# bentherien/point-cloud-reid

Hardware: AMD Instinct MI355X
Metric: siamese pair-comparisons/sec @1024 pts (higher is better)
Workload: dtype bf16x3

## Files before the change

### include/pcr.h

```cpp
#ifndef PCR_H_
#define PCR_H_

#ifdef __cplusplus
extern "C" {
#endif

typedef void *pcr_stream_t;

enum pcr_status {
  PCR_OK = 0,
  PCR_ERR_INVALID = 1,
  PCR_ERR_LAUNCH = 2
};

int pcr_abi_version(void);
#define PCR_PREC_F32 0
#define PCR_PREC_BF16X3 1
#define PCR_PREC_BF16 2
const char *pcr_status_string(int status);


int pcr_fps_f32(const float *xyz, float *temp, int *idx, int B, int N, int M, pcr_stream_t stream);

int pcr_fps_dist_f32(const float *dist, float *temp, int *idx, int B, int N, int M,
                     pcr_stream_t stream);

int pcr_pairwise_sqdist_f32(const float *a, const float *b, float *out, int B, int N, int M, int C, int norm,
                            pcr_stream_t stream);

int pcr_ball_query_f32(const float *centres, const float *xyz, int *idx, int B, int N, int M,
                       float min_r, float max_r, int K, pcr_stream_t stream);

int pcr_ball_query_cnt_f32(const float *centres, const float *xyz, int *idx, int *cnt, int B, int N, int M,
                           float min_r, float max_r, int K, pcr_stream_t stream);

long pcr_ball_query_rows_floats(int B, int M, int K);
int pcr_ball_query_rows_ok(int N, int K, float min_r);
int pcr_ball_query_rows_f32(const float *centres, const float *xyz, int *idx, int *cnt, float *rows, int B, int N, int M,
                            float min_r, float max_r, int K, pcr_stream_t stream);

int pcr_fps_ball_query_rows_ok(int N, int M, int K);
int pcr_fps_ball_query_rows_f32(const float *xyz, float *temp, int *idx, float *new_xyz, int *cnt, float *rows, int B,
                                int N, int M, float max_r, int K, pcr_stream_t stream);

int pcr_fps_py_f32(const float *xyz, float *temp, const int *start, int *idx, int B, int N, int M,
                   pcr_stream_t stream);
int pcr_query_ball_point_f32(const float *centres, const float *xyz, int *idx, int B, int N, int M, float radius,
                             int K, pcr_stream_t stream);

int pcr_knn_f32(const float *xyz, const float *centres, int *idx, float *dist2, int B, int N, int M,
                int K, pcr_stream_t stream);

int pcr_gather_fwd_f32(const float *feat, const int *idx, float *out, int B, int C, int N, int M,
                       pcr_stream_t stream);
int pcr_gather_bwd_f32(const float *grad_out, const int *idx, float *grad_feat, int B, int C, int N,
                       int M, pcr_stream_t stream);

int pcr_group_fwd_f32(const float *feat, const int *idx, float *out, int B, int C, int N, int S,
                      int K, pcr_stream_t stream);
int pcr_group_bwd_f32(const float *grad_out, const int *idx, float *grad_feat, int B, int C, int N,
                      int S, int K, pcr_stream_t stream);

int pcr_three_nn_f32(const float *unknown, const float *known, float *dist2, int *idx, int B, int N,
                     int M, pcr_stream_t stream);

int pcr_three_interp_fwd_f32(const float *feat, const int *idx, const float *weight, float *out,
                             int B, int C, int M, int N, pcr_stream_t stream);
int pcr_three_interp_bwd_f32(const float *grad_out, const int *idx, const float *weight,
                             float *grad_feat, int B, int C, int N, int M, pcr_stream_t stream);


int pcr_box_frames_f32(const float *boxes, float *frames, int T, pcr_stream_t stream);

int pcr_points_in_boxes_batch_f32(const float *points, const float *boxes, int *out, int B, int P, int T,
                                  pcr_stream_t stream);

int pcr_points_in_boxes_f32(const float *points, const float *boxes, int *out, int B, int P, int T, pcr_stream_t stream);

#define PCR_CROP_FRAME_SENSOR 0
#define PCR_CROP_FRAME_CENTRED 1
#define PCR_CROP_FRAME_BOX 2
#define PCR_CROP_RULE_TRACKER 0
#define PCR_CROP_RULE_DATASET 1
#define PCR_CROP_MAX_POINTS 2617344
#define PCR_CROP_MAX_BOXES 65536
#define PCR_CROP_MAX_SAMPLES 65536
#define PCR_CROP_MAX_STRIDE 16
int pcr_crop_boxes_ok(int P, int M, int n, int stride);
int pcr_crop_boxes_f32(const float *points, int stride, const float *boxes, const int *rand, const long long *seed,
                       float *clouds, int *lengths, int P, int M, int n, int frame, int rule, int z_is_centre,
                       pcr_stream_t stream);


int pcr_knn_prefix_f32(const float *xyz, int *idx, int B, int N, int S, int K, pcr_stream_t stream);
int pcr_knn_prefix2_f32(const float *xyz, int *idx, int *idx2, int B, int N, int S, int K, int S2, int K2,
                        pcr_stream_t stream);

long pcr_packed_weight_floats(int cout, int cin);
int pcr_pack_weight_f32(const float *w, int cout, int cin, float *packed);
long pcr_packed_weight_bf16_floats(int cout, int cin);
int pcr_pack_weight_bf16x2_f32(const float *w, int cout, int cin, float *packed);

typedef struct pcr_sa_params {
  int mode, B, N, S, K, D;
  int c1, c2, c3;
  const float *xyz, *feat;
  const int *idx, *centre_idx;
  const float *wp[3], *scale[3], *shift[3];
  const float *wa, *wpq;
  const float *wps[2], *shift_pad[2];
  const int *cnt;
  int *tile_ws;
  float *pq_ws;
  int pq_ready;
  int feat_point_major, out_point_major;
  float *out;
  const float *wa_packed;
  int precision;
  const float *wps_bf[2];
  const float *wa_shift_packed;
  const float *row_tab;
  int *claim_ws;
  int pq_has_xyz;
} pcr_sa_params;
int pcr_sa_mlp_f32(const pcr_sa_params *p, pcr_stream_t stream);
long pcr_sa_claim_ws_ints(int c1, int c2, int c3, int K, int N, int precision);
long pcr_sa_tile_ws_ints(int B, int S, int K, int c2, int c3);
int pcr_sa_krow_uses_tiles(int c1, int c2, int c3, int K, int precision);
int pcr_sa_uses_row_table(int c1, int c2, int c3, int K, int precision);

int pcr_dense_pm_f32(const float *x, const float *wp, float *y, int B, int cin, int cout, int L,
                     int x_point_major, pcr_stream_t stream);
int pcr_dense_pm_prec_f32(const float *x, const float *wp_bf, float *y, int B, int cin, int cout, int L,
                          int x_point_major, int precision, pcr_stream_t stream);
int pcr_dense_pm_xyz_f32(const float *x, const float *wp_bf, const float *xyz, const float *wxyz, float *y, int B, int cin,
                         int cout, int L, int x_point_major, int precision, int q_rows, int q_off, pcr_stream_t stream);
int pcr_sa_tables_take_xyz(int mode, int D, int c1, int c2, int c3, int K, int precision);

typedef struct pcr_attn_params {
  int B, Lq, Sk;
  int c1, c2, d, cout;
  int nhead;
  int q_pos, residual;
  const float *feat_q, *xyz_q;
  const float *feat_k, *xyz_k;
  const int *kv_index;
  const int *q_index;
  const float *pos0_w, *pos0_b;
  const float *wq, *bq;
  const float *wkv, *bkv;
  const float *wmerge;
  const float *wmlp0, *wmlp2;
  const float *ln1_g, *ln1_b, *ln2_g, *ln2_b;
  const float *wfinal, *bfinal; int cfinal;
  const float *wkv_wide, *bkv_wide, *wmerge_packed;
  float *kv;
  float *out;
  int precision;
  const float *wq_bf, *wmlp0_bf, *wmlp2_bf, *wfinal_bf;
  int kv_splits;
  float *kv_part;
  const float *wkv_bf;
  const float *wmlp0_bf_xpad;
  float *pool_out;
} pcr_attn_params;
long pcr_attn_kv_floats(int d);
int pcr_attn_kv_splits(int B, int Sk, int d);
int pcr_attn_kv_f32(const pcr_attn_params *p, pcr_stream_t stream);
int pcr_attn_apply_f32(const pcr_attn_params *p, pcr_stream_t stream);
int pcr_attn_apply_pool_ok(const pcr_attn_params *p);

typedef struct pcr_head_params {
  int P, C, L, groups;
  const float *o;
  const float *w1, *w2;
  const float *gn1_g, *gn1_b, *gn2_g, *gn2_b;
  const float *w_out, *b_out;
  float *pooled, *logits;
  const float *w1t, *w2t;
} pcr_head_params;
int pcr_pool_head_f32(const pcr_head_params *p, pcr_stream_t stream);

int pcr_pool_both_f32(const float *x, float *out, int B, int C, int L, pcr_stream_t stream);

int pcr_channel_max_f32(const float *x, float *out, int B, int C, int L, int window, pcr_stream_t stream);

int pcr_dense_f32(const float *x, const float *wp, const float *scale, const float *shift, float *y,
                  int B, int cin, int cout, int L, int act, pcr_stream_t stream);
int pcr_dense_xpm_f32(const float *x, const float *wp, const float *scale, const float *shift, float *y,
                      int B, int cin, int cout, int L, int act, pcr_stream_t stream);

int pcr_dense_gn_f32(const float *x, const float *wp, const float *gamma, const float *beta, const float *res,
                     float *y, int B, int cin, int cout, int L, int groups, int relu, pcr_stream_t stream);
int pcr_dense_prec_ok(int cin, int cout, int L);
int pcr_dense_prec_f32(const float *x, const float *wp_bf, const float *scale, const float *shift, float *y, int B, int cin,
                       int cout, int L, int act, int precision, pcr_stream_t stream);
int pcr_dense_gn_prec_f32(const float *x, const float *wp_bf, const float *gamma, const float *beta, const float *res,
                          float *y, int B, int cin, int cout, int L, int groups, int relu, int precision,
                          pcr_stream_t stream);
int pcr_dense_xpm_prec_ok(int cin, int cout, int L);
int pcr_dense_xpm_prec_f32(const float *x, const float *wp_bf, const float *scale, const float *shift, float *y, int B,
                           int cin, int cout, int L, int act, int precision, pcr_stream_t stream);


int pcr_max_over_l_f32(const float *x, float *out, int B, int C, int L, pcr_stream_t stream);

int pcr_dense_max_ok(int cin, int cout, int L);
int pcr_dense_max_f32(const float *x, const float *wp, const float *scale, const float *shift, float *out, int B, int cin,
                      int cout, int L, int act, pcr_stream_t stream);

int pcr_pack_bmm_f32(const float *t, float *wp_per_cloud, int B, int k, pcr_stream_t stream);
int pcr_dense_bmm_f32(const float *x, const float *wp_per_cloud, float *y, int B, int cin, int cout, int L,
                      pcr_stream_t stream);

int pcr_groupnorm_f32(const float *x, const float *gamma, const float *beta, const float *res, float *y, int B,
                      int C, int L, int groups, int relu, pcr_stream_t stream);


int pcr_knn_feat_f32(const float *x, float *xx_ws, int *idx, int B, int C, int N, int K, long x_bstride,
                     pcr_stream_t stream);

int pcr_edge_max_f32(const float *ta, const float *tb, const int *idx, const float *shift, float slope, float *out,
                     long out_bstride, float *out2, long out2_bstride, int B, int N, int Co, int K,
                     pcr_stream_t stream);

int pcr_local_attn_f32(const float *qkv, const int *idx, float *msg, int B, int N, int C, int K, int nhead, float eps,
                       pcr_stream_t stream);


int pcr_pack_weight_dev_f32(const float *w, int rows, int cols, int ld, int transpose, float *packed, pcr_stream_t stream);

int pcr_train_groups(int B, int L);
int pcr_train_groups_bwd(int B, int L, int cout, int cin);
struct pcr_tdense_fwd;
struct pcr_tdense_bwd;
int pcr_tdense_fwd_groups(const struct pcr_tdense_fwd *p);
int pcr_tdense_bwd_groups(const struct pcr_tdense_bwd *p);
int pcr_set_stream_min_blocks(int n);

typedef struct pcr_tdense_fwd {
  int B, cin1, cin2, cout, L;
  const float *x, *x2;
  const float *isc, *ish;
  int in_relu;
  const float *wp, *bias;
  const float *res;
  int out_relu;
  float *y;
  float *stats;
  int pool_K;
  const float *pool_gamma;
  float *pool_ymax;
  int *pool_arg;
} pcr_tdense_fwd;
int pcr_tdense_fwd_f32(const pcr_tdense_fwd *p, pcr_stream_t stream);
int pcr_tdense_fwd_pooled(const pcr_tdense_fwd *p);

typedef struct pcr_tdense_bwd {
  int B, cin1, cin2, cout, L;
  const float *g, *y;
  int dy_mode;
  const float *ka, *kb, *kc;
  const int *argmax;
  const float *pooled;
  int K, S;
  const float *x, *x2;
  const float *isc, *ish, *iinv;
  int in_relu;
  const float *wpT;
  float *dx, *dx2, *dstats, *dwp, *dbp;
  long part_stride;
  int precision;
  const float *wpT_bf;
} pcr_tdense_bwd;
int pcr_tdense_bwd_f32(const pcr_tdense_bwd *p, pcr_stream_t stream);
int pcr_pack_weight_bf16_dev_f32(const float *w, int rows, int cols, int ld, int transpose, float *packed,
                                 pcr_stream_t stream);

int pcr_local_attn_train_fwd_f32(const float *qkv, const int *idx, float *msg, int B, int N, int C, int K, int nhead,
                                 float eps, pcr_stream_t stream);
int pcr_local_attn_train_bwd_f32(const float *qkv, const int *idx, const float *g, float *dq, long dq_bstride, float *edge,
                                 int B, int N, int C, int K, int nhead, float eps, pcr_stream_t stream);

int pcr_reduce_parts_f32(const float *part, int nparts, long stride, int rows, int cols, int ld, float *out,
                         pcr_stream_t stream);

typedef struct pcr_reduce_job {
  const float *part;
  float *out;
  long stride;
  int nparts, rows, cols, ld;
} pcr_reduce_job;
int pcr_reduce_multi_f32(const pcr_reduce_job *jobs, int n, pcr_stream_t stream);

typedef struct pcr_bn_fwd_fin {
  const float *part;
  int nparts, C;
  double R;
  const float *gamma, *beta;
  float eps, momentum;
  float *running_mean, *running_var;
  float *scale, *shift, *inv_scale, *mean, *invstd;
  const float *shift0;
  int shift0_stride;
} pcr_bn_fwd_fin;
int pcr_bn_fwd_finalize_f32(const pcr_bn_fwd_fin *p, pcr_stream_t stream);

typedef struct pcr_bn_bwd_fin {
  const float *part;
  int nparts, C;
  double R;
  const float *gamma, *mean, *invstd;
  float *ka, *kb, *kc, *dgamma, *dbeta;
  const float *centre;
} pcr_bn_bwd_fin;
int pcr_bn_bwd_finalize_f32(const pcr_bn_bwd_fin *p, pcr_stream_t stream);

int pcr_sa_l1_fwd_f32(const float *xyz, const int *idx, const float *tab, const float *wa, const float *bias,
                      float *y, float *stats, int B, int N, int S, int K, int c1, pcr_stream_t stream);
int pcr_sa_l1_bwd_f32(const float *xyz, const int *idx, const float *g, const float *y, const float *ka,
                      const float *kb, const float *kc, float *dtab, float *dwa, int B, int N, int S, int K, int c1,
                      pcr_stream_t stream);
int pcr_sa_pool_fwd_f32(const float *y, const float *scale, const float *shift, float *pooled, int *argmax, float *ymax,
                        int B, int C, int S, int K, pcr_stream_t stream);
int pcr_sa_pool_bwd_stats_f32(const float *gp, const float *pooled, const float *ymax, float *part, float *gz, int B, int C,
                              int S, pcr_stream_t stream);

int pcr_tnorm_fwd_f32(const float *x, const float *gamma, const float *beta, const float *res, float *y, float *mean,
                      float *rstd, int B, int C, int L, int G, float eps, int relu, pcr_stream_t stream);
int pcr_tnorm_bwd_f32(const float *g, const float *x, const float *gamma, const float *mean, const float *rstd,
                      const float *y_relu, float *dx, float *dres, float *part, int B, int C, int L, int G,
                      pcr_stream_t stream);

typedef struct pcr_linattn {
  int B, Lq, Sk, d, H;
  float eps;
  const float *q, *k, *v;
  long q_bs, k_bs, v_bs;
  float *out, *A, *ks;
  const float *dout;
  float *dq, *dk, *dv;
  long dq_bs, dk_bs, dv_bs;
  int kv_roll;
} pcr_linattn;
int pcr_linattn_fwd_f32(const pcr_linattn *p, pcr_stream_t stream);
int pcr_linattn_bwd_f32(const pcr_linattn *p, pcr_stream_t stream);

typedef struct pcr_attn_tail {
  int B, L, d, c1, hid, out, residual;
  float eps;
  const float *msg, *res;
  const float *wm, *w0, *w2, *wmT, *w0T, *w2T;
  const float *g1, *b1, *g2, *b2;
  float *outp;
  const float *dout;
  float *dmsg, *dres, *parts;
  long part_stride;
  int precision;
  int fwd_precision;
} pcr_attn_tail;
int pcr_attn_tail_ok(int d, int c1, int hid, int out, int residual);
int pcr_attn_tail_part_floats(int d, int c1, int hid, int out);
int pcr_attn_tail_groups(const pcr_attn_tail *p);
int pcr_attn_tail_fwd_f32(const pcr_attn_tail *p, pcr_stream_t stream);
int pcr_attn_tail_bwd_f32(const pcr_attn_tail *p, pcr_stream_t stream);

typedef struct pcr_attn_head {
  int B, L, c, hd, d, np, src;
  const float *x, *xyz;
  const float *p1, *p2, *c1, *c2, *p2T;
  const float *w[3], *wT[3];
  float *outp;
  const float *dout;
  float *dx, *parts;
  long part_stride;
  int precision;
  int fwd_precision;
} pcr_attn_head;
int pcr_attn_head_ok(int c, int hd, int d, int np, int src);
int pcr_attn_head_part_floats(int c, int hd, int d, int np, int src);
int pcr_attn_head_groups(const pcr_attn_head *p);
int pcr_attn_head_fwd_f32(const pcr_attn_head *p, pcr_stream_t stream);
int pcr_attn_head_bwd_f32(const pcr_attn_head *p, pcr_stream_t stream);

int pcr_pool_pair_fwd_f32(const float *o, float *pooled, int *arg, int P, int C, int L, pcr_stream_t stream);
int pcr_pool_pair_bwd_f32(const float *g, const int *arg, float *dout, int P, int C, int L, pcr_stream_t stream);
int pcr_pool_both_fwd_f32(const float *o, float *pooled, int *arg, int P, int C, int L, pcr_stream_t stream);
int pcr_pool_both_bwd_f32(const float *g, const int *arg, float *dout, int P, int C, int L, pcr_stream_t stream);
int pcr_channel_max_fwd_f32(const float *x, float *y, int *arg, int B, int C, int L, int W, pcr_stream_t stream);
int pcr_channel_max_bwd_f32(const float *g, const int *arg, float *dx, int B, int C, int L, int W, pcr_stream_t stream);

int pcr_bn_sums_f32(const float *y, const float *g, const float *scale, const float *shift, int relu, float slope,
                    const float *centre, int centre_first, float *part, int nparts, int B, int C, int L,
                    pcr_stream_t stream);
int pcr_bn_affine_f32(const float *y, const float *g, const float *a0, const float *a1, const float *a2,
                      const float *scale, const float *shift, const float *centre, int relu, float slope, float *out,
                      int B, int C, int L, pcr_stream_t stream);
int pcr_edge_pool_fwd_f32(const float *y, const float *scale, const float *shift, float slope, float *pooled, int *arg,
                          float *yraw, int B, int C, int N, int K, pcr_stream_t stream);
int pcr_edge_pool_route_f32(const float *gp, const float *pooled, const int *arg, float slope, float *g, int B, int C,
                            int N, int K, pcr_stream_t stream);
int pcr_bmm_apply_f32(const float *x, const float *T, float *y, int B, int k, int N, int transposed, pcr_stream_t stream);
int pcr_bmm_dt_f32(const float *x, const float *dy, float *dT, int B, int k, int N, pcr_stream_t stream);

typedef struct pcr_pack_desc {
  const float *w;
  float *out;
  int rows, cols;
  int kind;
  int reserved;
} pcr_pack_desc;
int pcr_pack_weights_multi_f32(const pcr_pack_desc *descs_dev, int n, pcr_stream_t stream);

typedef struct pcr_opt_tensor {
  float *p, *g, *m, *v;
  long n;
  float step_size, bc2_sqrt, decay, one_m_beta1, beta2, one_m_beta2, eps, pad_;
} pcr_opt_tensor;
int pcr_opt_chunk(void);
int pcr_grad_sumsq_f32(const pcr_opt_tensor *tab, const int *chunk_tensor, const int *chunk_first, int n_chunks,
                       double *part, pcr_stream_t stream);
int pcr_adamw_step_f32(const pcr_opt_tensor *tab, const int *chunk_tensor, const int *chunk_first, int n_chunks,
                       const double *part, float max_norm, float *grad_norm, pcr_stream_t stream);


int pcr_wall_clock_khz(void);
int pcr_last_launch_arith(void);
int pcr_clock_probe(unsigned long long *ticks, int n_wg, int iters, pcr_stream_t stream);

#ifdef __cplusplus
}
#endif
#endif
```

### point-cloud-reid_amd/csrc/attn_kernels_impl.h

```cpp
#pragma once
#ifndef PCR_ATTN_PREC
#define PCR_ATTN_PREC 0
#endif
#include "tile_dense.h"

#include <stdio.h>

#include <vector>

namespace {
constexpr int kAPrec = PCR_ATTN_PREC;
struct AttnArgs {
  pcr_attn_params p;
  int dbg;
  int wpc;
};

constexpr int kATraceWgs = 512, kATraceRecs = 24, kATraceMarks = 8;
__device__ unsigned long long g_attn_trace[2 * kATraceWgs * kATraceRecs * kATraceMarks];


__device__ __forceinline__ void pos_hidden(float *dst, int RP, const float *P, const float *w0,
                                           const float *b0, int d, int T) {
  for (int e = threadIdx.x; e < d * T; e += blockDim.x) {
    const int o = e / T, t = e - o * T;
    const float v = w0[o * 3] * P[t] + w0[o * 3 + 1] * P[RP + t] + w0[o * 3 + 2] * P[2 * RP + t] + b0[o];
    dst[o * RP + t] = fmaxf(v, 0.f);
  }
}

__device__ __forceinline__ void load_xyz3(float *P, int RP, const float *xyz, int L, int t0, int T) {
  for (int e = threadIdx.x; e < 3 * T; e += blockDim.x) {
    const int c = e / T, t = e - c * T;
    P[c * RP + t] = t0 + t < L ? xyz[(size_t)(t0 + t) * 3 + c] : 0.f;
  }
}

__device__ __forceinline__ void attn_kv_fold_write(const pcr_attn_params &p, const float *KVl, const float *s_kt, size_t b) {
  const int d = p.d, dh = d / p.nhead, ld = d + 1, tid = threadIdx.x;
  float *kv = p.kv + b * ((size_t)d * d + d);
  const int d_o = kThreads / d, d_dd = kThreads - d_o * d;
  int o = tid / d, dd = tid - o * d;
  int v0 = (dd / dh) * dh;
  for (int e = tid; e < d * d; e += kThreads, o += d_o, dd += d_dd) {
    if (dd >= d) {
      dd -= d;
      o++;
    }
    if (d_dd) v0 = (dd / dh) * dh;
    const float *wm = p.wmerge + (size_t)o * d + v0;
    const float *kr = KVl + dd * ld + v0;
    float m = 0.f;
#pragma unroll 8
    for (int v = 0; v < dh; v++) m += wm[v] * kr[v];
    if constexpr (kAPrec == 0) {
      const int kb = dd >> 3, rem = dd & 7;
      kv[(((size_t)kb * d + o) * 2 + (rem & 1)) * 4 + (rem >> 1)] = m;
    } else {
      const int s16 = dd >> 4, kk = dd & 15;
      const int hh = (kk >> 2) & 1, jj = (kk & 3) + ((kk >> 3) << 2);
      const size_t unit = (((size_t)s16 * (d >> 5) + (o >> 5)) * 2) * 64 + hh * 32 + (o & 31);
      const __bf16 hi = (__bf16)m;
      const __bf16 lo = (__bf16)(m - (float)hi);
      __bf16 *img = reinterpret_cast<__bf16 *>(kv);
      img[unit * 8 + jj] = hi;
      img[(unit + 64) * 8 + jj] = lo;
    }
  }
  __syncthreads();
  if (tid < d) kv[(size_t)d * d + tid] = s_kt[tid];
}

__device__ __forceinline__ void attn_kv_fold_mfma(const pcr_attn_params &p, const float *KVt, const float *s_kt, size_t b) {
  const int d = p.d, dh = d / p.nhead, ld = d + 1, tid = threadIdx.x;
  float *kv = p.kv + b * ((size_t)d * d + d);
  for (int hd = 0; hd < p.nhead; hd++) {
    const float *wm = p.wmerge_packed + (size_t)(hd * dh / 8) * d * 8;
    tile_dense(KVt + (size_t)(hd * dh) * ld + hd * dh, dh, ld, dh >> 5, wm, d, [&](float m, int o, int t) {
      const int dd = hd * dh + t;
      if constexpr (kAPrec == 0) {
        const int kb = dd >> 3, rem = dd & 7;
        kv[(((size_t)kb * d + o) * 2 + (rem & 1)) * 4 + (rem >> 1)] = m;
      } else {
        const int s16 = dd >> 4, kk = dd & 15;
        const int hh = (kk >> 2) & 1, jj = (kk & 3) + ((kk >> 3) << 2);
        const size_t unit = (((size_t)s16 * (d >> 5) + (o >> 5)) * 2) * 64 + hh * 32 + (o & 31);
        const __bf16 hi = (__bf16)m;
        const __bf16 lo = (__bf16)(m - (float)hi);
        __bf16 *img = reinterpret_cast<__bf16 *>(kv);
        img[unit * 8 + jj] = hi;
        img[(unit + 64) * 8 + jj] = lo;
      }
    });
  }
  __syncthreads();
  if (tid < d) kv[(size_t)d * d + tid] = s_kt[tid];
}

template <int TB, int NR, int WSEL, int NTW, bool BFP = false>
__device__ __forceinline__ void attn_kv_body(const AttnArgs &a) {
  constexpr int T = 32 * TB, RP = T + 1;
  constexpr int NPF = 4;
  extern __shared__ __attribute__((aligned(16))) float smem[];
  const pcr_attn_params &p = a.p;
  const int d = p.d, c2 = p.c2;
  float *XH = smem;
  float *KB = XH;
  float *VB = XH + d * RP;
  float *P = XH + (c2 + d) * RP;
  float *s_w0 = P + 3 * RP, *s_b0 = s_w0 + 3 * d;
  const int tail_a = (c2 + d + 3) * RP + 4 * d, tail_b = d * (d + 1) + d;
  float *s_ks = smem + (tail_a > tail_b ? tail_a : tail_b);
  const int tid = threadIdx.x, lane = tid & 63, wave = tid >> 6;
  const int l31 = lane & 31, h = lane >> 5;
  const size_t b = blockIdx.x;
  for (int e = tid; e < 3 * d; e += kThreads) s_w0[e] = p.pos0_w[e];
  for (int e = tid; e < d; e += kThreads) s_b0[e] = p.pos0_b[e];
  const float *feat = p.feat_k + b * c2 * p.Sk;
  const float *xyz = p.xyz_k + b * p.Sk * 3;
  const int nb = d >> 5, nT = nb * nb;
  const int dh = d / p.nhead;
  const float sk = (float)p.Sk;
  const float *bkv = p.bkv;

  f32x16 acc[NTW];
#pragma unroll
  for (int i = 0; i < NTW; i++)
#pragma unroll
    for (int r = 0; r < 16; r++) acc[i][r] = 0.f;
  int tile_ib[NTW];
#pragma unroll
  for (int it = 0; it < NTW; it++) tile_ib[it] = (wave + 4 * it) / nb;
  const int krow = tid % d, kpart = tid / d, kparts = kThreads / d;
  float ksum = 0.f;

  const int Q = T >> 2, npieces = c2 * Q;
#ifndef PCR_KV_PREFETCH
#define PCR_KV_PREFETCH 1
#endif
  const bool vec_ok = PCR_KV_PREFETCH && ((p.Sk & 3) == 0) && ((reinterpret_cast<size_t>(feat) & 15) == 0) && npieces <= NPF * kThreads;
  f32x4 pf[NPF];
  auto fetch = [&](int t0) {
#pragma unroll
    for (int u = 0; u < NPF; u++) {
      const int e = tid + u * kThreads;
      const int c = e / Q, q = e - c * Q;
      const bool ok = e < npieces;
      pf[u] = *reinterpret_cast<const f32x4 *>(feat + (size_t)(ok ? c : 0) * p.Sk + t0 + 4 * (ok ? q : 0));
    }
  };
  auto stash = [&]() {
#pragma unroll
    for (int u = 0; u < NPF; u++) {
      const int e = tid + u * kThreads;
      if (e < npieces) {
        const int c = e / Q, q = e - c * Q;
        float *dst = XH + c * RP + 4 * q;
        dst[0] = pf[u][0];
        dst[1] = pf[u][1];
        dst[2] = pf[u][2];
        dst[3] = pf[u][3];
      }
    }
  };
  const int nsplit = p.kv_splits > 1 ? p.kv_splits : 1;
  const int ntile = (p.Sk + T - 1) / T, tps = (ntile + nsplit - 1) / nsplit;
  const int t_lo = (int)blockIdx.y * tps * T;
  const int t_hi = (t_lo + tps * T) < p.Sk ? (t_lo + tps * T) : p.Sk;
  bool have = false;
  if (vec_ok && t_lo + T <= p.Sk && t_lo < t_hi) {
    fetch(t_lo);
    have = true;
  }
  for (int t0 = t_lo; t0 < t_hi; t0 += T) {
    const int valid = p.Sk - t0;
    if (have) stash();
    else load_tile(XH, RP, feat, c2, c2, p.Sk, t0, T);
    load_xyz3(P, RP, xyz, p.Sk, t0, T);
    __syncthreads();
    have = vec_ok && t0 + 2 * T <= p.Sk && t0 + T < t_hi;
    pos_hidden(XH + c2 * RP, RP, P, s_w0, s_b0, d, T);
    __syncthreads();
    auto kv_epi = [&](const f32x16 &acc, int cb, int tb, int l31, int h) {
      const int t = tb * 32 + l31;
      float *dst = XH + (cb * 32 + 4 * h) * RP + t;
      const bool live = t < valid;
      if (cb * 32 < d) {
#pragma unroll
        for (int r = 0; r < 16; r++) dst[((r & 3) + 8 * (r >> 2)) * RP] = live ? elu1(acc[r]) : 0.f;
      } else {
#pragma unroll
        for (int r = 0; r < 16; r++) dst[((r & 3) + 8 * (r >> 2)) * RP] = live ? acc[r] / sk : 0.f;
      }
    };
    auto kv_hook = [&]() { if (have) fetch(t0 + T); };
    if constexpr (BFP && kAPrec != 0 && WSEL != 0)
      tile_dense2p<kAPrec, TB, NR, WSEL, true>(XH, c2 + d, p.wkv_bf, 2 * d, true, kv_epi, bkv, nullptr, kv_hook);
    else
      tile_dense2<TB, NR, WSEL, true>(XH, c2 + d, p.wkv, 2 * d, true, kv_epi, bkv, nullptr, kv_hook);
    __syncthreads();
    {
      const float *row = KB + krow * RP;
      for (int t = kpart; t < T; t += kparts) ksum += row[t];
    }
#pragma unroll
    for (int it = 0; it < NTW; it++) {
      const int item = wave + 4 * it;
      if (item < nT) {
        const int ib = tile_ib[it], jb = item - ib * nb;
        const float *ap = KB + (ib * 32 + l31) * RP + h;
        const float *bp = VB + (jb * 32 + l31) * RP + h;
#pragma unroll 4
        for (int ks = 0; ks < T / 2; ks++)
          acc[it] = __builtin_amdgcn_mfma_f32_32x32x2f32(ap[2 * ks], bp[2 * ks], acc[it], 0, 0, 0);
      }
    }
    __syncthreads();
  }
  if (nsplit > 1) {
    float *part = p.kv_part + ((size_t)b * nsplit + blockIdx.y) * ((size_t)d * d + d);
    s_ks[tid] = ksum;
#pragma unroll
    for (int it = 0; it < NTW; it++) {
      const int item = wave + 4 * it;
      if (item < nT) {
        const int ib = tile_ib[it], jb = item - ib * nb;
#pragma unroll
        for (int r = 0; r < 16; r++)
          part[(size_t)(ib * 32 + (r & 3) + 8 * (r >> 2) + 4 * h) * d + jb * 32 + l31] = acc[it][r];
      }
    }
    __syncthreads();
    if (tid < d) {
      float s = 0.f;
      for (int pp = 0; pp < kparts; pp++) s += s_ks[pp * d + tid];
      part[(size_t)d * d + tid] = s;
    }
    return;
  }
  float *KVl = smem;
  const int ld = d + 1;
  const bool mfma_fold = p.wmerge_packed != nullptr && (dh & 31) == 0 && (d & 31) == 0;
  float *s_kt = smem + d * ld;
  s_ks[tid] = ksum;
#pragma unroll
  for (int it = 0; it < NTW; it++) {
    const int item = wave + 4 * it;
    if (item < nT) {
      const int ib = tile_ib[it], jb = item - ib * nb;
      const int v = jb * 32 + l31;
      const int hv = v / dh;
      const bool aligned = (dh & 31) == 0;
      const bool same_blk = (ib * 32) / dh == hv;
#pragma unroll
      for (int r = 0; r < 16; r++) {
        const int dd = ib * 32 + (r & 3) + 8 * (r >> 2) + 4 * h;
        const bool same = aligned ? same_blk : (dd / dh == hv);
        if (mfma_fold) KVl[v * ld + dd] = same ? acc[it][r] : 0.f;
        else KVl[dd * ld + v] = same ? acc[it][r] : 0.f;
      }
    }
  }
  __syncthreads();
  if (tid < d) {
    float s = 0.f;
    for (int pp = 0; pp < kparts; pp++) s += s_ks[pp * d + tid];
    s_kt[tid] = s;
  }
  if (mfma_fold) attn_kv_fold_mfma(p, KVl, s_kt, b);
  else attn_kv_fold_write(p, KVl, s_kt, b);
}

template <int TB, int NR, int WSEL, int NTW>
__global__ __launch_bounds__(kThreads) void attn_kv_kernel(AttnArgs a) {
  attn_kv_body<TB, NR, WSEL, NTW>(a);
}
template <int TB, int NR, int WSEL, int NTW>
__global__ __launch_bounds__(kThreads) __attribute__((amdgpu_waves_per_eu(3, 3))) void attn_kv_kernel_o3(AttnArgs a) {
  attn_kv_body<TB, NR, WSEL, NTW>(a);
}
template <int TB, int NR, int WSEL, int NTW, bool BFP = false>
__global__ __launch_bounds__(kThreads) __attribute__((amdgpu_waves_per_eu(2, 2))) void attn_kv_kernel_o2(AttnArgs a) {
  attn_kv_body<TB, NR, WSEL, NTW, BFP>(a);
}

constexpr int kKvsWaves = 8;
template <bool DIAG, bool BF, int XS = 4, bool ONEW = false>
__global__ __launch_bounds__(64 * kKvsWaves) __attribute__((amdgpu_waves_per_eu(2, 2)))
void attn_kv_stream64_kernel(AttnArgs a) {
  static_assert(BF || XS == 4, "the f32 form is c2 = 64 only");
  constexpr int D = 64, LD = D + 1, KVS = D * LD + D;
  constexpr int NKV = DIAG ? 2 : 4;
  constexpr int C2 = 16 * XS, WU = BF ? (XS + 4) * 512 : 4096, MINW = XS == 8 ? 4 : 2;
  extern __shared__ __attribute__((aligned(16))) float smem[];
  const pcr_attn_params &p = a.p;
  f32x4 *s_w = reinterpret_cast<f32x4 *>(smem);
  f32x4 *s_p0 = reinterpret_cast<f32x4 *>(smem + 4 * WU);
  float *s_bkv = smem + 4 * WU + 256;
  float *s_wm = s_bkv + 128;
  float *s_red = s_wm + D * LD;
  const int tid = threadIdx.x, lane = tid & 63, j = lane & 31, h = lane >> 5;
  const int wave = __builtin_amdgcn_readfirstlane(tid >> 6);
  {
    const f32x4 *src = reinterpret_cast<const f32x4 *>(BF ? p.wkv_bf : p.wkv);
    for (int e = tid; e < WU; e += 64 * kKvsWaves) s_w[e] = src[e];
    for (int e = tid; e < D * D; e += 64 * kKvsWaves) s_wm[(e >> 6) * LD + (e & 63)] = p.wmerge[e];
    if (tid < D) s_p0[tid] = f32x4{p.pos0_w[3 * tid], p.pos0_w[3 * tid + 1], p.pos0_w[3 * tid + 2], p.pos0_b[tid]};
    if (tid < 2 * D) s_bkv[tid] = p.bkv[tid];
  }
  __syncthreads();
  const int nblk = p.Sk >> 5;
  constexpr int kMaxWpc = 4;
  const int wpc = nblk < kMaxWpc ? nblk : kMaxWpc;
  int wpc2 = 1;
  while (wpc2 * 2 <= wpc) wpc2 *= 2;
  if (wpc2 < MINW) wpc2 = MINW;
  if constexpr (ONEW) wpc2 = 1;
  const int cpg = kKvsWaves / wpc2;
  const int cslot = wave / wpc2, wsub = wave - cslot * wpc2;
  const float inv_sk = 1.0f / (float)p.Sk;
  float bias[4];
#pragma unroll
  for (int cb = 0; cb < 4; cb++) bias[cb] = s_bkv[cb * 32 + j];
  const int dh = D / p.nhead;
#ifdef PCR_SA_TRACE_BUILD
  const bool tracing = (a.dbg & 256) && lane == 0 && (wave == 0 || wave == 5) && blockIdx.x < kATraceWgs;
  unsigned long long *trace = g_attn_trace + (size_t)(2 * blockIdx.x + (wave ? 1 : 0)) * (kATraceRecs * kATraceMarks);
  int trace_it = 0;
#define PCR_AMARK(m)                                                                                       \
  do {                                                                                                     \
    if (tracing && trace_it < kATraceRecs) trace[trace_it * kATraceMarks + (m)] = __builtin_readcyclecounter(); \
  } while (0)
#define PCR_ANEXT() trace_it++
#else
#define PCR_AMARK(m) do { } while (0)
#define PCR_ANEXT() do { } while (0)
#endif
  for (long c0 = (long)blockIdx.x * cpg; c0 < p.B; c0 += (long)gridDim.x * cpg) {
    const long b = c0 + cslot;
    const bool live = b < p.B;
    PCR_AMARK(4);
    f32x16 kv[NKV];
#pragma unroll
    for (int i = 0; i < NKV; i++)
#pragma unroll
      for (int r = 0; r < 16; r++) kv[i][r] = 0.f;
    float ks0 = 0.f, ks1 = 0.f;
    if (live) {
      const float *feat = p.feat_k + (size_t)b * C2 * p.Sk;
      const float *xyz = p.xyz_k + (size_t)b * p.Sk * 3;
      const __amdgpu_buffer_rsrc_t rfeat =
          __builtin_amdgcn_make_buffer_rsrc(const_cast<float *>(feat), 0, C2 * p.Sk * 4, 0x00020000);
      for (int blk = wsub; blk < nblk; blk += wpc2) {
        asm volatile("" ::: "memory");
        PCR_AMARK(0);
        const int t = blk * 32 + j;
        const float px = xyz[3 * t], py = xyz[3 * t + 1], pz = xyz[3 * t + 2];
        f32x16 acc[4];
        if constexpr (!BF) {
          float xr[64];
          {
            const int vo = (h * p.Sk + t) * 4;
#pragma unroll
            for (int s2 = 0; s2 < 32; s2++)
              xr[s2] = __builtin_bit_cast(float, __builtin_amdgcn_raw_buffer_load_b32(rfeat, vo, s2 * 2 * p.Sk * 4, 0));
          }
#pragma unroll
          for (int s2 = 0; s2 < 32; s2++) {
            const f32x4 w = s_p0[2 * s2 + h];
            const float v = w[0] * px + w[1] * py + w[2] * pz + w[3];
            xr[32 + s2] = fmaxf(v, 0.f);
          }
#pragma unroll
          for (int s2 = 0; s2 < 32; s2++) asm volatile("" : "+v"(xr[s2]));
#pragma unroll
          for (int cb = 0; cb < 4; cb++)
#pragma unroll
            for (int r = 0; r < 16; r++) acc[cb][r] = 0.f;
#pragma unroll
          for (int kb = 0; kb < 16; kb++) {
            f32x4 w[4];
#pragma unroll
            for (int cb = 0; cb < 4; cb++) w[cb] = s_w[((kb * 128 + cb * 32 + j) << 1) + h];
#pragma unroll
            for (int i = 0; i < 4; i++)
#pragma unroll
              for (int cb = 0; cb < 4; cb++)
                acc[cb] = __builtin_amdgcn_mfma_f32_32x32x2f32(xr[4 * kb + i], w[cb][i], acc[cb], 0, 0, 0);
          }
        } else {
          float xf[8 * XS];
          {
            const int vo = (4 * h * p.Sk + t) * 4;
#pragma unroll
            for (int e = 0; e < 8 * XS; e++) {
              const int ch = 16 * (e >> 3) + bf_kpos(0, e & 7);
              xf[e] = __builtin_bit_cast(float, __builtin_amdgcn_raw_buffer_load_b32(rfeat, vo, ch * p.Sk * 4, 0));
            }
          }
          bf16x8 ah[XS + 4], al[XS + 4];
#pragma unroll
          for (int s2 = 0; s2 < 4; s2++) {
            float hv[8];
#pragma unroll
            for (int e = 0; e < 8; e++) {
              const f32x4 w = s_p0[16 * s2 + bf_kpos(0, e) + 4 * h];
              const float v = w[0] * px + w[1] * py + w[2] * pz + w[3];
              hv[e] = relu_i(v);
            }
            bf_split8(hv, ah[XS + s2], al[XS + s2], true);
          }
#pragma unroll
          for (int e = 0; e < 8 * XS; e++) asm volatile("" : "+v"(xf[e]));
#pragma unroll
          for (int s2 = 0; s2 < XS; s2++) {
            float xv[8];
#pragma unroll
            for (int e = 0; e < 8; e++) xv[e] = xf[8 * s2 + e];
            bf_split8(xv, ah[s2], al[s2], true);
          }
#pragma unroll
          for (int cb = 0; cb < 4; cb++)
#pragma unroll
            for (int r = 0; r < 16; r++) acc[cb][r] = 0.f;
          PCR_AMARK(1);
          const bf16x8 *wb = reinterpret_cast<const bf16x8 *>(s_w) + lane;
#pragma unroll
          for (int s2 = 0; s2 < XS + 4; s2++) {
            bf16x8 wh[4], wl[4];
#pragma unroll
            for (int cb = 0; cb < 4; cb++) {
              wh[cb] = wb[((s2 * 4 + cb) * 2) * 64];
              wl[cb] = wb[((s2 * 4 + cb) * 2 + 1) * 64];
            }
#pragma unroll
            for (int cb = 0; cb < 4; cb++) acc[cb] = __builtin_amdgcn_mfma_f32_32x32x16_bf16(ah[s2], wh[cb], acc[cb], 0, 0, 0);
#pragma unroll
            for (int cb = 0; cb < 4; cb++) acc[cb] = __builtin_amdgcn_mfma_f32_32x32x16_bf16(al[s2], wh[cb], acc[cb], 0, 0, 0);
#pragma unroll
            for (int cb = 0; cb < 4; cb++) acc[cb] = __builtin_amdgcn_mfma_f32_32x32x16_bf16(ah[s2], wl[cb], acc[cb], 0, 0, 0);
          }
        }
        PCR_AMARK(2);
#pragma unroll
        for (int r = 0; r < 16; r++) {
          acc[0][r] = elu1(acc[0][r] + bias[0]);
          acc[1][r] = elu1(acc[1][r] + bias[1]);
          acc[2][r] = (acc[2][r] + bias[2]) * inv_sk;
          acc[3][r] = (acc[3][r] + bias[3]) * inv_sk;
          ks0 += acc[0][r];
          ks1 += acc[1][r];
        }
#pragma unroll
        for (int i = 0; i < NKV; i++) {
          const int ib = DIAG ? i : (i >> 1), jb = DIAG ? i : (i & 1);
#pragma unroll
          for (int r = 0; r < 16; r++) {
            if constexpr (ONEW) kv[i] = __builtin_amdgcn_mfma_f32_32x32x2f32(acc[2 + jb][r], acc[ib][r], kv[i], 0, 0, 0);
            else kv[i] = __builtin_amdgcn_mfma_f32_32x32x2f32(acc[ib][r], acc[2 + jb][r], kv[i], 0, 0, 0);
          }
        }
        PCR_AMARK(3);
      }
    }
    PCR_AMARK(5);
    ks0 += __shfl_xor(ks0, 32, 64);
    ks1 += __shfl_xor(ks1, 32, 64);
    if constexpr (ONEW) {
      if (live) {
        float *kvo = p.kv + (size_t)b * ((size_t)D * D + D);
        bf16x8 *img = reinterpret_cast<bf16x8 *>(kvo);
#pragma unroll
        for (int db = 0; db < 2; db++) {
          const int hd = (db * 32 + j) / dh;
#pragma unroll
          for (int ob = 0; ob < 2; ob++) {
            f32x16 m;
#pragma unroll
            for (int r = 0; r < 16; r++) m[r] = 0.f;
#pragma unroll
            for (int i = 0; i < NKV; i++) {
              const int ib = DIAG ? i : (i >> 1), jb = DIAG ? i : (i & 1);
              if (ib != db) continue;
              const float *wr = s_wm + (ob * 32 + j) * LD + jb * 32 + 4 * h;
#pragma unroll
              for (int r = 0; r < 16; r++) {
                const int vl = (r & 3) + 8 * (r >> 2);
                const float av = (jb * 32 + vl + 4 * h) / dh == hd ? kv[i][r] : 0.f;
                m = __builtin_amdgcn_mfma_f32_32x32x2f32(av, wr[vl], m, 0, 0, 0);
              }
            }
#pragma unroll
            for (int G = 0; G < 2; G++) {
              float v[8];
#pragma unroll
              for (int e = 0; e < 8; e++) v[e] = m[8 * G + e];
              bf16x8 hi, lo;
              bf_split8(v, hi, lo, true);
              const size_t unit = (((size_t)(db * 2 + G) * (D >> 5) + ob) * 2) * 64 + h * 32 + j;
              img[unit] = hi;
              img[unit + 64] = lo;
            }
          }
        }
        if (h == 0) {
          kvo[(size_t)D * D + j] = ks0;
          kvo[(size_t)D * D + 32 + j] = ks1;
        }
      }
      PCR_AMARK(6);
      PCR_AMARK(7);
      PCR_ANEXT();
      continue;
    }
    float *KVl = s_red + cslot * KVS, *s_kt = KVl + D * LD;
    for (int round = 0; round < wpc2; round++) {
      if (wsub == round) {
#pragma unroll
        for (int i = 0; i < NKV; i++) {
          const int ib = DIAG ? i : (i >> 1), jb = DIAG ? i : (i & 1);
#pragma unroll
          for (int r = 0; r < 16; r++) {
            const int dd = ib * 32 + (r & 3) + 8 * (r >> 2) + 4 * h, v = jb * 32 + j;
            float *dst = KVl + dd * LD + v;
            *dst = round == 0 ? kv[i][r] : *dst + kv[i][r];
          }
        }
        if (h == 0) {
          s_kt[j] = round == 0 ? ks0 : s_kt[j] + ks0;
          s_kt[32 + j] = round == 0 ? ks1 : s_kt[32 + j] + ks1;
        }
      }
      __syncthreads();
    }
    PCR_AMARK(6);
    if (live) {
      float *kvo = p.kv + (size_t)b * ((size_t)D * D + D);
      for (int ti = wsub; ti < 4; ti += wpc2) {
        const int ob = ti >> 1, db = ti & 1;
        const float *ap = s_wm + (ob * 32 + j) * LD + h;
        const float *bp = KVl + (db * 32 + j) * LD + h;
        const int hd = (db * 32 + j) / dh;
        f32x16 m;
#pragma unroll
        for (int r = 0; r < 16; r++) m[r] = 0.f;
        const int s_lo = DIAG ? db * 16 : 0, s_hi = DIAG ? db * 16 + 16 : 32;
        if constexpr (kAPrec == 0) {
#pragma unroll 4
          for (int s2 = s_lo; s2 < s_hi; s2++) {
            const float bv = bp[2 * s2];
            m = __builtin_amdgcn_mfma_f32_32x32x2f32(ap[2 * s2], (2 * s2 + h) / dh == hd ? bv : 0.f, m, 0, 0, 0);
          }
          const int dd = db * 32 + j;
#pragma unroll
          for (int r = 0; r < 16; r++) {
            const int o = ob * 32 + (r & 3) + 8 * (r >> 2) + 4 * h;
            const int kb = dd >> 3, rem = dd & 7;
            kvo[(((size_t)kb * D + o) * 2 + (rem & 1)) * 4 + (rem >> 1)] = m[r];
          }
        } else {
#pragma unroll 4
          for (int s2 = s_lo; s2 < s_hi; s2++) {
            const float bv = bp[2 * s2];
            m = __builtin_amdgcn_mfma_f32_32x32x2f32((2 * s2 + h) / dh == hd ? bv : 0.f, ap[2 * s2], m, 0, 0, 0);
          }
          bf16x8 *img = reinterpret_cast<bf16x8 *>(kvo);
#pragma unroll
          for (int G = 0; G < 2; G++) {
            float v[8];
#pragma unroll
            for (int e = 0; e < 8; e++) v[e] = m[8 * G + e];
            bf16x8 hi, lo;
            bf_split8(v, hi, lo, true);
            const size_t unit = (((size_t)(db * 2 + G) * (D >> 5) + ob) * 2) * 64 + h * 32 + j;
            img[unit] = hi;
            img[unit + 64] = lo;
          }
        }
      }
      for (int e = wsub * 64 + lane; e < D; e += 64 * wpc2) kvo[(size_t)D * D + e] = s_kt[e];
    }
    PCR_AMARK(7);
    PCR_ANEXT();
    __syncthreads();
  }
#undef PCR_AMARK
#undef PCR_ANEXT
}

#if PCR_ATTN_PREC != 0
__global__ __launch_bounds__(64 * kKvsWaves) __attribute__((amdgpu_waves_per_eu(2, 4)))
void attn_kv_stream32_kernel(AttnArgs a) {
  constexpr int D = 32, LD = D + 1, KVS = D * LD + D;
  extern __shared__ __attribute__((aligned(16))) float smem[];
  const pcr_attn_params &p = a.p;
  f32x4 *s_w = reinterpret_cast<f32x4 *>(smem);
  f32x4 *s_p0 = reinterpret_cast<f32x4 *>(smem + 4096);
  float *s_bkv = smem + 4096 + 128;
  float *s_wm = s_bkv + 64;
  float *s_red = s_wm + D * LD;
  const int tid = threadIdx.x, lane = tid & 63, j = lane & 31, h = lane >> 5;
  const int wave = __builtin_amdgcn_readfirstlane(tid >> 6);
  {
    const f32x4 *src = reinterpret_cast<const f32x4 *>(p.wkv_bf);
    for (int e = tid; e < 1024; e += 64 * kKvsWaves) s_w[e] = src[e];
    for (int e = tid; e < D * D; e += 64 * kKvsWaves) s_wm[(e >> 5) * LD + (e & 31)] = p.wmerge[e];
    if (tid < D) s_p0[tid] = f32x4{p.pos0_w[3 * tid], p.pos0_w[3 * tid + 1], p.pos0_w[3 * tid + 2], p.pos0_b[tid]};
    if (tid < 2 * D) s_bkv[tid] = p.bkv[tid];
  }
  __syncthreads();
  const int nblk = p.Sk >> 5;
  const int wpc = nblk < kKvsWaves ? nblk : kKvsWaves;
  int wpc2 = 1;
  while (wpc2 * 2 <= wpc) wpc2 *= 2;
  if (wpc2 < 2) wpc2 = 2;
  const int cpg = kKvsWaves / wpc2;
  const int cslot = wave / wpc2, wsub = wave - cslot * wpc2;
  const float inv_sk = 1.0f / (float)p.Sk;
  const float bias0 = s_bkv[j], bias1 = s_bkv[32 + j];
  const int dh = D / p.nhead;
  for (long c0 = (long)blockIdx.x * cpg; c0 < p.B; c0 += (long)gridDim.x * cpg) {
    const long b = c0 + cslot;
    const bool live = b < p.B;
    f32x16 kv;
#pragma unroll
    for (int r = 0; r < 16; r++) kv[r] = 0.f;
    float ks = 0.f;
    if (live) {
      const float *feat = p.feat_k + (size_t)b * D * p.Sk;
      const float *xyz = p.xyz_k + (size_t)b * p.Sk * 3;
      const __amdgpu_buffer_rsrc_t rfeat =
          __builtin_amdgcn_make_buffer_rsrc(const_cast<float *>(feat), 0, D * p.Sk * 4, 0x00020000);
      for (int blk = wsub; blk < nblk; blk += wpc2) {
        asm volatile("" ::: "memory");
        const int t = blk * 32 + j;
        const float px = xyz[3 * t], py = xyz[3 * t + 1], pz = xyz[3 * t + 2];
        float xf[16];
        {
          const int vo = (4 * h * p.Sk + t) * 4;
#pragma unroll
          for (int e = 0; e < 16; e++) {
            const int ch = 16 * (e >> 3) + bf_kpos(0, e & 7);
            xf[e] = __builtin_bit_cast(float, __builtin_amdgcn_raw_buffer_load_b32(rfeat, vo, ch * p.Sk * 4, 0));
          }
        }
        bf16x8 ah[4], al[4];
#pragma unroll
        for (int s2 = 0; s2 < 2; s2++) {
          float hv[8];
#pragma unroll
          for (int e = 0; e < 8; e++) {
            const f32x4 w = s_p0[16 * s2 + bf_kpos(0, e) + 4 * h];
            const float v = w[0] * px + w[1] * py + w[2] * pz + w[3];
            hv[e] = relu_i(v);
          }
          bf_split8(hv, ah[2 + s2], al[2 + s2], true);
        }
#pragma unroll
        for (int e = 0; e < 16; e++) asm volatile("" : "+v"(xf[e]));
#pragma unroll
        for (int s2 = 0; s2 < 2; s2++) {
          float xv[8];
#pragma unroll
          for (int e = 0; e < 8; e++) xv[e] = xf[8 * s2 + e];
          bf_split8(xv, ah[s2], al[s2], true);
        }
        f32x16 acc[2];
#pragma unroll
        for (int cb = 0; cb < 2; cb++)
#pragma unroll
          for (int r = 0; r < 16; r++) acc[cb][r] = 0.f;
        const bf16x8 *wb = reinterpret_cast<const bf16x8 *>(s_w) + lane;
#pragma unroll
        for (int s2 = 0; s2 < 4; s2++) {
          bf16x8 wh[2], wl[2];
#pragma unroll
          for (int cb = 0; cb < 2; cb++) {
            wh[cb] = wb[((s2 * 2 + cb) * 2) * 64];
            wl[cb] = wb[((s2 * 2 + cb) * 2 + 1) * 64];
          }
#pragma unroll
          for (int cb = 0; cb < 2; cb++) acc[cb] = __builtin_amdgcn_mfma_f32_32x32x16_bf16(ah[s2], wh[cb], acc[cb], 0, 0, 0);
#pragma unroll
          for (int cb = 0; cb < 2; cb++) acc[cb] = __builtin_amdgcn_mfma_f32_32x32x16_bf16(al[s2], wh[cb], acc[cb], 0, 0, 0);
#pragma unroll
          for (int cb = 0; cb < 2; cb++) acc[cb] = __builtin_amdgcn_mfma_f32_32x32x16_bf16(ah[s2], wl[cb], acc[cb], 0, 0, 0);
        }
#pragma unroll
        for (int r = 0; r < 16; r++) {
          acc[0][r] = elu1(acc[0][r] + bias0);
          acc[1][r] = (acc[1][r] + bias1) * inv_sk;
          ks += acc[0][r];
        }
#pragma unroll
        for (int r = 0; r < 16; r++) kv = __builtin_amdgcn_mfma_f32_32x32x2f32(acc[0][r], acc[1][r], kv, 0, 0, 0);
      }
    }
    ks += __shfl_xor(ks, 32, 64);
    float *KVl = s_red + cslot * KVS, *s_kt = KVl + D * LD;
    for (int round = 0; round < wpc2; round++) {
      if (wsub == round) {
#pragma unroll
        for (int r = 0; r < 16; r++) {
          float *dst = KVl + ((r & 3) + 8 * (r >> 2) + 4 * h) * LD + j;
          *dst = round == 0 ? kv[r] : *dst + kv[r];
        }
        if (h == 0) s_kt[j] = round == 0 ? ks : s_kt[j] + ks;
      }
      __syncthreads();
    }
    if (live && wsub == 0) {
      float *kvo = p.kv + (size_t)b * ((size_t)D * D + D);
      const float *ap = s_wm + j * LD + h;
      const float *bp = KVl + j * LD + h;
      const int hd = j / dh;
      f32x16 m;
#pragma unroll
      for (int r = 0; r < 16; r++) m[r] = 0.f;
#pragma unroll 4
      for (int s2 = 0; s2 < 16; s2++) {
        const float bv = bp[2 * s2];
        m = __builtin_amdgcn_mfma_f32_32x32x2f32((2 * s2 + h) / dh == hd ? bv : 0.f, ap[2 * s2], m, 0, 0, 0);
      }
      bf16x8 *img = reinterpret_cast<bf16x8 *>(kvo);
#pragma unroll
      for (int G = 0; G < 2; G++) {
        float v[8];
#pragma unroll
        for (int e = 0; e < 8; e++) v[e] = m[8 * G + e];
        bf16x8 hi, lo;
        bf_split8(v, hi, lo, true);
        const size_t unit = (((size_t)G * (D >> 5)) * 2) * 64 + h * 32 + j;
        img[unit] = hi;
        img[unit + 64] = lo;
      }
      if (lane < D) kvo[(size_t)D * D + lane] = s_kt[lane];
    }
    __syncthreads();
  }
}
#endif

__global__ __launch_bounds__(kThreads) void attn_kv_fold_kernel(AttnArgs a) {
  extern __shared__ __attribute__((aligned(16))) float smem[];
  const pcr_attn_params &p = a.p;
  const int d = p.d, dh = d / p.nhead, ld = d + 1, nsplit = p.kv_splits, tid = threadIdx.x;
  const size_t b = blockIdx.x, per = (size_t)d * d + d;
  float *KVl = smem, *s_kt = smem + d * ld;
  const float *part = p.kv_part + b * nsplit * per;
  for (int e = tid; e < d * d + d; e += kThreads) {
    float v = part[e];
    for (int y = 1; y < nsplit; y++) v += part[(size_t)y * per + e];
    if (e < d * d) {
      const int dd = e / d, c = e - dd * d;
      KVl[dd * ld + c] = (dd / dh == c / dh) ? v : 0.f;
    } else {
      s_kt[e - d * d] = v;
    }
  }
  __syncthreads();
  attn_kv_fold_write(p, KVl, s_kt, b);
}

#if PCR_ATTN_PREC == 0
template <int NRW>
__global__ __launch_bounds__(kThreads) void attn_kv_wide_kernel(AttnArgs a) {
  constexpr int TB = 1, T = 32, RP = 33, BAND = 64, RPK = BAND + 1;
  extern __shared__ __attribute__((aligned(16))) float smem[];
  const pcr_attn_params &p = a.p;
  const int d = p.d, c2 = p.c2, dh = d / p.nhead;
  const int g = blockIdx.x, hd = (g * BAND) / dh;
  const int OPW = BAND + dh;
  float *XH = smem;
  float *KB = XH, *VB = XH + BAND * RP;
  float *P = XH + (c2 + d) * RP;
  float *s_w0 = P + 3 * RP, *s_b0 = s_w0 + 3 * d;
  float *s_ks = s_b0 + d;
  const int tid = threadIdx.x, lane = tid & 63, wave = tid >> 6;
  const int l31 = lane & 31, h = lane >> 5;
  const size_t b = blockIdx.y;
  for (int e = tid; e < 3 * d; e += kThreads) s_w0[e] = p.pos0_w[e];
  for (int e = tid; e < d; e += kThreads) s_b0[e] = p.pos0_b[e];
  const float *feat = p.feat_k + b * c2 * p.Sk;
  const float *xyz = p.xyz_k + b * p.Sk * 3;
  const float sk = (float)p.Sk;
  const float *wband = p.wkv_wide + (size_t)g * ((size_t)ceil8(c2 + d) * OPW);
  const float *bband = p.bkv_wide + (size_t)g * OPW;
  const int nj = dh >> 5, nT = 2 * nj;
  f32x16 acc[4];
#pragma unroll
  for (int i = 0; i < 4; i++)
#pragma unroll
    for (int r = 0; r < 16; r++) acc[i][r] = 0.f;
  const int krow = tid & (BAND - 1), kpart = tid >> 6;
  float ksum = 0.f;
  for (int t0 = 0; t0 < p.Sk; t0 += T) {
    const int valid = p.Sk - t0;
    load_tile(XH, RP, feat, c2, c2, p.Sk, t0, T);
    load_xyz3(P, RP, xyz, p.Sk, t0, T);
    __syncthreads();
    pos_hidden(XH + c2 * RP, RP, P, s_w0, s_b0, d, T);
    __syncthreads();
    tile_dense2<TB, NRW, 0, true>(XH, c2 + d, wband, OPW, true,
                                  [&](const f32x16 &acc, int cb, int tb, int l31, int h) {
      const int t = tb * 32 + l31;
      float *dst = XH + (cb * 32 + 4 * h) * RP + t;
      const bool live = t < valid;
      if (cb * 32 < BAND) {
#pragma unroll
        for (int r = 0; r < 16; r++) dst[((r & 3) + 8 * (r >> 2)) * RP] = live ? elu1(acc[r]) : 0.f;
      } else {
#pragma unroll
        for (int r = 0; r < 16; r++) dst[((r & 3) + 8 * (r >> 2)) * RP] = live ? acc[r] / sk : 0.f;
      }
    }, bband);
    __syncthreads();
    {
      const float *row = KB + krow * RP;
      for (int t = kpart; t < T; t += 4) ksum += row[t];
    }
#pragma unroll
    for (int it = 0; it < 4; it++) {
      const int item = wave + 4 * it;
      if (item < nT) {
        const int ib = item / nj, jb = item - ib * nj;
        const float *ap = KB + (ib * 32 + l31) * RP + h;
        const float *bp = VB + (jb * 32 + l31) * RP + h;
#pragma unroll 4
        for (int ks = 0; ks < T / 2; ks++)
          acc[it] = __builtin_amdgcn_mfma_f32_32x32x2f32(ap[2 * ks], bp[2 * ks], acc[it], 0, 0, 0);
      }
    }
    __syncthreads();
  }
  float *KVt = smem;
  s_ks[tid] = ksum;
  __syncthreads();
  const float ks_total = tid < BAND ? s_ks[tid] + s_ks[64 + tid] + s_ks[128 + tid] + s_ks[192 + tid] : 0.f;
  __syncthreads();
#pragma unroll
  for (int it = 0; it < 4; it++) {
    const int item = wave + 4 * it;
    if (item < nT) {
      const int ib = item / nj, jb = item - ib * nj;
      const int v = jb * 32 + l31;
#pragma unroll
      for (int r = 0; r < 16; r++) KVt[v * RPK + ib * 32 + (r & 3) + 8 * (r >> 2) + 4 * h] = acc[it][r];
    }
  }
  __syncthreads();
  float *kv = p.kv + b * ((size_t)d * d + d);
  if (tid < BAND) kv[(size_t)d * d + g * BAND + tid] = ks_total;
  const float *wm = p.wmerge_packed + (size_t)(hd * dh / 8) * d * 8;
  tile_dense(KVt, dh, RPK, 2, wm, d, [&](float m, int o, int t) {
    const int dd = g * BAND + t;
    const int kb = dd >> 3, rem = dd & 7;
    kv[(((size_t)kb * d + o) * 2 + (rem & 1)) * 4 + (rem >> 1)] = m;
  });
}

#endif

template <int TB, int NR>
__global__ __launch_bounds__(kThreads) void attn_apply_kernel(AttnArgs a) {
  constexpr int T = 32 * TB, RP = T + 1;
  extern __shared__ __attribute__((aligned(16))) float smem[];
  const pcr_attn_params &p = a.p;
  const int d = p.d, c1 = p.c1, cout = p.cout;
  const int catC = c1 + d, catP = ceil8(catC);
  int rowsU = catP > 2 * d ? catP : 2 * d;
  if (ceil32(cout) > rowsU) rowsU = ceil32(cout);
  if (ceil32(p.cfinal) > rowsU) rowsU = ceil32(p.cfinal);
  float *U = smem;
  float *P = U + rowsU * RP;
  float *zs = P + 3 * RP;
  float *red = zs + p.nhead * RP;
  float *cst = red + 2 * (kThreads / T) * T;
  float *s_ksum = cst, *s_ln1g = cst + d, *s_ln1b = cst + 2 * d, *s_ln2g = cst + 3 * d, *s_ln2b = s_ln2g + cout;
  float *s_w0 = s_ln2b + cout, *s_b0 = s_w0 + 3 * d;
  const int tid = threadIdx.x;
  const size_t b = blockIdx.y;
  const int t0 = blockIdx.x * T;
  const size_t bq_ = p.q_index ? (size_t)p.q_index[b] : b;
  const float *feat = p.feat_q + bq_ * c1 * p.Lq;
  const size_t kb_ = p.kv_index ? (size_t)p.kv_index[b] : b;
  const float *kv = p.kv + kb_ * ((size_t)d * d + d);
  const int dh = d / p.nhead;
  for (int e = tid; e < d; e += kThreads) {
    s_ksum[e] = kv[(size_t)d * d + e];
    s_ln1g[e] = p.ln1_g[e];
    s_ln1b[e] = p.ln1_b[e];
    if (p.q_pos) {
      s_w0[3 * e] = p.pos0_w[3 * e];
      s_w0[3 * e + 1] = p.pos0_w[3 * e + 1];
      s_w0[3 * e + 2] = p.pos0_w[3 * e + 2];
      s_b0[e] = p.pos0_b[e];
    }
  }
  for (int e = tid; e < cout; e += kThreads) {
    s_ln2g[e] = p.ln2_g[e];
    s_ln2b[e] = p.ln2_b[e];
  }
  const float *ksum = s_ksum;
  float *MSG = U + c1 * RP;

  load_tile(U, RP, feat, c1, c1, p.Lq, t0, T);
  if (p.q_pos) {
    load_xyz3(P, RP, p.xyz_q + bq_ * p.Lq * 3, p.Lq, t0, T);
    __syncthreads();
    pos_hidden(MSG, RP, P, s_w0, s_b0, d, T);
    for (int e = tid; e < (catP - catC) * T; e += kThreads) U[(catC + e / T) * RP + e % T] = 0.f;
  } else {
    for (int e = tid; e < (catP - c1) * T; e += kThreads) U[(c1 + e / T) * RP + e % T] = 0.f;
  }
  __syncthreads();
  tile_dense2p<kAPrec, TB, NR>(U, p.q_pos ? catP : ceil8(c1), p.wq, d, true,
                               [&](float v, int o, int t) { MSG[o * RP + t] = elu1(v); }, p.bq);
  __syncthreads();
  for (int e = tid; e < p.nhead * T; e += kThreads) {
    const int hd = e / T, t = e - hd * T;
    float z = 0.f;
    for (int c = 0; c < dh; c++) z += MSG[(hd * dh + c) * RP + t] * ksum[hd * dh + c];
    zs[hd * RP + t] = (1.0f / (z + 1e-6f)) * (float)p.Sk;
  }
  __syncthreads();
  for (int hd = 0; hd < p.nhead; hd++)
    for (int e = tid; e < dh * T; e += kThreads) {
      const int o = hd * dh + e / T, t = e % T;
      MSG[o * RP + t] *= zs[hd * RP + t];
    }
  __syncthreads();
  tile_dense2p<kAPrec, TB, NR>(MSG, d, kv, d, true, [&](float v, int o, int t) { MSG[o * RP + t] = v; });
  __syncthreads();
  tile_layernorm(MSG, d, RP, T, s_ln1g, s_ln1b, red);
  tile_dense2p<kAPrec, TB, NR>(U, catP, p.wmlp0, 2 * d, true, [&](float v, int o, int t) { U[o * RP + t] = fmaxf(v, 0.f); });
  __syncthreads();
  tile_dense2p<kAPrec, TB, NR>(U, 2 * d, p.wmlp2, ceil32(cout), true, [&](float v, int o, int t) { U[o * RP + t] = v; });
  __syncthreads();
  tile_layernorm(U, cout, RP, T, s_ln2g, s_ln2b, red);
  if (p.residual) {
    for (int e = tid; e < cout * T; e += kThreads) {
      const int c = e / T, t = e - c * T;
      if (t0 + t < p.Lq) U[c * RP + t] += feat[(size_t)c * p.Lq + t0 + t];
    }
    __syncthreads();
  }
  int cres = cout;
  if (p.cfinal) {
    const int cf = p.cfinal;
    tile_dense2p<kAPrec, TB, NR>(U, cout, p.wfinal, ceil32(cf), true, [&](float v, int o, int t) { U[o * RP + t] = v; },
                                 p.bfinal);
    __syncthreads();
    cres = cf;
  }
  float *out = p.out + b * cres * p.Lq;
  for (int e = tid; e < cres * T; e += kThreads) {
    const int c = e / T, t = e - c * T;
    if (t0 + t < p.Lq) out[(size_t)c * p.Lq + t0 + t] = U[c * RP + t];
  }
}

#if PCR_ATTN_PREC != 0
constexpr int kApsWaves = 8;
template <bool QPOS, int C1S, int CF, int NOB = 2, int ND = 2, bool POOL = false>
__global__ __launch_bounds__(64 * kApsWaves) __attribute__((amdgpu_waves_per_eu(2, 2)))
void attn_apply_stream64_kernel(AttnArgs a) {
  static_assert(!QPOS || C1S == 2 * ND, "q_pos needs c1 == d");
  static_assert(NOB <= 2 || (NOB == 4 && !CF), "cout = 128 has no trailing conv");
  static_assert(!POOL || (!CF && NOB == 2), "pooled output: cout = 64, no trailing conv");
  constexpr int D = 32 * ND, SD = 2 * ND;
  constexpr int SQ = C1S + (QPOS ? SD : 0), S0 = C1S + SD, NX = 8 * C1S;
  extern __shared__ __attribute__((aligned(16))) float smem[];
  const pcr_attn_params &p = a.p;
  bf16x8 *s_wq = reinterpret_cast<bf16x8 *>(smem);
  bf16x8 *s_w0 = s_wq + SQ * ND * 128;
  bf16x8 *s_w2 = s_w0 + S0 * ND * 256;
  float *s_c = reinterpret_cast<float *>(s_w2 + ND * NOB * 512);
  f32x4 *s_p0 = reinterpret_cast<f32x4 *>(s_c + 448);
  float *s_ks = reinterpret_cast<float *>(s_p0 + 64);
  const int tid = threadIdx.x, lane = tid & 63, j = lane & 31, h = lane >> 5;
  const int wave = __builtin_amdgcn_readfirstlane(tid >> 6);
  {
    const f32x4 *wq = reinterpret_cast<const f32x4 *>(p.wq),
                *w0 = reinterpret_cast<const f32x4 *>((p.c1 & 15) ? p.wmlp0_bf_xpad : p.wmlp0),
                *w2 = reinterpret_cast<const f32x4 *>(p.wmlp2);
    f32x4 *dq = reinterpret_cast<f32x4 *>(s_wq), *d0 = reinterpret_cast<f32x4 *>(s_w0), *d2 = reinterpret_cast<f32x4 *>(s_w2);
    for (int e = tid; e < SQ * ND * 128; e += 64 * kApsWaves) dq[e] = wq[e];
    for (int e = tid; e < S0 * ND * 256; e += 64 * kApsWaves) d0[e] = w0[e];
    for (int e = tid; e < ND * NOB * 512; e += 64 * kApsWaves) d2[e] = w2[e];
    if (tid < D) {
      s_c[tid] = p.bq[tid];
      s_c[64 + tid] = p.ln1_g[tid];
      s_c[128 + tid] = p.ln1_b[tid];

      if (QPOS) s_p0[tid] = f32x4{p.pos0_w[3 * tid], p.pos0_w[3 * tid + 1], p.pos0_w[3 * tid + 2], p.pos0_b[tid]};
    }
    if (tid < 32 * NOB) {
      s_c[192 + tid] = p.ln2_g[tid];
      s_c[192 + 32 * NOB + tid] = p.ln2_b[tid];
    }
    if (CF && tid < 32 * CF) s_c[320 + tid] = p.bfinal[tid];
  }
  __syncthreads();
  const int nblk = p.Lq >> 5;
  const long nitem = (long)p.B * nblk;
  const int dh = D / p.nhead;
  const float skf = (float)p.Sk;
  float *ksw = s_ks + wave * 64;
  auto cvec = [&](const float *base, int cb, int g) __attribute__((always_inline)) {
    return *reinterpret_cast<const f32x4 *>(base + 32 * cb + 8 * g + 4 * h);
  };
  auto to_ops = [&](const f32x16 &acc, int G, bf16x8 &oh, bf16x8 &ol) __attribute__((always_inline)) {
    float v[8];
#pragma unroll
    for (int e = 0; e < 8; e++) v[e] = acc[8 * G + e];
    bf_split8(v, oh, ol, true);
  };
#ifdef PCR_SA_TRACE_BUILD
  const bool tracing = (a.dbg & 256) && lane == 0 && (wave == 0 || wave == 5) && blockIdx.x < kATraceWgs;
  unsigned long long *trace = g_attn_trace + (size_t)(2 * blockIdx.x + (wave ? 1 : 0)) * (kATraceRecs * kATraceMarks);
  int trace_it = 0;
#define PCR_AMARK(m)                                                                                       \
  do {                                                                                                     \
    if (tracing && trace_it < kATraceRecs) trace[trace_it * kATraceMarks + (m)] = __builtin_readcyclecounter(); \
  } while (0)
#define PCR_ANEXT() trace_it++
#else
#define PCR_AMARK(m) do { } while (0)
#define PCR_ANEXT() do { } while (0)
#endif
  const long nwav = (long)gridDim.x * kApsWaves, gw = (long)blockIdx.x * kApsWaves + wave;
  long pc = gw;
  int pblk = 0;
  float pmax = -INFINITY, psum = 0.f;
  for (long it = gw; POOL ? pc < p.B : it < nitem; it += POOL ? 0 : nwav) {
    asm volatile("" ::: "memory");
    PCR_AMARK(0);
    const long b = POOL ? pc : it / nblk;
    const int blk = POOL ? pblk : (int)(it - b * nblk);
    const size_t bq_ = p.q_index ? (size_t)p.q_index[b] : (size_t)b;
    const size_t kb_ = p.kv_index ? (size_t)p.kv_index[b] : (size_t)b;
    const float *kvp = p.kv + kb_ * ((size_t)D * D + D);
    const int t = blk * 32 + j;
    const __amdgpu_buffer_rsrc_t rfeat = __builtin_amdgcn_make_buffer_rsrc(
        const_cast<float *>(p.feat_q + bq_ * p.c1 * p.Lq), 0, p.c1 * p.Lq * 4, 0x00020000);
    const int vo = (4 * h * p.Lq + t) * 4;
    float xf[NX];
#pragma unroll
    for (int e = 0; e < NX; e++) {
      const int ch = 16 * (e >> 3) + bf_kpos(0, e & 7);
      xf[e] = __builtin_bit_cast(float, __builtin_amdgcn_raw_buffer_load_b32(rfeat, vo, ch * p.Lq * 4, 0));
    }
    if (lane < D) ksw[lane] = kvp[(size_t)D * D + lane];
    bf16x8 bh[4 * ND], bl[4 * ND];
    if constexpr (QPOS) {
      const float *xyz = p.xyz_q + (bq_ * p.Lq + t) * 3;
      const float px = xyz[0], py = xyz[1], pz = xyz[2];
#pragma unroll
      for (int s2 = 0; s2 < SD; s2++) {
        float hv[8];
#pragma unroll
        for (int e = 0; e < 8; e++) {
          const f32x4 w = s_p0[16 * s2 + bf_kpos(0, e) + 4 * h];
          const float v = w[0] * px + w[1] * py + w[2] * pz + w[3];
          hv[e] = relu_i(v);
        }
        bf_split8(hv, bh[C1S + s2], bl[C1S + s2], true);
      }
    }
#pragma unroll
    for (int e = 0; e < NX; e++) asm volatile("" : "+v"(xf[e]));
#pragma unroll
    for (int s2 = 0; s2 < C1S; s2++) {
      float xv[8];
#pragma unroll
      for (int e = 0; e < 8; e++) xv[e] = xf[8 * s2 + e];
      bf_split8(xv, bh[s2], bl[s2], true);
    }
    PCR_AMARK(1);
    f32x16 q[ND];
#pragma unroll
    for (int cb = 0; cb < ND; cb++)
#pragma unroll
      for (int r = 0; r < 16; r++) q[cb][r] = 0.f;
    {
      const bf16x8 *wb = s_wq + lane;
#pragma unroll
      for (int s2 = 0; s2 < SQ; s2++) {
        bf16x8 wh[ND], wl[ND];
#pragma unroll
        for (int cb = 0; cb < ND; cb++) {
          wh[cb] = wb[((s2 * ND + cb) * 2) * 64];
          wl[cb] = wb[((s2 * ND + cb) * 2 + 1) * 64];
        }
#pragma unroll
        for (int cb = 0; cb < ND; cb++) q[cb] = __builtin_amdgcn_mfma_f32_32x32x16_bf16(wh[cb], bh[s2], q[cb], 0, 0, 0);
#pragma unroll
        for (int cb = 0; cb < ND; cb++) q[cb] = __builtin_amdgcn_mfma_f32_32x32x16_bf16(wh[cb], bl[s2], q[cb], 0, 0, 0);
#pragma unroll
        for (int cb = 0; cb < ND; cb++) q[cb] = __builtin_amdgcn_mfma_f32_32x32x16_bf16(wl[cb], bh[s2], q[cb], 0, 0, 0);
      }
    }
    PCR_AMARK(2);
    bf16x8 mh[SD][ND], ml[SD][ND];
    {
      const bf16x8 *mb = reinterpret_cast<const bf16x8 *>(kvp) + lane;
#pragma unroll
      for (int s2 = 0; s2 < SD; s2++)
#pragma unroll
        for (int cb = 0; cb < ND; cb++) {
          mh[s2][cb] = mb[((s2 * ND + cb) * 2) * 64];
          ml[s2][cb] = mb[((s2 * ND + cb) * 2 + 1) * 64];
        }
    }
    __builtin_amdgcn_fence(__ATOMIC_RELEASE, "wavefront");
    __builtin_amdgcn_wave_barrier();
    __builtin_amdgcn_fence(__ATOMIC_ACQUIRE, "wavefront");
    float z16[2][2] = {{0.f, 0.f}, {0.f, 0.f}};
#pragma unroll
    for (int cb = 0; cb < ND; cb++)
#pragma unroll
      for (int g = 0; g < 4; g++) {
        const f32x4 bqv = cvec(s_c, cb, g), ksv = cvec(ksw, cb, g);
        float zz = 0.f;
#pragma unroll
        for (int qq = 0; qq < 4; qq++) {
          const float v = elu1(q[cb][4 * g + qq] + bqv[qq]);
          q[cb][4 * g + qq] = v;
          zz += v * ksv[qq];
        }
        if ((g & 1) == 0) z16[cb][g >> 1] = zz;
        else z16[cb][g >> 1] += zz;
      }
    float zs[2][2];
    {
      float za = z16[0][0], zb = z16[0][1], zc = z16[1][0], zd = z16[1][1];
      if (dh >= 32) {
        za += zb; zb = za;
        zc += zd; zd = zc;
      }
      if (ND == 2 && dh >= 64) {
        za += zc; zb = za; zc = za; zd = za;
      }
      za += __shfl_xor(za, 32, 64);
      zb += __shfl_xor(zb, 32, 64);
      zc += __shfl_xor(zc, 32, 64);
      zd += __shfl_xor(zd, 32, 64);
      zs[0][0] = (1.0f / (za + 1e-6f)) * skf;
      zs[0][1] = (1.0f / (zb + 1e-6f)) * skf;
      zs[1][0] = (1.0f / (zc + 1e-6f)) * skf;
      zs[1][1] = (1.0f / (zd + 1e-6f)) * skf;
    }
#pragma unroll
    for (int cb = 0; cb < ND; cb++)
#pragma unroll
      for (int r = 0; r < 16; r++) q[cb][r] *= zs[cb][r >> 3];
    bf16x8 ch_[SD], cl_[SD];
#pragma unroll
    for (int cb = 0; cb < ND; cb++)
#pragma unroll
      for (int G = 0; G < 2; G++) to_ops(q[cb], G, ch_[2 * cb + G], cl_[2 * cb + G]);
    f32x16 m[ND];
#pragma unroll
    for (int cb = 0; cb < ND; cb++)
#pragma unroll
      for (int r = 0; r < 16; r++) m[cb][r] = 0.f;
#pragma unroll
    for (int s2 = 0; s2 < SD; s2++) {
#pragma unroll
      for (int cb = 0; cb < ND; cb++) m[cb] = __builtin_amdgcn_mfma_f32_32x32x16_bf16(mh[s2][cb], ch_[s2], m[cb], 0, 0, 0);
#pragma unroll
      for (int cb = 0; cb < ND; cb++) m[cb] = __builtin_amdgcn_mfma_f32_32x32x16_bf16(mh[s2][cb], cl_[s2], m[cb], 0, 0, 0);
#pragma unroll
      for (int cb = 0; cb < ND; cb++) m[cb] = __builtin_amdgcn_mfma_f32_32x32x16_bf16(ml[s2][cb], ch_[s2], m[cb], 0, 0, 0);
    }
    auto layernorm = [&](auto &v, auto nb_tag, const float *gam, const float *bet) __attribute__((always_inline)) {
      constexpr int NB = decltype(nb_tag)::value;
      float sm = 0.f;
#pragma unroll
      for (int cb = 0; cb < NB; cb++)
#pragma unroll
        for (int r = 0; r < 16; r++) sm += v[cb][r];
      sm += __shfl_xor(sm, 32, 64);
      const float mean = sm / (32.0f * NB);
      float vr = 0.f;
#pragma unroll
      for (int cb = 0; cb < NB; cb++)
#pragma unroll
        for (int r = 0; r < 16; r++) {
          const float dlt = v[cb][r] - mean;
          vr += dlt * dlt;
        }
      vr += __shfl_xor(vr, 32, 64);
      const float inv = 1.0f / sqrtf(vr / (32.0f * NB) + 1e-5f);
#pragma unroll
      for (int cb = 0; cb < NB; cb++)
#pragma unroll
        for (int g = 0; g < 4; g++) {
          const f32x4 gv = cvec(gam, cb, g), bv = cvec(bet, cb, g);
#pragma unroll
          for (int qq = 0; qq < 4; qq++) v[cb][4 * g + qq] = (v[cb][4 * g + qq] - mean) * inv * gv[qq] + bv[qq];
        }
    };
    PCR_AMARK(3);
    layernorm(m, std::integral_constant<int, ND>{}, s_c + 64, s_c + 128);
    PCR_AMARK(4);
#pragma unroll
    for (int s2 = 0; s2 < C1S; s2++) {
      float xv[8];
#pragma unroll
      for (int e = 0; e < 8; e++) xv[e] = xf[8 * s2 + e];
      bf_split8(xv, bh[s2], bl[s2], true);
    }
#pragma unroll
    for (int cb = 0; cb < ND; cb++)
#pragma unroll
      for (int G = 0; G < 2; G++) to_ops(m[cb], G, bh[C1S + 2 * cb + G], bl[C1S + 2 * cb + G]);
    f32x16 f[SD];
#pragma unroll
    for (int cb = 0; cb < SD; cb++)
#pragma unroll
      for (int r = 0; r < 16; r++) f[cb][r] = 0.f;
    {
      const bf16x8 *wb = s_w0 + lane;
#pragma unroll
      for (int s2 = 0; s2 < S0; s2++) {
        bf16x8 wh[SD], wl[SD];
#pragma unroll
        for (int cb = 0; cb < SD; cb++) {
          wh[cb] = wb[((s2 * SD + cb) * 2) * 64];
          wl[cb] = wb[((s2 * SD + cb) * 2 + 1) * 64];
        }
#pragma unroll
        for (int cb = 0; cb < SD; cb++) f[cb] = __builtin_amdgcn_mfma_f32_32x32x16_bf16(wh[cb], bh[s2], f[cb], 0, 0, 0);
#pragma unroll
        for (int cb = 0; cb < SD; cb++) f[cb] = __builtin_amdgcn_mfma_f32_32x32x16_bf16(wh[cb], bl[s2], f[cb], 0, 0, 0);
#pragma unroll
        for (int cb = 0; cb < SD; cb++) f[cb] = __builtin_amdgcn_mfma_f32_32x32x16_bf16(wl[cb], bh[s2], f[cb], 0, 0, 0);
      }
    }
#pragma unroll
    for (int cb = 0; cb < SD; cb++) {
#pragma unroll
      for (int r = 0; r < 16; r++) f[cb][r] = relu_i(f[cb][r]);
#pragma unroll
      for (int G = 0; G < 2; G++) to_ops(f[cb], G, bh[2 * cb + G], bl[2 * cb + G]);
    }
    PCR_AMARK(5);
    f32x16 o[NOB];
#pragma unroll
    for (int cb = 0; cb < NOB; cb++)
#pragma unroll
      for (int r = 0; r < 16; r++) o[cb][r] = 0.f;
    {
      const bf16x8 *wb = s_w2 + lane;
#pragma unroll
      for (int s2 = 0; s2 < 4 * ND; s2++) {
        bf16x8 wh[NOB], wl[NOB];
#pragma unroll
        for (int cb = 0; cb < NOB; cb++) {
          wh[cb] = wb[((s2 * NOB + cb) * 2) * 64];
          wl[cb] = wb[((s2 * NOB + cb) * 2 + 1) * 64];
        }
#pragma unroll
        for (int cb = 0; cb < NOB; cb++) o[cb] = __builtin_amdgcn_mfma_f32_32x32x16_bf16(wh[cb], bh[s2], o[cb], 0, 0, 0);
#pragma unroll
        for (int cb = 0; cb < NOB; cb++) o[cb] = __builtin_amdgcn_mfma_f32_32x32x16_bf16(wh[cb], bl[s2], o[cb], 0, 0, 0);
#pragma unroll
        for (int cb = 0; cb < NOB; cb++) o[cb] = __builtin_amdgcn_mfma_f32_32x32x16_bf16(wl[cb], bh[s2], o[cb], 0, 0, 0);
      }
    }
    PCR_AMARK(6);
    layernorm(o, std::integral_constant<int, NOB>{}, s_c + 192, s_c + 192 + 32 * NOB);
    if constexpr (C1S == 2 * NOB) {
      if (p.residual) {
#pragma unroll
        for (int cb = 0; cb < NOB; cb++)
#pragma unroll
          for (int r = 0; r < 16; r++) o[cb][r] += xf[16 * cb + r];
      }
    }
    if constexpr (POOL) {
      float vm[16], vs[16];
      {
        const bool up = (j & 1) != 0;
#pragma unroll
        for (int r = 0; r < 16; r++) {
          const float lo_ = o[r >> 4][r & 15], hi_ = o[(r + 16) >> 4][(r + 16) & 15];
          const float tk = up ? hi_ : lo_, uk = up ? lo_ : hi_;
          const float pu = __uint_as_float(pcr_sort_partner<2, 1>(__float_as_uint(uk), lane));
          vm[r] = fmaxf(tk, pu);
          vs[r] = tk + pu;
        }
      }
#define PCR_POOL_STEP(N, J, BIT)                                                                      \
      {                                                                                               \
        const bool up = (j & BIT) != 0;                                                               \
        _Pragma("unroll") for (int r = 0; r < N; r++) {                                               \
          const float tm = up ? vm[r + N] : vm[r], um = up ? vm[r] : vm[r + N];                       \
          const float ts = up ? vs[r + N] : vs[r], us = up ? vs[r] : vs[r + N];                       \
          vm[r] = fmaxf(tm, __uint_as_float(pcr_sort_partner<2 * J, J>(__float_as_uint(um), lane)));  \
          vs[r] = ts + __uint_as_float(pcr_sort_partner<2 * J, J>(__float_as_uint(us), lane));        \
        }                                                                                             \
      }
      PCR_POOL_STEP(8, 2, 2)
      PCR_POOL_STEP(4, 4, 4)
      PCR_POOL_STEP(2, 8, 8)
      PCR_POOL_STEP(1, 16, 16)
#undef PCR_POOL_STEP
      pmax = fmaxf(pmax, vm[0]);
      psum += vs[0];
      if (++pblk == nblk) {
        const int e = ((j & 1) << 4) | ((j & 2) << 2) | (j & 4) | ((j & 8) >> 2) | ((j & 16) >> 4);
        const int ch = 16 * (e >> 3) + bf_kpos(h, e & 7);
        float *po = p.pool_out + (size_t)b * 128;
        po[ch] = pmax;
        po[64 + ch] = psum;
        pmax = -INFINITY;
        psum = 0.f;
        pblk = 0;
        pc += nwav;
      }
    } else if constexpr (!CF) {
      const __amdgpu_buffer_rsrc_t rout =
          __builtin_amdgcn_make_buffer_rsrc(p.out + (size_t)b * (32 * NOB) * p.Lq, 0, 32 * NOB * p.Lq * 4, 0x00020000);
#pragma unroll
      for (int e = 0; e < 16 * NOB; e++) {
        const int ch = 16 * (e >> 3) + bf_kpos(0, e & 7);
        const float v = o[e >> 4][e & 15];
        __builtin_amdgcn_raw_buffer_store_b32(__builtin_bit_cast(unsigned, v), rout, vo, ch * p.Lq * 4, 0);
      }
    } else {
#pragma unroll
      for (int cb = 0; cb < NOB; cb++)
#pragma unroll
        for (int G = 0; G < 2; G++) to_ops(o[cb], G, bh[2 * cb + G], bl[2 * cb + G]);
      f32x16 fo[CF ? CF : 1];
#pragma unroll
      for (int cb = 0; cb < CF; cb++)
#pragma unroll
        for (int r = 0; r < 16; r++) fo[cb][r] = 0.f;
      const bf16x8 *wb = reinterpret_cast<const bf16x8 *>(p.wfinal) + lane;
#pragma unroll
      for (int s2 = 0; s2 < 2 * NOB; s2++) {
        bf16x8 wh[CF ? CF : 1], wl[CF ? CF : 1];
#pragma unroll
        for (int cb = 0; cb < CF; cb++) {
          wh[cb] = wb[((s2 * CF + cb) * 2) * 64];
          wl[cb] = wb[((s2 * CF + cb) * 2 + 1) * 64];
        }
#pragma unroll
        for (int cb = 0; cb < CF; cb++) fo[cb] = __builtin_amdgcn_mfma_f32_32x32x16_bf16(wh[cb], bh[s2], fo[cb], 0, 0, 0);
#pragma unroll
        for (int cb = 0; cb < CF; cb++) fo[cb] = __builtin_amdgcn_mfma_f32_32x32x16_bf16(wh[cb], bl[s2], fo[cb], 0, 0, 0);
#pragma unroll
        for (int cb = 0; cb < CF; cb++) fo[cb] = __builtin_amdgcn_mfma_f32_32x32x16_bf16(wl[cb], bh[s2], fo[cb], 0, 0, 0);
      }
      const __amdgpu_buffer_rsrc_t rout =
          __builtin_amdgcn_make_buffer_rsrc(p.out + (size_t)b * (32 * CF) * p.Lq, 0, 32 * CF * p.Lq * 4, 0x00020000);
#pragma unroll
      for (int cb = 0; cb < CF; cb++)
#pragma unroll
        for (int g = 0; g < 4; g++) {
          const f32x4 bv = cvec(s_c + 320, cb, g);
#pragma unroll
          for (int qq = 0; qq < 4; qq++) {
            const int e = 16 * cb + 4 * g + qq;
            const int ch = 16 * (e >> 3) + bf_kpos(0, e & 7);
            const float v = fo[cb][4 * g + qq] + bv[qq];
            __builtin_amdgcn_raw_buffer_store_b32(__builtin_bit_cast(unsigned, v), rout, vo, ch * p.Lq * 4, 0);
          }
        }
    }
    __builtin_amdgcn_wave_barrier();
    PCR_AMARK(7);
    PCR_ANEXT();
  }
#undef PCR_AMARK
#undef PCR_ANEXT
}

template <int NB, bool TRANS = false>
__device__ __forceinline__ void ap128_step(f32x16 (&acc)[NB], const bf16x8 *wb, int ls, const bf16x8 &bh, const bf16x8 &bl) {
  auto mm = [](const bf16x8 &w, const bf16x8 &x, const f32x16 &c) __attribute__((always_inline)) {
    return TRANS ? __builtin_amdgcn_mfma_f32_32x32x16_bf16(x, w, c, 0, 0, 0) : __builtin_amdgcn_mfma_f32_32x32x16_bf16(w, x, c, 0, 0, 0);
  };
#pragma unroll
  for (int c0 = 0; c0 < NB; c0 += 4) {
    bf16x8 wh[4], wl[4];
#pragma unroll
    for (int cb = 0; cb < 4; cb++) {
      wh[cb] = wb[((ls * NB + c0 + cb) * 2) * 64];
      wl[cb] = wb[((ls * NB + c0 + cb) * 2 + 1) * 64];
    }
#pragma unroll
    for (int cb = 0; cb < 4; cb++) acc[c0 + cb] = mm(wh[cb], bh, acc[c0 + cb]);
#pragma unroll
    for (int cb = 0; cb < 4; cb++) acc[c0 + cb] = mm(wh[cb], bl, acc[c0 + cb]);
#pragma unroll
    for (int cb = 0; cb < 4; cb++) acc[c0 + cb] = mm(wl[cb], bh, acc[c0 + cb]);
    asm volatile("" ::: "memory");
  }
}
constexpr int kAp128Waves = 4, kAp128ChunkU = 2048, kAp128Chunks = 16;
constexpr int kAp128Npc = kAp128ChunkU / (64 * kAp128Waves);
__device__ __forceinline__ void ring128_fetch(f32x4 (&stg)[kAp128Npc], __amdgpu_buffer_rsrc_t r, int kk, int tid) {
#pragma unroll
  for (int u = 0; u < kAp128Npc; u++)
    stg[u] = __builtin_bit_cast(f32x4, __builtin_amdgcn_raw_buffer_load_b128(r, tid * 16, (kk * kAp128ChunkU + u * 64 * kAp128Waves) * 16, 0));
  asm volatile("" ::: "memory");
}
__device__ __forceinline__ void ring128_commit(f32x4 *s_ring, const f32x4 (&stg)[kAp128Npc], int k, int tid) {
  f32x4 *dst = s_ring + (k & 1) * kAp128ChunkU + tid;
#pragma unroll
  for (int u = 0; u < kAp128Npc; u++) dst[u * 64 * kAp128Waves] = stg[u];
  __syncthreads();
}
constexpr size_t kAp128Lds = (size_t)2 * kAp128ChunkU * 16 + (640 + 4 * 128 + kAp128Waves * 128) * sizeof(float);
template <int NH>
__global__ __launch_bounds__(64 * kAp128Waves) __attribute__((amdgpu_waves_per_eu(1, 1)))
void attn_apply_stream128_kernel(AttnArgs a) {
  constexpr int D = 128, ND = 4, SD = 8, GPH = 8 / NH;
  extern __shared__ __attribute__((aligned(16))) float smem[];
  const pcr_attn_params &p = a.p;
  f32x4 *s_ring = reinterpret_cast<f32x4 *>(smem);
  int coff = 2 * kAp128ChunkU * 4;
  asm volatile("" : "+s"(coff));
  float *s_c = smem + coff;
  f32x4 *s_p0 = reinterpret_cast<f32x4 *>(s_c + 640);
  float *s_ks = s_c + 640 + 4 * 128;
  const int tid = threadIdx.x, lane = tid & 63, j = lane & 31, h = lane >> 5;
  const int wave = __builtin_amdgcn_readfirstlane(tid >> 6);
  const __amdgpu_buffer_rsrc_t rwq = __builtin_amdgcn_make_buffer_rsrc(const_cast<float *>(p.wq), 0, 4 * kAp128ChunkU * 16, 0x00020000),
                               rw0 = __builtin_amdgcn_make_buffer_rsrc(const_cast<float *>(p.wmlp0), 0, 8 * kAp128ChunkU * 16, 0x00020000),
                               rw2 = __builtin_amdgcn_make_buffer_rsrc(const_cast<float *>(p.wmlp2), 0, 4 * kAp128ChunkU * 16, 0x00020000);
  f32x4 stg[kAp128Npc];
  auto fetch = [&](int k) __attribute__((always_inline)) {
    k %= kAp128Chunks;
    ring128_fetch(stg, k < 4 ? rwq : (k < 12 ? rw0 : rw2), k < 4 ? k : (k < 12 ? k - 4 : k - 12), tid);
  };
  auto commit = [&](int k) __attribute__((always_inline)) { ring128_commit(s_ring, stg, k, tid); };
  for (int e = tid; e < D; e += 64 * kAp128Waves) {
    s_c[e] = p.bq[e];
    s_c[128 + e] = p.ln1_g[e];
    s_c[256 + e] = p.ln1_b[e];
    s_c[384 + e] = p.ln2_g[e];
    s_c[512 + e] = p.ln2_b[e];
    s_p0[e] = f32x4{p.pos0_w[3 * e], p.pos0_w[3 * e + 1], p.pos0_w[3 * e + 2], p.pos0_b[e]};
  }
  fetch(0);
  commit(0);
  const int nblk = p.Lq >> 5;
  const long nitem = (long)p.B * nblk;
  const float skf = (float)p.Sk;
  float *ksw = s_ks + wave * 128;
  auto cvec = [&](const float *base, int cb, int g) __attribute__((always_inline)) {
    return *reinterpret_cast<const f32x4 *>(base + 32 * cb + 8 * g + 4 * h);
  };
  auto to_ops = [&](const f32x16 &acc, int G, bf16x8 &oh, bf16x8 &ol) __attribute__((always_inline)) {
    float v[8];
#pragma unroll
    for (int e = 0; e < 8; e++) v[e] = acc[8 * G + e];
    bf_split8(v, oh, ol, true);
  };
  auto layernorm = [&](f32x16 (&v)[ND], const float *gam, const float *bet) __attribute__((always_inline)) {
    float sm = 0.f;
#pragma unroll
    for (int cb = 0; cb < ND; cb++)
#pragma unroll
      for (int r = 0; r < 16; r++) sm += v[cb][r];
    sm += __shfl_xor(sm, 32, 64);
    const float mean = sm / (float)D;
    float vr = 0.f;
#pragma unroll
    for (int cb = 0; cb < ND; cb++)
#pragma unroll
      for (int r = 0; r < 16; r++) {
        const float dlt = v[cb][r] - mean;
        vr += dlt * dlt;
      }
    vr += __shfl_xor(vr, 32, 64);
    const float inv = 1.0f / sqrtf(vr / (float)D + 1e-5f);
#pragma unroll
    for (int cb = 0; cb < ND; cb++)
#pragma unroll
      for (int g = 0; g < 4; g++) {
        const f32x4 gv = cvec(gam, cb, g), bv = cvec(bet, cb, g);
#pragma unroll
        for (int qq = 0; qq < 4; qq++) v[cb][4 * g + qq] = (v[cb][4 * g + qq] - mean) * inv * gv[qq] + bv[qq];
      }
  };
  for (long it0 = (long)blockIdx.x * kAp128Waves; it0 < nitem; it0 += (long)gridDim.x * kAp128Waves) {
    const long item = it0 + wave;
    const bool live = item < nitem;
    const long it = live ? item : nitem - 1;
    const long b = it / nblk;
    const int blk = (int)(it - b * nblk);
    const size_t bq_ = p.q_index ? (size_t)p.q_index[b] : (size_t)b;
    const size_t kb_ = p.kv_index ? (size_t)p.kv_index[b] : (size_t)b;
    const float *kvp = p.kv + kb_ * ((size_t)D * D + D);
    const int t = blk * 32 + j;
    const __amdgpu_buffer_rsrc_t rfeat = __builtin_amdgcn_make_buffer_rsrc(
        const_cast<float *>(p.feat_q + bq_ * D * p.Lq), 0, D * p.Lq * 4, 0x00020000);
    const int vo = (4 * h * p.Lq + t) * 4;
    auto load_x = [&](float (&xf)[64]) __attribute__((always_inline)) {
#pragma unroll
      for (int e = 0; e < 64; e++) {
        const int ch = 16 * (e >> 3) + bf_kpos(0, e & 7);
        xf[e] = __builtin_bit_cast(float, __builtin_amdgcn_raw_buffer_load_b32(rfeat, vo, ch * p.Lq * 4, 0));
      }
    };
    ksw[lane] = kvp[(size_t)D * D + lane];
    ksw[64 + lane] = kvp[(size_t)D * D + 64 + lane];
    bf16x8 bh[16], bl[16];
    {
      float xf[64];
      load_x(xf);
      const float *xyz = p.xyz_q + (bq_ * p.Lq + t) * 3;
      const float px = xyz[0], py = xyz[1], pz = xyz[2];
#pragma unroll
      for (int s2 = 0; s2 < SD; s2++) {
        float hv[8];
#pragma unroll
        for (int e = 0; e < 8; e++) {
          const f32x4 w = s_p0[16 * s2 + bf_kpos(0, e) + 4 * h];
          const float v = w[0] * px + w[1] * py + w[2] * pz + w[3];
          hv[e] = relu_i(v);
        }
        bf_split8(hv, bh[SD + s2], bl[SD + s2], true);
      }
#pragma unroll
      for (int e = 0; e < 64; e++) asm volatile("" : "+v"(xf[e]));
#pragma unroll
      for (int s2 = 0; s2 < SD; s2++) {
        float xv[8];
#pragma unroll
        for (int e = 0; e < 8; e++) xv[e] = xf[8 * s2 + e];
        bf_split8(xv, bh[s2], bl[s2], true);
      }
    }
    f32x16 q[ND];
#pragma unroll
    for (int cb = 0; cb < ND; cb++)
#pragma unroll
      for (int g = 0; g < 4; g++) {
        const f32x4 bqv = cvec(s_c, cb, g);
#pragma unroll
        for (int qq = 0; qq < 4; qq++) q[cb][4 * g + qq] = bqv[qq];
      }
#pragma unroll
    for (int k = 0; k < 4; k++) {
      fetch(k + 1);
      const bf16x8 *wb = reinterpret_cast<const bf16x8 *>(s_ring + (k & 1) * kAp128ChunkU) + lane;
#pragma unroll
      for (int ls = 0; ls < 4; ls++) ap128_step<ND>(q, wb, ls, bh[4 * k + ls], bl[4 * k + ls]);
      commit(k + 1);
    }
    float zg[SD];
#pragma unroll
    for (int cb = 0; cb < ND; cb++)
#pragma unroll
      for (int g = 0; g < 4; g++) {
        const f32x4 ksv = cvec(ksw, cb, g);
        float zz = 0.f;
#pragma unroll
        for (int qq = 0; qq < 4; qq++) {
          const float v = elu1(q[cb][4 * g + qq]);
          q[cb][4 * g + qq] = v;
          zz += v * ksv[qq];
        }
        if ((g & 1) == 0) zg[2 * cb + (g >> 1)] = zz;
        else zg[2 * cb + (g >> 1)] += zz;
      }
    float zs[NH];
#pragma unroll
    for (int hd = 0; hd < NH; hd++) {
      float z = zg[hd * GPH];
#pragma unroll
      for (int gi = 1; gi < GPH; gi++) z += zg[hd * GPH + gi];
      z += __shfl_xor(z, 32, 64);
      zs[hd] = (1.0f / (z + 1e-6f)) * skf;
    }
#pragma unroll
    for (int cb = 0; cb < ND; cb++)
#pragma unroll
      for (int r = 0; r < 16; r++) q[cb][r] *= zs[(2 * cb + (r >> 3)) / GPH];
    {
      bf16x8 ch_[SD], cl_[SD];
#pragma unroll
      for (int cb = 0; cb < ND; cb++)
#pragma unroll
        for (int G = 0; G < 2; G++) to_ops(q[cb], G, ch_[2 * cb + G], cl_[2 * cb + G]);
#pragma unroll
      for (int cb = 0; cb < ND; cb++)
#pragma unroll
        for (int r = 0; r < 16; r++) q[cb][r] = 0.f;
      const bf16x8 *mb = reinterpret_cast<const bf16x8 *>(kvp) + lane;
      bf16x8 mh[2][ND], ml[2][ND];
#pragma unroll
      for (int cb = 0; cb < ND; cb++) {
        mh[0][cb] = mb[(cb * 2) * 64];
        ml[0][cb] = mb[(cb * 2 + 1) * 64];
      }
#pragma unroll
      for (int s2 = 0; s2 < SD; s2++) {
        const int c = s2 & 1;
        if (s2 + 1 < SD) {
#pragma unroll
          for (int cb = 0; cb < ND; cb++) {
            mh[c ^ 1][cb] = mb[(((s2 + 1) * ND + cb) * 2) * 64];
            ml[c ^ 1][cb] = mb[(((s2 + 1) * ND + cb) * 2 + 1) * 64];
          }
        }
        asm volatile("" ::: "memory");
#pragma unroll
        for (int cb = 0; cb < ND; cb++) q[cb] = __builtin_amdgcn_mfma_f32_32x32x16_bf16(mh[c][cb], ch_[s2], q[cb], 0, 0, 0);
#pragma unroll
        for (int cb = 0; cb < ND; cb++) q[cb] = __builtin_amdgcn_mfma_f32_32x32x16_bf16(mh[c][cb], cl_[s2], q[cb], 0, 0, 0);
#pragma unroll
        for (int cb = 0; cb < ND; cb++) q[cb] = __builtin_amdgcn_mfma_f32_32x32x16_bf16(ml[c][cb], ch_[s2], q[cb], 0, 0, 0);
      }
    }
    layernorm(q, s_c + 128, s_c + 256);
#pragma unroll
    for (int cb = 0; cb < ND; cb++)
#pragma unroll
      for (int G = 0; G < 2; G++) to_ops(q[cb], G, bh[SD + 2 * cb + G], bl[SD + 2 * cb + G]);
    f32x16 f[2 * ND];
#pragma unroll
    for (int cb = 0; cb < 2 * ND; cb++)
#pragma unroll
      for (int r = 0; r < 16; r++) f[cb][r] = 0.f;
#pragma unroll
    for (int k = 4; k < 12; k++) {
      fetch(k + 1);
      const bf16x8 *wb = reinterpret_cast<const bf16x8 *>(s_ring + (k & 1) * kAp128ChunkU) + lane;
#pragma unroll
      for (int ls = 0; ls < 2; ls++) ap128_step<2 * ND>(f, wb, ls, bh[2 * (k - 4) + ls], bl[2 * (k - 4) + ls]);
      commit(k + 1);
    }
    float xf[64];
    load_x(xf);
    f32x16 o[ND];
#pragma unroll
    for (int cb = 0; cb < ND; cb++)
#pragma unroll
      for (int r = 0; r < 16; r++) o[cb][r] = 0.f;
#pragma unroll
    for (int k = 12; k < 16; k++) {
      fetch(k + 1);
      bf16x8 oh[4], ol[4];
#pragma unroll
      for (int i = 0; i < 2; i++) {
        f32x16 &fc = f[2 * (k - 12) + i];
#pragma unroll
        for (int r = 0; r < 16; r++) fc[r] = relu_i(fc[r]);
#pragma unroll
        for (int G = 0; G < 2; G++) to_ops(fc, G, oh[2 * i + G], ol[2 * i + G]);
      }
      const bf16x8 *wb = reinterpret_cast<const bf16x8 *>(s_ring + (k & 1) * kAp128ChunkU) + lane;
#pragma unroll
      for (int ls = 0; ls < 4; ls++) ap128_step<ND>(o, wb, ls, oh[ls], ol[ls]);
      commit(k + 1);
    }
    layernorm(o, s_c + 384, s_c + 512);
#pragma unroll
    for (int cb = 0; cb < ND; cb++)
#pragma unroll
      for (int r = 0; r < 16; r++) o[cb][r] += xf[16 * cb + r];
    if (live) {
      const __amdgpu_buffer_rsrc_t rout =
          __builtin_amdgcn_make_buffer_rsrc(p.out + (size_t)b * D * p.Lq, 0, D * p.Lq * 4, 0x00020000);
#pragma unroll
      for (int e = 0; e < 16 * ND; e++) {
        const int ch = 16 * (e >> 3) + bf_kpos(0, e & 7);
        const float v = o[e >> 4][e & 15];
        __builtin_amdgcn_raw_buffer_store_b32(__builtin_bit_cast(unsigned, v), rout, vo, ch * p.Lq * 4, 0);
      }
    }
  }
}

__host__ __device__ constexpr int attn_kv128_wpc(int nblk) { return nblk >= 32 ? 4 : (nblk >= 16 ? 2 : 1); }
constexpr size_t kKv128Lds0 = (size_t)2 * kAp128ChunkU * 16 + 128 * 16 + 256 * 4;
template <int NH>
__global__ __launch_bounds__(64 * kAp128Waves) __attribute__((amdgpu_waves_per_eu(1, 1)))
void attn_kv_stream128_kernel(AttnArgs a) {
  constexpr int D = 128, SD = 8, TPH = 4 / NH, NKV = NH * TPH * TPH;
  constexpr int KVU = NKV * 16 + 4;
  typedef unsigned u32x4 __attribute__((ext_vector_type(4)));
  extern __shared__ __attribute__((aligned(16))) float smem[];
  const pcr_attn_params &p = a.p;
  f32x4 *s_ring = reinterpret_cast<f32x4 *>(smem);
  int coff = 2 * kAp128ChunkU * 4;
  asm volatile("" : "+s"(coff));
  f32x4 *s_p0 = reinterpret_cast<f32x4 *>(smem + coff);
  float *s_bkv = smem + coff + 4 * D;
  float *s_red = s_bkv + 2 * D;
  const int tid = threadIdx.x, lane = tid & 63, j = lane & 31, h = lane >> 5;
  const int wave = __builtin_amdgcn_readfirstlane(tid >> 6);
  const __amdgpu_buffer_rsrc_t rw = __builtin_amdgcn_make_buffer_rsrc(const_cast<float *>(p.wkv_bf), 0, 8 * kAp128ChunkU * 16, 0x00020000);
  f32x4 stg[kAp128Npc];
  auto fetch = [&](int k) __attribute__((always_inline)) { ring128_fetch(stg, rw, k & 7, tid); };
  auto commit = [&](int k) __attribute__((always_inline)) { ring128_commit(s_ring, stg, k, tid); };
  for (int e = tid; e < D; e += 64 * kAp128Waves) s_p0[e] = f32x4{p.pos0_w[3 * e], p.pos0_w[3 * e + 1], p.pos0_w[3 * e + 2], p.pos0_b[e]};
  for (int e = tid; e < 2 * D; e += 64 * kAp128Waves) s_bkv[e] = p.bkv[e];
  fetch(0);
  commit(0);
  const int Sk = p.Sk, nblk = Sk >> 5;
  const int wpc = a.wpc, cpg = kAp128Waves / wpc;
  const int cslot = wave / wpc, wsub = wave - cslot * wpc;
  const int nper = (nblk + wpc - 1) / wpc;
  const long cstep = (long)gridDim.x * cpg;
  const float inv_sk = 1.0f / (float)Sk;
  float xf[64], pxyz[3];
  auto issue = [&](long bq, int blk) __attribute__((always_inline)) {
    const __amdgpu_buffer_rsrc_t rfeat =
        __builtin_amdgcn_make_buffer_rsrc(const_cast<float *>(p.feat_k + (size_t)bq * D * Sk), 0, D * Sk * 4, 0x00020000);
    const int t = blk * 32 + j, vo = (4 * h * Sk + t) * 4;
#pragma unroll
    for (int e = 0; e < 64; e++) {
      const int ch = 16 * (e >> 3) + bf_kpos(0, e & 7);
      xf[e] = __builtin_bit_cast(float, __builtin_amdgcn_raw_buffer_load_b32(rfeat, vo, ch * Sk * 4, 0));
    }
    const __amdgpu_buffer_rsrc_t rxyz =
        __builtin_amdgcn_make_buffer_rsrc(const_cast<float *>(p.xyz_k + (size_t)bq * Sk * 3), 0, Sk * 12, 0x00020000);
#pragma unroll
    for (int c = 0; c < 3; c++) pxyz[c] = __builtin_bit_cast(float, __builtin_amdgcn_raw_buffer_load_b32(rxyz, t * 12, c * 4, 0));
    asm volatile("" ::: "memory");
  };
  if ((long)blockIdx.x * cpg + cslot < p.B && wsub < nblk) issue((long)blockIdx.x * cpg + cslot, wsub);
  for (long c0 = (long)blockIdx.x * cpg; c0 < p.B; c0 += cstep) {
    const long b = c0 + cslot;
    const bool live = b < p.B;
    f32x16 kv[NKV];
#pragma unroll
    for (int i = 0; i < NKV; i++)
#pragma unroll
      for (int r = 0; r < 16; r++) kv[i][r] = 0.f;
    float ks[4] = {0.f, 0.f, 0.f, 0.f};
    for (int it = 0; it < nper; it++) {
      const int blk = wsub + it * wpc;
      const bool has = live && blk < nblk;
      const bool last = it + 1 == nper;
      const long bn = last ? b + cstep : b;
      const int blkn = last ? wsub : blk + wpc;
      const bool hasn = bn < p.B && blkn < nblk;
      bf16x8 bh[SD], bl[SD];
      if (has) {
#pragma unroll
        for (int s2 = 0; s2 < SD; s2++) {
          float xv[8];
#pragma unroll
          for (int e = 0; e < 8; e++) xv[e] = xf[8 * s2 + e];
          bf_split8(xv, bh[s2], bl[s2], true);
        }
      }
      f32x16 acc[8];
#pragma unroll
      for (int cb = 0; cb < 8; cb++)
#pragma unroll
        for (int r = 0; r < 16; r++) acc[cb][r] = 0.f;
#pragma unroll
      for (int k = 0; k < 8; k++) {
        fetch(k + 1);
        if (has) {
          const bf16x8 *wb = reinterpret_cast<const bf16x8 *>(s_ring + (k & 1) * kAp128ChunkU) + lane;
#pragma unroll
          for (int ls = 0; ls < 2; ls++) {
            if (k < 4) {
              ap128_step<8, true>(acc, wb, ls, bh[2 * k + ls], bl[2 * k + ls]);
            } else {
              const int s2 = 2 * k + ls - SD;
              float hv[8];
#pragma unroll
              for (int e = 0; e < 8; e++) {
                const f32x4 w = s_p0[16 * s2 + bf_kpos(0, e) + 4 * h];
                const float v = w[0] * pxyz[0] + w[1] * pxyz[1] + w[2] * pxyz[2] + w[3];
                hv[e] = relu_i(v);
              }
              bf16x8 hh, hl;
              bf_split8(hv, hh, hl, true);
              ap128_step<8, true>(acc, wb, ls, hh, hl);
            }
          }
        }
        commit(k + 1);
      }
      if (hasn) issue(bn, blkn);
      else {
#pragma unroll
        for (int e = 0; e < 64; e++) xf[e] = 0.f;
        pxyz[0] = pxyz[1] = pxyz[2] = 0.f;
      }
      if (has) {
        float bias[8];
#pragma unroll
        for (int cb = 0; cb < 8; cb++) bias[cb] = s_bkv[cb * 32 + j];
#pragma unroll
        for (int r = 0; r < 16; r++) {
#pragma unroll
          for (int cb = 0; cb < 4; cb++) {
            acc[cb][r] = elu1(acc[cb][r] + bias[cb]);
            ks[cb] += acc[cb][r];
            acc[4 + cb][r] = (acc[4 + cb][r] + bias[4 + cb]) * inv_sk;
          }
        }
#pragma unroll
        for (int i = 0; i < NKV; i++) {
          const int hd = i / (TPH * TPH), ib = hd * TPH + (i % (TPH * TPH)) / TPH, jb = hd * TPH + i % TPH;
#pragma unroll
          for (int r = 0; r < 16; r++) kv[i] = __builtin_amdgcn_mfma_f32_32x32x2f32(acc[4 + jb][r], acc[ib][r], kv[i], 0, 0, 0);
        }
      }
    }
#pragma unroll
    for (int cb = 0; cb < 4; cb++) ks[cb] += __shfl_xor(ks[cb], 32, 64);
    if (wpc > 1) {
      int ln = lane;
      asm volatile("" : "+v"(ln));
      float *red = s_red + (size_t)cslot * KVU * 64 + ln;
      for (int round = 0; round < wpc; round++) {
        if (wsub == round) {
#pragma unroll
          for (int i = 0; i < NKV; i++)
#pragma unroll
            for (int r = 0; r < 16; r++) {
              float *dst = red + (i * 16 + r) * 64;
              *dst = round == 0 ? kv[i][r] : *dst + kv[i][r];
            }
#pragma unroll
          for (int cb = 0; cb < 4; cb++) {
            float *dst = red + (NKV * 16 + cb) * 64;
            *dst = round == 0 ? ks[cb] : *dst + ks[cb];
          }
        }
        __syncthreads();
      }
#pragma unroll
      for (int i = 0; i < NKV; i++)
#pragma unroll
        for (int r = 0; r < 16; r++) kv[i][r] = red[(i * 16 + r) * 64];
#pragma unroll
      for (int cb = 0; cb < 4; cb++) ks[cb] = red[(NKV * 16 + cb) * 64];
    }
    if (live) {
      int ln = lane;
      asm volatile("" : "+v"(ln));
      const int j = ln & 31, h = ln >> 5;
      const __amdgpu_buffer_rsrc_t rkv =
          __builtin_amdgcn_make_buffer_rsrc(p.kv + (size_t)b * ((size_t)D * D + D), 0, (D * D + D) * 4, 0x00020000);
      const __amdgpu_buffer_rsrc_t rwm = __builtin_amdgcn_make_buffer_rsrc(const_cast<float *>(p.wmerge), 0, D * D * 4, 0x00020000);
      for (int ob = wsub; ob < 4; ob += wpc) {
        const int wrow = ((ob * 32 + j) * D + 4 * h) * 4;
#pragma unroll
        for (int hd = 0; hd < NH; hd++) {
          f32x4 w[TPH][4];
#pragma unroll
          for (int jj = 0; jj < TPH; jj++)
#pragma unroll
            for (int g = 0; g < 4; g++)
              w[jj][g] = __builtin_bit_cast(f32x4, __builtin_amdgcn_raw_buffer_load_b128(rwm, wrow, ((hd * TPH + jj) * 32 + 8 * g) * 4, 0));
#pragma unroll
          for (int dl = 0; dl < TPH; dl++) {
            const int db = hd * TPH + dl;
            f32x16 m;
#pragma unroll
            for (int r = 0; r < 16; r++) m[r] = 0.f;
#pragma unroll
            for (int jj = 0; jj < TPH; jj++) {
              const int i = hd * TPH * TPH + dl * TPH + jj;
#pragma unroll
              for (int r = 0; r < 16; r++) m = __builtin_amdgcn_mfma_f32_32x32x2f32(kv[i][r], w[jj][r >> 2][r & 3], m, 0, 0, 0);
            }
#pragma unroll
            for (int G = 0; G < 2; G++) {
              float v[8];
#pragma unroll
              for (int e = 0; e < 8; e++) v[e] = m[8 * G + e];
              bf16x8 hi, lo;
              bf_split8(v, hi, lo, true);
              const int unit = (((db * 2 + G) * (D >> 5) + ob) * 2) * 64 + h * 32 + j;
              __builtin_amdgcn_raw_buffer_store_b128(__builtin_bit_cast(u32x4, hi), rkv, unit * 16, 0, 0);
              __builtin_amdgcn_raw_buffer_store_b128(__builtin_bit_cast(u32x4, lo), rkv, (unit + 64) * 16, 0, 0);
            }
          }
        }
      }
      if (wsub == 0 && h == 0) {
#pragma unroll
        for (int cb = 0; cb < 4; cb++)
          __builtin_amdgcn_raw_buffer_store_b32(__builtin_bit_cast(unsigned, ks[cb]), rkv, (D * D + cb * 32 + j) * 4, 0, 0);
      }
    }
  }
}
#endif

}

static int attn_check(const pcr_attn_params &p) {
  if (p.B < 0 || p.Lq < 1 || p.Sk < 1 || p.c1 < 1 || p.c2 < 1 || p.cout < 1 || p.nhead < 1) return 1;
  if (p.d < 32 || p.d > 512 || (p.d & 31) || p.d % p.nhead) return 1;
  if (p.d > 128 && ((p.d & 63) || ((p.d / p.nhead) & 63) || p.d / p.nhead > 256)) return 1;
  if ((p.c2 & 7) || p.cout > 512 || p.cfinal > 512) return 1;
  if (!p.feat_q || !p.feat_k || !p.xyz_k || !p.kv || !p.pos0_w || !p.pos0_b || !p.wq || !p.bq || !p.wkv ||
      !p.bkv || !p.wmerge || !p.wmlp0 || !p.wmlp2 || !p.ln1_g || !p.ln1_b || !p.ln2_g || !p.ln2_b)
    return 1;
  if (p.q_pos && (!p.xyz_q || p.c1 != p.c2 || p.c1 != p.d)) return 1;
  if (p.residual && p.cout != p.c1) return 1;
  if (p.cfinal && (!p.wfinal || !p.bfinal || (p.cout & 7))) return 1;
  return 0;
}

static void attn_dump_trace(const char *path, const char *tag, int wgs, int B, int Sk) {
  static int launches = 0;
  static const int skip = pcr_tune_int("PCR_SA_TRACE_SKIP");
  launches++;
  if (launches <= skip || launches > skip + 8) return;
  static std::vector<unsigned long long> host(2 * kATraceWgs * kATraceRecs * kATraceMarks);
  if (hipDeviceSynchronize() != hipSuccess) return;
  if (hipMemcpyFromSymbol(host.data(), HIP_SYMBOL(g_attn_trace), host.size() * sizeof(unsigned long long)) != hipSuccess) return;
  FILE *f = fopen(path, "a");
  if (!f) return;
  const int n = 2 * (wgs < kATraceWgs ? wgs : kATraceWgs);
  fprintf(f, "launch %d kernel %s wgs %d B %d Sk %d\n", launches, tag, wgs, B, Sk);
  for (int w = 0; w < n; w++) {
    const unsigned long long *t = host.data() + (size_t)w * (kATraceRecs * kATraceMarks);
    fprintf(f, "wg %d", w);
    for (int i = 0; i < kATraceRecs * kATraceMarks; i++) fprintf(f, " %llu", t[i]);
    fprintf(f, "\n");
  }
  fclose(f);
}

static int attn_kv_narrow(const pcr_attn_params *pp, pcr_stream_t stream) {
  AttnArgs a;
  a.p = *pp;
  a.dbg = 0;
  a.wpc = 0;
  const int d = pp->d;
  if (pp->c2 < pp->d) return PCR_ERR_INVALID;
  const int tb = d <= 64 ? 2 : 1, RP = 32 * tb + 1;
  size_t lds = (size_t)(pp->c2 + d + 3) * RP + 4 * d;
  const size_t lds2 = (size_t)d * (d + 1) + d;
  if (lds2 > lds) lds = lds2;
  lds = (lds + kThreads) * sizeof(float);
  if (lds > (size_t)kMaxDynLds) return PCR_ERR_INVALID;
  const int ntile = (pp->Sk + 32 * tb - 1) / (32 * tb);
  int ns = pp->kv_splits > 1 ? pp->kv_splits : 1;
  if (ns > 1 && (!pp->kv_part || ns > 64)) return PCR_ERR_INVALID;
  if (ns > ntile) ns = ntile;
  a.p.kv_splits = ns;
  dim3 g(pp->B, ns), blk(kThreads);
  hipStream_t st = pcr_s(stream);
  constexpr bool kBfUnit = kAPrec != 0;
  const bool bfk = kBfUnit && pp->wkv_bf != nullptr;
  if (ns == 1 && d == 64 && (pp->c2 == 64 || (pp->c2 == 128 && bfk && pp->Sk >= 128)) && (pp->Sk & 31) == 0 && pp->nhead >= 1 &&
      64 % pp->nhead == 0) {
    const bool bf = bfk;
    const bool wide = pp->c2 == 128;
    pcr_note_arith(bf ? PCR_PREC_BF16X3 : PCR_PREC_F32);
    const int nblk = pp->Sk >> 5;
    const int minw = wide ? 4 : 2;
    int wpc2 = 1;
    while (wpc2 * 2 <= (nblk < 4 ? nblk : 4)) wpc2 *= 2;
    if (wpc2 < minw) wpc2 = minw;
    static const int no_onew = pcr_tune_int("PCR_ATTN_NO_ONEW");
    const bool onew = kBfUnit && bf && !wide && nblk <= 4 && !no_onew;
    if (onew) wpc2 = 1;
    const int cpg = kKvsWaves / wpc2;
    const size_t wu = bf ? (size_t)((wide ? 8 : 4) + 4) * 512 : 4096;
    const size_t lds_s = (wu * 4 + 256 + 128 + 64 * 65 + (onew ? (size_t)0 : (size_t)cpg * (64 * 65 + 64))) * sizeof(float);
    const long rounds = ((long)pp->B + cpg - 1) / cpg;
    const int gs = (int)(rounds < pcr_cu_count() ? rounds : pcr_cu_count());
    const dim3 gg(gs), bb(64 * kKvsWaves);
    const bool mh = pp->nhead >= 2;
    if (bf && wide) {
      constexpr int W = kBfUnit ? 8 : 4;
      return mh ? pcr_launch_lds<attn_kv_stream64_kernel<true, kBfUnit, W>>(gg, bb, lds_s, st, a)
                : pcr_launch_lds<attn_kv_stream64_kernel<false, kBfUnit, W>>(gg, bb, lds_s, st, a);
    }
    if (!bf)
      return mh ? pcr_launch_lds<attn_kv_stream64_kernel<true, false>>(gg, bb, lds_s, st, a)
                : pcr_launch_lds<attn_kv_stream64_kernel<false, false>>(gg, bb, lds_s, st, a);
    static const char *atrace = pcr_tune_str("PCR_ATTN_TRACE");
    if (atrace) a.dbg |= 256;
    int rc;
    if (onew)
      rc = mh ? pcr_launch_lds<attn_kv_stream64_kernel<true, kBfUnit, 4, kBfUnit>>(gg, bb, lds_s, st, a)
              : pcr_launch_lds<attn_kv_stream64_kernel<false, kBfUnit, 4, kBfUnit>>(gg, bb, lds_s, st, a);
    else
      rc = mh ? pcr_launch_lds<attn_kv_stream64_kernel<true, kBfUnit>>(gg, bb, lds_s, st, a)
              : pcr_launch_lds<attn_kv_stream64_kernel<false, kBfUnit>>(gg, bb, lds_s, st, a);
    if (atrace) attn_dump_trace(atrace, "kv64", gs, (int)pp->B, pp->Sk);
    return rc;
  }
#if PCR_ATTN_PREC != 0
  if (ns == 1 && d == 32 && pp->c2 == 32 && pp->wkv_bf && (pp->Sk & 31) == 0 && pp->nhead >= 1 && 32 % pp->nhead == 0) {
    pcr_note_arith(PCR_PREC_BF16X3);
    const int nblk = pp->Sk >> 5;
    int wpc2 = 1;
    while (wpc2 * 2 <= (nblk < kKvsWaves ? nblk : kKvsWaves)) wpc2 *= 2;
    if (wpc2 < 2) wpc2 = 2;
    const int cpg = kKvsWaves / wpc2;
    const size_t lds_s = (size_t)(4096 + 128 + 64 + 32 * 33 + cpg * (32 * 33 + 32)) * sizeof(float);
    const long rounds = ((long)pp->B + cpg - 1) / cpg;
    const long cap = 2L * pcr_cu_count();
    return pcr_launch_lds<attn_kv_stream32_kernel>(dim3((unsigned)(rounds < cap ? rounds : cap)), dim3(64 * kKvsWaves), lds_s, st, a);
  }
  static const int no_kv128 = pcr_tune_int("PCR_ATTN_NO_KV128");
  if (ns == 1 && d == 128 && pp->c2 == 128 && pp->wkv_bf && (pp->Sk & 31) == 0 && pp->Sk >= 256 &&
      (pp->nhead == 2 || pp->nhead == 4) && !no_kv128) {
    pcr_note_arith(PCR_PREC_BF16X3);
    a.wpc = attn_kv128_wpc(pp->Sk >> 5);
    static const int wpc_t = pcr_tune_int("PCR_ATTN_KV128_WPC");
    if (wpc_t == 1 || wpc_t == 2 || wpc_t == 4) a.wpc = wpc_t;
    const int cpg = kAp128Waves / a.wpc;
    const size_t lds_s = kKv128Lds0 + (a.wpc > 1 ? (size_t)cpg * (16 * (16 / pp->nhead) + 4) * 64 * sizeof(float) : 0);
    const long nwg = ((long)pp->B + cpg - 1) / cpg;
    const dim3 gg((unsigned)(nwg < pcr_cu_count() ? nwg : pcr_cu_count())), bb(64 * kAp128Waves);
    return pp->nhead == 2 ? pcr_launch_lds<attn_kv_stream128_kernel<2>>(gg, bb, lds_s, st, a)
                          : pcr_launch_lds<attn_kv_stream128_kernel<4>>(gg, bb, lds_s, st, a);
  }
#endif
  pcr_note_arith(PCR_PREC_F32);
  int rc;
  if (d == 32) rc = pcr_launch_lds<attn_kv_kernel<2, 1, 2, 1>>(g, blk, lds, st, a);
  else if (d == 64) rc = pcr_launch_lds<attn_kv_kernel_o3<2, 1, 1, 1>>(g, blk, lds, st, a);
  else if (d == 128) {
    if (kBfUnit && pp->wkv_bf && pp->Sk >= 256) rc = pcr_launch_lds<attn_kv_kernel_o2<1, 2, 1, 4, true>>(g, blk, lds, st, a);
    else rc = pcr_launch_lds<attn_kv_kernel_o2<1, 2, 1, 4>>(g, blk, lds, st, a);
  }
  else rc = pcr_launch_lds<attn_kv_kernel<1, 2, 0, 4>>(g, blk, lds, st, a);
  if (rc != PCR_OK || ns == 1) return rc;
  return pcr_launch_lds<attn_kv_fold_kernel>(dim3(pp->B), blk, ((size_t)d * (d + 1) + d) * sizeof(float), st, a);
}

static bool aps64_shape(const pcr_attn_params &p) {
  const bool aps_in = p.c1 == 64 || ((p.c1 == 32 || (p.c1 < 16 && p.wmlp0_bf_xpad)) && !p.q_pos && !p.residual);
  const bool aps_out = (p.cout == 64 && (p.cfinal == 0 || p.cfinal == 128) && p.c1 >= 32) ||
                       (p.cout == 128 && !p.cfinal && !p.residual && p.c1 == 64) ||
                       (p.cout == 32 && p.cfinal == 64 && !p.residual && p.c1 < 16);
  return p.d == 64 && aps_in && aps_out && (p.Lq & 31) == 0 && (p.nhead == 1 || p.nhead == 2 || p.nhead == 4);
}

static int attn_apply_launch(const pcr_attn_params *pp, pcr_stream_t stream) {
  const pcr_attn_params &p = *pp;
  AttnArgs a;
  a.p = p;
  a.dbg = 0;
  a.wpc = 0;
  const int tb = p.d <= 32 ? 4 : (p.d <= 64 ? 2 : 1), T = 32 * tb, RP = T + 1;
  const int catP = ceil8(p.c1 + p.d);
  int rowsU = catP > 2 * p.d ? catP : 2 * p.d;
  if (ceil32(p.cout) > rowsU) rowsU = ceil32(p.cout);
  if (ceil32(p.cfinal) > rowsU) rowsU = ceil32(p.cfinal);
  size_t lds = ((size_t)(rowsU + 3 + p.nhead) * RP + 2 * (kThreads / T) * T + 7 * p.d + 2 * p.cout) *
               sizeof(float);
  if (lds > (size_t)kMaxDynLds) return PCR_ERR_INVALID;
  dim3 g((p.Lq + T - 1) / T, p.B), blk(kThreads);
  hipStream_t st = pcr_s(stream);
  pcr_note_arith(kAPrec != 0 ? PCR_PREC_BF16X3 : PCR_PREC_F32);
#if PCR_ATTN_PREC != 0
  const int aps_c1s = (p.c1 + 15) >> 4, aps_nd = p.d >> 5;
  const size_t aps_lds = (size_t)((aps_c1s + (p.q_pos ? 2 * aps_nd : 0)) * aps_nd * 128 + (aps_c1s + 2 * aps_nd) * aps_nd * 256 +
                                  aps_nd * (p.cout >> 5) * 512) * 16 +
                         (size_t)(448 + 256 + 64 * kApsWaves) * sizeof(float);
  static const int no_s128 = pcr_tune_int("PCR_ATTN_NO_STREAM128");
  if (p.d == 128 && p.c1 == 128 && p.cout == 128 && !p.cfinal && p.q_pos && p.residual && (p.Lq & 31) == 0 && p.Lq >= 256 &&
      (p.nhead == 1 || p.nhead == 2 || p.nhead == 4) && !no_s128) {
    const long nitem = (long)p.B * (p.Lq >> 5);
    const long nwg = (nitem + kAp128Waves - 1) / kAp128Waves;
    const dim3 gg((unsigned)(nwg < pcr_cu_count() ? nwg : pcr_cu_count())), bb(64 * kAp128Waves);
    if (p.nhead == 1) return pcr_launch_lds<attn_apply_stream128_kernel<1>>(gg, bb, kAp128Lds, st, a);
    if (p.nhead == 2) return pcr_launch_lds<attn_apply_stream128_kernel<2>>(gg, bb, kAp128Lds, st, a);
    return pcr_launch_lds<attn_apply_stream128_kernel<4>>(gg, bb, kAp128Lds, st, a);
  }
  if (p.d == 32 && p.c1 == 32 && p.cout == 32 && !p.cfinal && (p.Lq & 31) == 0 && (p.nhead == 1 || p.nhead == 2)) {
    const long nitem = (long)p.B * (p.Lq >> 5);
    const long nwg = (nitem + kApsWaves - 1) / kApsWaves;
    const dim3 gg((unsigned)(nwg < pcr_cu_count() ? nwg : pcr_cu_count())), bb(64 * kApsWaves);
    return p.q_pos ? pcr_launch_lds<attn_apply_stream64_kernel<true, 2, 0, 1, 1>>(gg, bb, aps_lds, st, a)
                   : pcr_launch_lds<attn_apply_stream64_kernel<false, 2, 0, 1, 1>>(gg, bb, aps_lds, st, a);
  }
  if (aps64_shape(p) && aps_lds <= (size_t)kMaxDynLds) {
    const int nob = p.cout >> 5;
    const long nitem = (long)p.B * (p.Lq >> 5);
    const long nwg = (nitem + kApsWaves - 1) / kApsWaves;
    const dim3 gg((unsigned)(nwg < pcr_cu_count() ? nwg : pcr_cu_count())), bb(64 * kApsWaves);
    const bool cf = p.cfinal != 0;
    static const char *aptrace = pcr_tune_str("PCR_ATTN_TRACE");
    if (aptrace) a.dbg = 256;
    if (pp->pool_out) {
      const long nwgp = ((long)p.B + kApsWaves - 1) / kApsWaves;
      const dim3 ggp((unsigned)(nwgp < pcr_cu_count() ? nwgp : pcr_cu_count()));
      return pcr_launch_lds<attn_apply_stream64_kernel<false, 4, 0, 2, 2, true>>(ggp, bb, aps_lds, st, a);
    }
    int rc;
    if (nob == 4)
      rc = p.q_pos ? pcr_launch_lds<attn_apply_stream64_kernel<true, 4, 0, 4>>(gg, bb, aps_lds, st, a)
                   : pcr_launch_lds<attn_apply_stream64_kernel<false, 4, 0, 4>>(gg, bb, aps_lds, st, a);
    else if (p.c1 < 16) rc = pcr_launch_lds<attn_apply_stream64_kernel<false, 1, 2, 1>>(gg, bb, aps_lds, st, a);
    else if (p.c1 == 32)
      rc = cf ? pcr_launch_lds<attn_apply_stream64_kernel<false, 2, 4>>(gg, bb, aps_lds, st, a)
              : pcr_launch_lds<attn_apply_stream64_kernel<false, 2, 0>>(gg, bb, aps_lds, st, a);
    else if (p.q_pos)
      rc = cf ? pcr_launch_lds<attn_apply_stream64_kernel<true, 4, 4>>(gg, bb, aps_lds, st, a)
              : pcr_launch_lds<attn_apply_stream64_kernel<true, 4, 0>>(gg, bb, aps_lds, st, a);
    else
      rc = cf ? pcr_launch_lds<attn_apply_stream64_kernel<false, 4, 4>>(gg, bb, aps_lds, st, a)
              : pcr_launch_lds<attn_apply_stream64_kernel<false, 4, 0>>(gg, bb, aps_lds, st, a);
    if (aptrace) attn_dump_trace(aptrace, "apply64", (int)gg.x, (int)p.B, p.Lq);
    return rc;
  }
#endif
  const bool wide = 2 * p.d > 128 || p.cout > 128 || p.cfinal > 128;
  if (tb == 4)
    return wide ? pcr_launch_lds<attn_apply_kernel<4, 2>>(g, blk, lds, st, a) : pcr_launch_lds<attn_apply_kernel<4, 1>>(g, blk, lds, st, a);
  if (tb == 2)
    return wide ? pcr_launch_lds<attn_apply_kernel<2, 2>>(g, blk, lds, st, a) : pcr_launch_lds<attn_apply_kernel<2, 1>>(g, blk, lds, st, a);
  int widest = 2 * p.d > p.cout ? 2 * p.d : p.cout;
  if (p.cfinal > widest) widest = p.cfinal;
#if PCR_ATTN_PREC == 0
  if (widest > 512) return pcr_launch_lds<attn_apply_kernel<1, 8>>(g, blk, lds, st, a);
  if (widest > 256) return pcr_launch_lds<attn_apply_kernel<1, 4>>(g, blk, lds, st, a);
#else
  if (widest > 256) return PCR_ERR_INVALID;
#endif
  return pcr_launch_lds<attn_apply_kernel<1, 2>>(g, blk, lds, st, a);
}

#if PCR_ATTN_PREC == 1
int pcr_attn_kv_bf3(const pcr_attn_params *pp, pcr_stream_t stream) { return attn_kv_narrow(pp, stream); }
int pcr_attn_apply_bf3(const pcr_attn_params *pp, pcr_stream_t stream) { return attn_apply_launch(pp, stream); }
#else
int pcr_attn_kv_bf3(const pcr_attn_params *pp, pcr_stream_t stream);
int pcr_attn_apply_bf3(const pcr_attn_params *pp, pcr_stream_t stream);

static bool attn_bf(const pcr_attn_params &p, pcr_attn_params &q) {
  const int widest = 2 * p.d > p.cout ? (2 * p.d > p.cfinal ? 2 * p.d : p.cfinal) : (p.cout > p.cfinal ? p.cout : p.cfinal);
  if (p.precision == 0 || p.d > 128 || widest > 256 || !p.wq_bf || !p.wmlp0_bf || !p.wmlp2_bf ||
      (p.cfinal && !p.wfinal_bf))
    return false;
  q = p;
  q.wq = p.wq_bf; q.wmlp0 = p.wmlp0_bf; q.wmlp2 = p.wmlp2_bf; q.wfinal = p.wfinal_bf;
  return true;
}

PCR_EXPORT int pcr_attn_kv_splits(int B, int Sk, int d) {
  (void)B;
  if (Sk < 1 || d > 64) return 1;
  if ((d == 64 || d == 32) && (Sk & 31) == 0) return 1;
  const int ntile = (Sk + 63) / 64;
  return ntile >= 16 ? 4 : (ntile >= 8 ? 2 : 1);
}

PCR_EXPORT int pcr_attn_kv_f32(const pcr_attn_params *pp, pcr_stream_t stream) {
  if (!pp || attn_check(*pp)) return PCR_ERR_INVALID;
  if (pp->B == 0) return PCR_OK;
  const int d = pp->d;
  if (d > 128) {
    AttnArgs a;
    a.p = *pp;
    a.dbg = 0;
    a.wpc = 0;
    if (!pp->wkv_wide || !pp->bkv_wide || !pp->wmerge_packed || pp->B > 65535) return PCR_ERR_INVALID;
    pcr_note_arith(PCR_PREC_F32);
    const int dh = d / pp->nhead;
    size_t lds = ((size_t)(pp->c2 + d + 3) * 33 + 4 * d + kThreads) * sizeof(float);
    const size_t lds2 = (size_t)dh * 65 * sizeof(float);
    if (lds2 > lds) lds = lds2;
    if (lds > (size_t)kMaxDynLds) return PCR_ERR_INVALID;
    dim3 g(d / 64, pp->B), blk(kThreads);
    if (64 + dh <= 256) return pcr_launch_lds<attn_kv_wide_kernel<2>>(g, blk, lds, pcr_s(stream), a);
    return pcr_launch_lds<attn_kv_wide_kernel<3>>(g, blk, lds, pcr_s(stream), a);
  }
  pcr_attn_params q;
  if (attn_bf(*pp, q)) return pcr_attn_kv_bf3(&q, stream);
  return attn_kv_narrow(pp, stream);
}

static bool attn_pool_ok(const pcr_attn_params &p) {
  pcr_attn_params q;
  return aps64_shape(p) && p.c1 == 64 && p.cout == 64 && !p.cfinal && !p.q_pos && attn_bf(p, q);
}

PCR_EXPORT int pcr_attn_apply_pool_ok(const pcr_attn_params *pp) {
  return (pp && !attn_check(*pp) && attn_pool_ok(*pp)) ? 1 : 0;
}

PCR_EXPORT int pcr_attn_apply_f32(const pcr_attn_params *pp, pcr_stream_t stream) {
  if (!pp || attn_check(*pp) || (!pp->out && !pp->pool_out)) return PCR_ERR_INVALID;
  if (pp->pool_out && !attn_pool_ok(*pp)) return PCR_ERR_INVALID;
  if (pp->B == 0) return PCR_OK;
  if (pp->B > 65535) return PCR_ERR_INVALID;
  pcr_attn_params q;
  if (attn_bf(*pp, q)) return pcr_attn_apply_bf3(&q, stream);
  return attn_apply_launch(pp, stream);
}
#endif
```

### point-cloud-reid_amd/pcr_amd/engine.py

```python
import ctypes
import os

import numpy as np
import torch

from . import _lib as L

c_float_p = ctypes.c_void_p
c_int_p = ctypes.c_void_p

import os as _os
PRECISIONS = {"f32": 0, "bf16x3": 1, "bf16": 2}
PRECISION = _os.environ.get("PCR_PRECISION", "bf16x3")
if PRECISION not in PRECISIONS:
    raise L.PcrError("PCR_PRECISION must be one of %s" % sorted(PRECISIONS))


KV_SPLITS = int(os.environ["PCR_KV_SPLITS"]) if os.environ.get("PCR_KV_SPLITS") else None


def set_precision(name):
    global PRECISION
    if name not in PRECISIONS:
        raise L.PcrError("precision must be one of %s" % sorted(PRECISIONS))
    prev, PRECISION = PRECISION, name
    return prev


class precision:

    def __init__(self, name):
        self.name = name

    def __enter__(self):
        self.prev = set_precision(self.name)

    def __exit__(self, *exc):
        set_precision(self.prev)
        return False


GUARD = _os.environ.get("PCR_GUARD", "1") != "0"
GUARD_BOUND = float(_os.environ.get("PCR_GUARD_BOUND", "5e-5"))
GUARD_ACCEPT = float(_os.environ.get("PCR_GUARD_ACCEPT", "0.9"))
GUARD_EVERY = int(_os.environ.get("PCR_GUARD_EVERY", "64"))
GUARD_SENTINEL_PAIRS = int(_os.environ.get("PCR_GUARD_SENTINEL_PAIRS", "8"))
_LEVEL = 0


class guard_level:

    def __init__(self, level):
        self.level = int(level)

    def __enter__(self):
        global _LEVEL
        self.prev_level, _LEVEL = _LEVEL, self.level
        self.prev_prec = set_precision("f32") if (self.level >= 2 and PRECISION == "bf16x3") else None

    def __exit__(self, *exc):
        global _LEVEL
        _LEVEL = self.prev_level
        if self.prev_prec is not None:
            set_precision(self.prev_prec)
        return False


def guarded(fn):
    if _LEVEL >= 1 and PRECISION == "bf16x3":
        with precision("f32"):
            return fn()
    return fn()


SA_CLAIMS = _os.environ.get("PCR_SA_CLAIMS", "1") != "0"

SA_XYZ_TABLES = _os.environ.get("PCR_SA_XYZ_TABLES", "1") != "0"

PROFILE = None
ARITH_NAMES = {0: "f32", 1: "bf16x3", 2: "bf16"}


class _prof:
    def __init__(self, name, flops=0.0, nbytes=0.0, exec_flops=None, arith=None):
        self.name, self.flops, self.nbytes, self.arith = name, flops, nbytes, arith
        self.exec_flops = flops if exec_flops is None else exec_flops

    def __enter__(self):
        if PROFILE is not None:
            self.e0 = torch.cuda.Event(enable_timing=True)
            self.e1 = torch.cuda.Event(enable_timing=True)
            self.e0.record()
        return self

    def __exit__(self, *exc):
        if PROFILE is not None:
            self.e1.record()
            arith = self.arith
            if arith == "lib":
                arith = ARITH_NAMES.get(L.load().pcr_last_launch_arith(), "f32")
            PROFILE.append((self.name, self.e0, self.e1, self.flops, self.nbytes, self.exec_flops, arith))
        return False


class SaParams(ctypes.Structure):
    _fields_ = [("mode", ctypes.c_int), ("B", ctypes.c_int), ("N", ctypes.c_int), ("S", ctypes.c_int),
                ("K", ctypes.c_int), ("D", ctypes.c_int),
                ("c1", ctypes.c_int), ("c2", ctypes.c_int), ("c3", ctypes.c_int),
                ("xyz", c_float_p), ("feat", c_float_p), ("idx", c_int_p), ("centre_idx", c_int_p),
                ("wp", c_float_p * 3), ("scale", c_float_p * 3), ("shift", c_float_p * 3),
                ("wa", c_float_p), ("wpq", c_float_p), ("wps", c_float_p * 2), ("shift_pad", c_float_p * 2),
                ("cnt", c_int_p), ("tile_ws", c_int_p),
                ("pq_ws", c_float_p), ("pq_ready", ctypes.c_int),
                ("feat_point_major", ctypes.c_int), ("out_point_major", ctypes.c_int),
                ("out", c_float_p), ("wa_packed", c_float_p),
                ("precision", ctypes.c_int), ("wps_bf", c_float_p * 2), ("wa_shift_packed", c_float_p),
                ("row_tab", c_float_p), ("claim_ws", c_int_p), ("pq_has_xyz", ctypes.c_int)]


class AttnParams(ctypes.Structure):
    _fields_ = [("B", ctypes.c_int), ("Lq", ctypes.c_int), ("Sk", ctypes.c_int),
                ("c1", ctypes.c_int), ("c2", ctypes.c_int), ("d", ctypes.c_int), ("cout", ctypes.c_int),
                ("nhead", ctypes.c_int), ("q_pos", ctypes.c_int), ("residual", ctypes.c_int),
                ("feat_q", c_float_p), ("xyz_q", c_float_p), ("feat_k", c_float_p), ("xyz_k", c_float_p),
                ("kv_index", c_int_p), ("q_index", c_int_p),
                ("pos0_w", c_float_p), ("pos0_b", c_float_p),
                ("wq", c_float_p), ("bq", c_float_p), ("wkv", c_float_p), ("bkv", c_float_p),
                ("wmerge", c_float_p), ("wmlp0", c_float_p), ("wmlp2", c_float_p),
                ("ln1_g", c_float_p), ("ln1_b", c_float_p), ("ln2_g", c_float_p), ("ln2_b", c_float_p),
                ("wfinal", c_float_p), ("bfinal", c_float_p), ("cfinal", ctypes.c_int),
                ("wkv_wide", c_float_p), ("bkv_wide", c_float_p), ("wmerge_packed", c_float_p),
                ("kv", c_float_p), ("out", c_float_p),
                ("precision", ctypes.c_int),
                ("wq_bf", c_float_p), ("wmlp0_bf", c_float_p), ("wmlp2_bf", c_float_p), ("wfinal_bf", c_float_p),
                ("kv_splits", ctypes.c_int), ("kv_part", c_float_p), ("wkv_bf", c_float_p),
                ("wmlp0_bf_xpad", c_float_p), ("pool_out", c_float_p)]


class HeadParams(ctypes.Structure):
    _fields_ = [("P", ctypes.c_int), ("C", ctypes.c_int), ("L", ctypes.c_int), ("groups", ctypes.c_int),
                ("o", c_float_p), ("w1", c_float_p), ("w2", c_float_p),
                ("gn1_g", c_float_p), ("gn1_b", c_float_p), ("gn2_g", c_float_p), ("gn2_b", c_float_p),
                ("w_out", c_float_p), ("b_out", c_float_p),
                ("pooled", c_float_p), ("logits", c_float_p), ("w1t", c_float_p), ("w2t", c_float_p)]


def _p(t):
    return t.data_ptr() if t is not None else None


def _dev32(t, device):
    return t.detach().to(device=device, dtype=torch.float32).contiguous()


def pack_weight(w, device):
    w2 = w.detach().reshape(w.shape[0], -1).to("cpu", torch.float32).contiguous().numpy()
    cout, cin = w2.shape
    lib = L.load()
    n = lib.pcr_packed_weight_floats(cout, cin)
    out = np.empty(n, np.float32)
    L.check(lib.pcr_pack_weight_f32(w2.ctypes.data_as(ctypes.c_void_p), cout, cin,
                                    out.ctypes.data_as(ctypes.c_void_p)), "pcr_pack_weight_f32")
    return torch.from_numpy(out).to(device)


def pack_weight_bf(w, device):
    w2 = w.detach().reshape(w.shape[0], -1).to("cpu", torch.float32).contiguous().numpy()
    cout, cin = w2.shape
    lib = L.load()
    n = lib.pcr_packed_weight_bf16_floats(cout, cin)
    out = np.empty(n, np.float32)
    L.check(lib.pcr_pack_weight_bf16x2_f32(w2.ctypes.data_as(ctypes.c_void_p), cout, cin,
                                           out.ctypes.data_as(ctypes.c_void_p)), "pcr_pack_weight_bf16x2_f32")
    return torch.from_numpy(out).to(device)


def pack_weight_dual(w, device):
    wp = pack_weight(w, device)
    cout, cin = w.shape[0], int(np.prod(w.shape[1:]))
    if L.load().pcr_dense_prec_ok(cin, cout, 1) or L.load().pcr_dense_xpm_prec_ok(cin, cout, 1):
        wp._pcr_bf = pack_weight_bf(w, device)
    return wp


def fold_bn(bn, conv_bias, device):
    scale = bn.weight.detach().double() / torch.sqrt(bn.running_var.detach().double() + bn.eps)
    bias = conv_bias.detach().double() if conv_bias is not None else 0.0
    shift = (bias - bn.running_mean.detach().double()) * scale + bn.bias.detach().double()
    return _dev32(scale.float(), device), _dev32(shift.float(), device)


def param_version(module):
    return tuple((t.data_ptr(), t._version) for t in list(module.parameters()) + list(module.buffers()))


def knn_prefix(xyz, S, K):
    L.require_cuda(xyz)
    assert xyz.is_contiguous() and xyz.dtype == torch.float32
    B, N, _ = xyz.shape
    idx = torch.empty((B, S, K), dtype=torch.int32, device=xyz.device)
    with _prof("knn_prefix[N=%d,S=%d,K=%d]" % (N, S, K), 8.0 * B * S * N, 12.0 * B * N + 4.0 * B * S * K):
        L.check(L.load().pcr_knn_prefix_f32(L.ptr(xyz), L.ptr(idx), B, N, S, K, L.stream_ptr()),
                "pcr_knn_prefix_f32")
    return idx


def knn_prefix2(xyz, S, K, S2, K2):
    L.require_cuda(xyz)
    assert xyz.is_contiguous() and xyz.dtype == torch.float32 and S2 <= S and K2 >= K
    B, N, _ = xyz.shape
    if S2 == 0 or B == 0:
        return knn_prefix(xyz, S, K), torch.empty((B, S2, K2), dtype=torch.int32, device=xyz.device)
    idx = torch.empty((B, S, K), dtype=torch.int32, device=xyz.device)
    idx2 = torch.empty((B, S2, K2), dtype=torch.int32, device=xyz.device)
    with _prof("knn_prefix2[N=%d,S=%d,K=%d,S2=%d,K2=%d]" % (N, S, K, S2, K2), 8.0 * B * S * N,
               12.0 * B * N + 4.0 * B * (S * K + S2 * K2)):
        L.check(L.load().pcr_knn_prefix2_f32(L.ptr(xyz), L.ptr(idx), L.ptr(idx2), B, N, S, K, S2, K2, L.stream_ptr()),
                "pcr_knn_prefix2_f32")
    return idx, idx2


class SaPlan:

    def __init__(self, convs, bns, device, mode, fast=True):
        assert len(convs) == 3 and len(bns) == 3, "the fused SA kernel covers 3-layer MLPs"
        self.mode = mode
        self.cin = convs[0].weight.shape[1]
        self.couts = [c.weight.shape[0] for c in convs]
        self.wp = [pack_weight(c.weight, device) for c in convs]
        folded = [fold_bn(b, c.bias, device) for c, b in zip(convs, bns)]
        self.scale = [f[0] for f in folded]
        self.shift = [f[1] for f in folded]
        w1 = convs[0].weight.detach().reshape(self.couts[0], -1).double().cpu()
        D = (self.cin - 3) // 2 if mode == 0 else self.cin - 3
        self.D = D
        sc1 = self.scale[0].detach().double().cpu().unsqueeze(1)
        self.wa = _dev32((w1[:, :3] * sc1).float(), device)
        self.wa_packed = pack_weight((w1[:, :3] * sc1).float(), device)
        self.wa_shift_packed = pack_weight(torch.cat([w1[:, :3] * sc1, self.shift[0].detach().double().cpu().unsqueeze(1)],
                                                     dim=1).float(), device)
        self.wpq = None
        self.fast = fast
        self.wps, self.shift_pad, self.wps_bf = [], [], []
        for l in (1, 2):
            w = convs[l].weight.detach().reshape(self.couts[l], -1).double().cpu()
            sc = self.scale[l].detach().double().cpu().unsqueeze(1)
            self.wps.append(pack_weight((w * sc).float(), device))
            self.wps_bf.append(pack_weight_bf((w * sc).float(), device))
            pad = torch.zeros((self.couts[l] + 31) // 32 * 32, dtype=torch.float32, device=device)
            pad[:self.couts[l]] = self.shift[l]
            self.shift_pad.append(pad)
        if D > 0:
            if mode == 0:
                wc, wf = w1[:, 3:3 + D], w1[:, 3 + D:3 + 2 * D]
                stacked = torch.cat([wf * sc1, (wc - wf) * sc1], dim=0)
            else:
                stacked = w1[:, 3:3 + D] * sc1
            self.wpq = pack_weight(stacked.float(), device)
            self.wpq_bf = pack_weight_bf(stacked.float(), device)
            if mode == 0:
                wa64 = w1[:, :3] * sc1
                sh64 = self.shift[0].detach().double().cpu().unsqueeze(1)
                self.wxyz = _dev32(torch.cat([torch.cat([wa64, torch.zeros_like(sh64)], dim=1),
                                              torch.cat([-wa64, sh64], dim=1)], dim=0).float().contiguous(), device)

    def wants_row_table(self, N, K, min_radius, B=1, S=1):
        lib = L.load()
        if os.environ.get("PCR_SA_NO_STREAM") or int(B) * int(S) >= 2 ** 31:
            return False
        return bool(self.fast and self.mode == 1 and lib.pcr_ball_query_rows_ok(N, K, ctypes.c_float(min_radius or 0.0)) and
                    lib.pcr_sa_uses_row_table(self.couts[0], self.couts[1], self.couts[2], K, PRECISIONS[PRECISION]))

    def run(self, xyz, feat, idx, centre_idx=None, cnt=None, out_point_major=False, rows=None, K=None):
        B, N, _ = xyz.shape
        if rows is not None:
            S = cnt.shape[1]
            assert cnt is not None and self.wants_row_table(N, K, 0.0, B, S), "row table given to a layer that does not read it"
            L.require_cuda(xyz, cnt, rows)
            assert rows.is_contiguous() and rows.numel() == L.load().pcr_ball_query_rows_floats(B, S, K)
        else:
            L.require_cuda(xyz, idx)
            _, S, K = idx.shape
        D = 0 if feat is None else feat.shape[1]
        want = 3 + (2 * D if self.mode == 0 else D)
        assert want == self.cin, "feature width %d does not match the first conv (%d)" % (want, self.cin)
        feat, feat_pm = as_cm_or_pm(feat)
        assert xyz.is_contiguous() and (idx is None or idx.is_contiguous())
        out = torch.empty((B, S, self.couts[2]) if out_point_major else (B, self.couts[2], S),
                          dtype=torch.float32, device=xyz.device)
        p = SaParams()
        p.mode, p.B, p.N, p.S, p.K, p.D = self.mode, B, N, S, K, D
        p.c1, p.c2, p.c3 = self.couts
        p.xyz, p.feat, p.idx, p.centre_idx = _p(xyz), _p(feat), _p(idx), _p(centre_idx)
        for i in range(3):
            p.wp[i], p.scale[i], p.shift[i] = _p(self.wp[i]), _p(self.scale[i]), _p(self.shift[i])
        p.out = _p(out)
        p.feat_point_major, p.out_point_major = int(feat_pm), int(bool(out_point_major))
        ragged = cnt is not None and self.fast and self.mode == 1
        if cnt is not None:
            assert cnt.is_contiguous() and cnt.dtype == torch.int32 and cnt.shape == (B, S)
        tiled = ragged or (self.fast and self.mode == 1 and L.load().pcr_sa_krow_uses_tiles(
            self.couts[0], self.couts[1], self.couts[2], K, PRECISIONS[PRECISION]))
        if tiled:
            n_ws = L.load().pcr_sa_tile_ws_ints(B, S, K, self.couts[1], self.couts[2])
            if n_ws > 0:
                tile_ws = torch.empty((n_ws,), dtype=torch.int32, device=xyz.device)
                p.tile_ws = _p(tile_ws)
            if ragged:
                p.cnt = _p(cnt)
                p.row_tab = _p(rows)
        if self.fast:
            p.wa = _p(self.wa)
            p.wa_packed = _p(self.wa_packed)
            p.wa_shift_packed = _p(self.wa_shift_packed)
            p.precision = PRECISIONS[PRECISION]
            n_claim = 0 if (ragged or not SA_CLAIMS) else L.load().pcr_sa_claim_ws_ints(
                self.couts[0], self.couts[1], self.couts[2], K, N, PRECISIONS[PRECISION])
            if n_claim > 0:
                claim_ws = torch.empty((n_claim,), dtype=torch.int32, device=xyz.device)
                p.claim_ws = _p(claim_ws)
            for i in range(2):
                p.wps[i], p.shift_pad[i] = _p(self.wps[i]), _p(self.shift_pad[i])
                p.wps_bf[i] = _p(self.wps_bf[i])
            if D:
                c1_, c2_, c3_ = self.couts
                pqw = (2 if self.mode == 0 else 1) * self.couts[0]
                ws = torch.empty((B, N, pqw), dtype=torch.float32, device=xyz.device)
                p.wpq, p.pq_ws = _p(self.wpq), _p(ws)
                with _prof("sa_tables[D=%d,out=%d,N=%d]" % (D, pqw, N), 2.0 * B * N * D * pqw,
                           4.0 * B * N * (D + pqw), arith="lib"):
                    if PRECISION == "f32":
                        L.check(L.load().pcr_dense_pm_f32(L.ptr(feat), L.ptr(self.wpq), L.ptr(ws), B, D, pqw, N,
                                                          int(feat_pm), L.stream_ptr()), "pcr_dense_pm_f32")
                    elif (SA_XYZ_TABLES and not ragged and not tiled and idx is not None and
                          L.load().pcr_sa_tables_take_xyz(self.mode, D, c1_, c2_, c3_, K, PRECISIONS[PRECISION])):
                        q_rows = min(N, (S + 63) // 64 * 64) if centre_idx is None else N
                        q_rows = q_rows if q_rows % 64 == 0 else N
                        L.check(L.load().pcr_dense_pm_xyz_f32(L.ptr(feat), L.ptr(self.wpq_bf), L.ptr(xyz), L.ptr(self.wxyz),
                                                              L.ptr(ws), B, D, pqw, N, int(feat_pm), PRECISIONS[PRECISION],
                                                              q_rows, c1_ if q_rows < N else pqw,
                                                              L.stream_ptr()), "pcr_dense_pm_xyz_f32")
                        p.pq_has_xyz = 1
                    else:
                        L.check(L.load().pcr_dense_pm_prec_f32(L.ptr(feat), L.ptr(self.wpq_bf), L.ptr(ws), B, D, pqw, N,
                                                               int(feat_pm), PRECISIONS[PRECISION], L.stream_ptr()),
                                "pcr_dense_pm_prec_f32")
                p.pq_ready = 1
        c1, c2, c3 = self.couts
        flops = 2.0 * B * S * K * (self.cin * c1 + c1 * c2 + c2 * c3)
        nbytes = 4.0 * B * (3 * N + D * N + S * K + c3 * S)
        exec_flops = 2.0 * B * S * K * (c1 * c2 + c2 * c3) if self.fast else flops
        if ragged:
            rows = float(((cnt.clamp(1, K) + 1) // 2 * 2).sum().item()) if PROFILE is not None else 0.0
            exec_flops = 2.0 * rows * (c1 * c2 + c2 * c3)
        name = "sa_ragged" if ragged else "sa_fused"
        with _prof("%s[D=%d,c=%d/%d/%d,N=%d,S=%d,K=%d]" % (name, D, c1, c2, c3, N, S, K), flops, nbytes, exec_flops,
                   arith="lib"):
            L.check(L.load().pcr_sa_mlp_f32(ctypes.byref(p), L.stream_ptr()), "pcr_sa_mlp_f32")
        return out.transpose(1, 2) if out_point_major else out


class AttnPlan:

    def __init__(self, m, pos_name, device, nhead, q_pos, k_pos, residual, final=None):
        pos = getattr(m, pos_name)
        L.require_default_eps(m.norm1, m.norm2)
        self.device = device
        self.nhead, self.q_pos, self.k_pos, self.residual = nhead, int(q_pos), int(k_pos), int(residual)
        self.d = d = m.q_proj.weight.shape[0]
        self.c1 = m.q_proj.weight.shape[1]
        self.c2 = m.k_proj.weight.shape[1]
        self.cout = m.mlp[2].weight.shape[0]
        f64 = lambda x: x.detach().double().cpu()
        W2, b2 = f64(pos[2].weight), f64(pos[2].bias)
        Wq, Wk, Wv = f64(m.q_proj.weight), f64(m.k_proj.weight), f64(m.v_proj.weight)
        if q_pos:
            wq = torch.cat([Wq, Wq @ W2], dim=1)
            bq = Wq @ b2
        else:
            wq, bq = Wq, torch.zeros(d, dtype=torch.float64)
        kz = (Wk @ W2) if k_pos else torch.zeros(d, d, dtype=torch.float64)
        wkv = torch.cat([torch.cat([Wk, kz], dim=1), torch.cat([Wv, Wv @ W2], dim=1)], dim=0)
        bkv = torch.cat([(Wk @ b2) if k_pos else torch.zeros(d, dtype=torch.float64), Wv @ b2])
        self.t = dict(
            pos0_w=_dev32(pos[0].weight, device), pos0_b=_dev32(pos[0].bias, device),
            wq=pack_weight(wq.float(), device), bq=_dev32(bq.float(), device),
            wkv=pack_weight(wkv.float(), device), bkv=_dev32(bkv.float(), device),
            wmerge=_dev32(m.merge.weight, device),
            wmlp0=pack_weight(m.mlp[0].weight, device), wmlp2=pack_weight(m.mlp[2].weight, device),
            ln1_g=_dev32(m.norm1.weight, device), ln1_b=_dev32(m.norm1.bias, device),
            ln2_g=_dev32(m.norm2.weight, device), ln2_b=_dev32(m.norm2.bias, device))
        if d <= 128:
            if d % 32 == 0 and (d // nhead) % 32 == 0:
                self.t["wmerge_packed"] = pack_weight(m.merge.weight, device)
            if (d == 64 and self.c2 in (64, 128)) or (d == 32 and self.c2 == 32) or d == 128:
                self.t["wkv_bf"] = pack_weight_bf(wkv.float(), device)
            if d == 64 and self.c1 % 16:
                w0 = m.mlp[0].weight.detach().float().cpu()
                pad = torch.zeros(w0.shape[0], 16 * ((self.c1 + 15) // 16) - self.c1)
                self.t["wmlp0_bf_xpad"] = pack_weight_bf(torch.cat([w0[:, :self.c1], pad, w0[:, self.c1:]], dim=1), device)
            self.t.update(wq_bf=pack_weight_bf(wq.float(), device),
                          wmlp0_bf=pack_weight_bf(m.mlp[0].weight, device), wmlp2_bf=pack_weight_bf(m.mlp[2].weight, device))
        if d > 128:
            dh = d // nhead
            if d % 64 or dh % 64 or dh > 256:
                raise L.PcrError("attention with d_model %d, %d heads is not covered (heads of 64..256 channels)" % (d, nhead))
            imgs, biases = [], []
            for g in range(d // 64):
                hd = (64 * g) // dh
                rows = torch.cat([torch.arange(64 * g, 64 * g + 64), torch.arange(d + hd * dh, d + (hd + 1) * dh)])
                imgs.append(pack_weight(wkv[rows].float(), device))
                biases.append(bkv[rows].float())
            self.t["wkv_wide"] = torch.cat(imgs).contiguous()
            self.t["bkv_wide"] = _dev32(torch.cat(biases), device)
            self.t["wmerge_packed"] = pack_weight(m.merge.weight, device)
        self.cfinal = 0
        if final is not None:
            self.t["wfinal"] = pack_weight(final.weight, device)
            if d <= 128:
                self.t["wfinal_bf"] = pack_weight_bf(final.weight, device)
            self.cfinal = final.weight.shape[0]
            bpad = torch.zeros((self.cfinal + 31) // 32 * 32, dtype=torch.float32, device=device)
            bpad[:self.cfinal] = final.bias.detach().to(device).float()
            self.t["bfinal"] = bpad

    def _params(self, B, Lq, Sk, feat_q, xyz_q, feat_k, xyz_k, kv, out, kv_index=None, q_index=None):
        p = AttnParams()
        p.B, p.Lq, p.Sk = B, Lq, Sk
        p.c1, p.c2, p.d, p.cout, p.nhead = self.c1, self.c2, self.d, self.cout, self.nhead
        p.q_pos, p.residual = self.q_pos, self.residual
        p.feat_q, p.xyz_q, p.feat_k, p.xyz_k = _p(feat_q), _p(xyz_q), _p(feat_k), _p(xyz_k)
        p.kv_index, p.q_index = _p(kv_index), _p(q_index)
        for k, v in self.t.items():
            setattr(p, k, _p(v))
        p.cfinal = self.cfinal
        p.kv, p.out = _p(kv), _p(out)
        p.precision = PRECISIONS[PRECISION]
        return p

    def kv(self, feat_k, xyz_k):
        L.require_cuda(feat_k, xyz_k)
        assert feat_k.is_contiguous() and xyz_k.is_contiguous() and feat_k.dtype == torch.float32
        B, c2, Sk = feat_k.shape
        assert c2 == self.c2
        lib = L.load()
        kv = torch.empty((B, lib.pcr_attn_kv_floats(self.d)), dtype=torch.float32, device=feat_k.device)
        p = self._params(B, 1, Sk, feat_k, xyz_k, feat_k, xyz_k, kv, kv)
        d = self.d
        ns = lib.pcr_attn_kv_splits(B, Sk, d) if KV_SPLITS is None else KV_SPLITS
        if ns > 1:
            part = torch.empty((B, ns, lib.pcr_attn_kv_floats(d)), dtype=torch.float32, device=feat_k.device)
            p.kv_splits, p.kv_part = ns, _p(part)
        kv_flops = 2.0 * B * Sk * (3 * d + d * c2 + 2 * c2 * d + d * d / self.nhead)
        with _prof("attn_kv[d=%d,c2=%d,Sk=%d]" % (d, c2, Sk), kv_flops, 4.0 * B * (c2 * Sk + 3 * Sk + d * d + d),
                   arith="lib"):
            L.check(lib.pcr_attn_kv_f32(ctypes.byref(p), L.stream_ptr()), "pcr_attn_kv_f32")
        kv._pcr_precision = PRECISION
        return kv

    def pool_ok(self, Lq, Sk):
        dummy = torch.empty(0)
        p = self._params(1, Lq, Sk, dummy, None, dummy, None, dummy, dummy)
        p.feat_q = p.feat_k = p.xyz_k = p.kv = p.out = 1
        return bool(L.load().pcr_attn_apply_pool_ok(ctypes.byref(p)))

    def apply(self, feat_q, xyz_q, kv, Sk, kv_index=None, q_index=None, n_out=None, pooled=False):
        L.require_cuda(feat_q, kv)
        assert feat_q.is_contiguous() and feat_q.dtype == torch.float32 and (xyz_q is None or xyz_q.is_contiguous())
        Bq, c1, Lq = feat_q.shape
        assert c1 == self.c1
        made = getattr(kv, "_pcr_precision", PRECISION)
        if (made == "f32") != (PRECISION == "f32") and self.d <= 128:
            raise L.PcrError("attention state was built in %r mode and is applied in %r mode: the per-cloud matrix is "
                             "stored in the arithmetic's own layout" % (made, PRECISION))
        B = n_out if n_out is not None else Bq
        if pooled:
            out = torch.empty((B, 2, self.cout), dtype=torch.float32, device=feat_q.device)
            p = self._params(B, Lq, Sk, feat_q, xyz_q, feat_q, xyz_q if xyz_q is not None else feat_q, kv, None,
                             kv_index, q_index)
            p.pool_out = _p(out)
        else:
            out = torch.empty((B, self.cfinal or self.cout, Lq), dtype=torch.float32, device=feat_q.device)
            p = self._params(B, Lq, Sk, feat_q, xyz_q, feat_q, xyz_q if xyz_q is not None else feat_q, kv, out,
                             kv_index, q_index)
        d = self.d
        ap_flops = 2.0 * B * Lq * (c1 * d + d * d / self.nhead + d * d + (c1 + d) * 2 * d + 2 * d * self.cout
                                   + self.cout * self.cfinal + (self.q_pos * (3 * d + d * c1)))
        with _prof("attn_apply[d=%d,c1=%d,out=%d,Lq=%d%s]" % (d, c1, self.cfinal or self.cout, Lq, ",pooled" if pooled else ""),
                   ap_flops, 4.0 * B * (c1 * Lq + d * d + d + (2 if pooled else Lq) * (self.cfinal or self.cout)), arith="lib"):
            L.check(L.load().pcr_attn_apply_f32(ctypes.byref(p), L.stream_ptr()), "pcr_attn_apply_f32")
        return out

    def run(self, feat_q, xyz_q, feat_k, xyz_k, kv_index=None):
        assert feat_k.shape[0] == feat_q.shape[0]
        kv = self.kv(feat_k, xyz_k)
        return self.apply(feat_q, xyz_q, kv, feat_k.shape[2], kv_index=kv_index)


class HeadPlan:

    def __init__(self, linres, out_linear, device):
        if getattr(linres, "transform", None) is not None:
            raise L.PcrError("pcr_pool_head_f32 covers LinearRes with n_in == n_out only")
        L.require_default_eps(linres.norm1, linres.norm2)
        self.n = linres.linear1.weight.shape[0]
        self.groups = linres.norm1.num_groups
        self.t = dict(w1=_dev32(linres.linear1.weight, device), w2=_dev32(linres.linear2.weight, device),
                      gn1_g=_dev32(linres.norm1.weight, device), gn1_b=_dev32(linres.norm1.bias, device),
                      gn2_g=_dev32(linres.norm2.weight, device), gn2_b=_dev32(linres.norm2.bias, device),
                      w_out=_dev32(out_linear.weight, device), b_out=_dev32(out_linear.bias, device),
                      w1t=_dev32(linres.linear1.weight.detach().t().contiguous(), device),
                      w2t=_dev32(linres.linear2.weight.detach().t().contiguous(), device))

    def run(self, o, want_pooled=False):
        L.require_cuda(o)
        assert o.is_contiguous() and o.dtype == torch.float32
        twoP, C, Lp = o.shape
        P = twoP // 2
        assert 2 * C == self.n, "pooled width %d != match head width %d" % (2 * C, self.n)
        logits = torch.empty((P,), dtype=torch.float32, device=o.device)
        pooled = torch.empty((P, 2 * C), dtype=torch.float32, device=o.device) if want_pooled else None
        p = HeadParams()
        p.P, p.C, p.L, p.groups = P, C, Lp, self.groups
        p.o = _p(o)
        for k, v in self.t.items():
            setattr(p, k, _p(v))
        p.pooled, p.logits = _p(pooled), _p(logits)
        with _prof("pool_head", 4.0 * P * (2 * C) ** 2, 4.0 * twoP * C * Lp):
            L.check(L.load().pcr_pool_head_f32(ctypes.byref(p), L.stream_ptr()), "pcr_pool_head_f32")
        return (logits, pooled) if want_pooled else logits


def as_cm_or_pm(x):
    if x is None or x.is_contiguous():
        return x, False
    if x.dim() == 3 and x.transpose(1, 2).is_contiguous():
        return x, True
    return x.contiguous(), False


def dense(x, wp, cout, scale=None, shift=None, act=0):
    L.require_cuda(x)
    assert x.dtype == torch.float32
    x, x_pm = as_cm_or_pm(x)
    B, cin, Ln = x.shape
    y = torch.empty((B, cout, Ln), dtype=torch.float32, device=x.device)
    lib = L.load()
    bf = getattr(wp, "_pcr_bf", None)
    if PRECISION != "f32" and bf is not None and not x_pm and lib.pcr_dense_prec_ok(cin, cout, Ln):
        with _prof("dense[cin=%d,cout=%d,L=%d]" % (cin, cout, Ln), 2.0 * B * Ln * cin * cout, 4.0 * B * Ln * (cin + cout),
                   arith=PRECISION):
            L.check(lib.pcr_dense_prec_f32(L.ptr(x), L.ptr(bf), L.ptr(scale), L.ptr(shift), L.ptr(y), B, cin, cout, Ln, act,
                                           PRECISIONS[PRECISION], L.stream_ptr()), "pcr_dense_prec_f32")
        return y
    if PRECISION != "f32" and bf is not None and x_pm and lib.pcr_dense_xpm_prec_ok(cin, cout, Ln):
        with _prof("dense[cin=%d,cout=%d,L=%d]" % (cin, cout, Ln), 2.0 * B * Ln * cin * cout, 4.0 * B * Ln * (cin + cout),
                   arith="lib"):
            L.check(lib.pcr_dense_xpm_prec_f32(L.ptr(x), L.ptr(bf), L.ptr(scale), L.ptr(shift), L.ptr(y), B, cin, cout, Ln,
                                               act, PRECISIONS[PRECISION], L.stream_ptr()), "pcr_dense_xpm_prec_f32")
        return y
    fn = lib.pcr_dense_xpm_f32 if x_pm else lib.pcr_dense_f32
    with _prof("dense[cin=%d,cout=%d,L=%d]" % (cin, cout, Ln), 2.0 * B * Ln * cin * cout, 4.0 * B * Ln * (cin + cout),
               arith="f32"):
        L.check(fn(L.ptr(x), L.ptr(wp), L.ptr(scale), L.ptr(shift), L.ptr(y), B, cin, cout, Ln, act, L.stream_ptr()),
                "pcr_dense_f32")
    return y
```

Baseline: 68120.

## Fold LayerNorm mean-centering and affine into attention weights

Pre-multiplies the merge and second MLP weights by a centering matrix so the LayerNorm mean subtraction is done by the weights themselves. The first LayerNorm's gain is folded into the first MLP weight and its bias into a seed that initialises the FFN accumulators. The kernels get a FOLD template variant whose layernorm only computes the RMS scale, which cuts reductions and per-element work per tile. This adds host-side weight images and a flag that tags the KV state as centred, and it may shift bf16x3 rounding slightly.

Result: faster. 69040, median of 6 (+1.3%).

```diff
diff --git a/include/pcr.h b/include/pcr.h
--- a/include/pcr.h
+++ b/include/pcr.h
@@ -163,12 +163,15 @@
   const float *wkv_bf;
   const float *wmlp0_bf_xpad;
   float *pool_out;
+  const float *ffn0_seed;
+  int ln_folded;
 } pcr_attn_params;
 long pcr_attn_kv_floats(int d);
 int pcr_attn_kv_splits(int B, int Sk, int d);
 int pcr_attn_kv_f32(const pcr_attn_params *p, pcr_stream_t stream);
 int pcr_attn_apply_f32(const pcr_attn_params *p, pcr_stream_t stream);
 int pcr_attn_apply_pool_ok(const pcr_attn_params *p);
+int pcr_attn_fold_ok(const pcr_attn_params *p, int kv);
 
 typedef struct pcr_head_params {
   int P, C, L, groups;
diff --git a/point-cloud-reid_amd/csrc/attn_kernels_impl.h b/point-cloud-reid_amd/csrc/attn_kernels_impl.h
--- a/point-cloud-reid_amd/csrc/attn_kernels_impl.h
+++ b/point-cloud-reid_amd/csrc/attn_kernels_impl.h
@@ -960,9 +960,9 @@
   }
 }
 
+constexpr int kApsWaves = 8;
 #if PCR_ATTN_PREC != 0
-constexpr int kApsWaves = 8;
-template <bool QPOS, int C1S, int CF, int NOB = 2, int ND = 2, bool POOL = false>
+template <bool QPOS, int C1S, int CF, int NOB = 2, int ND = 2, bool POOL = false, bool FOLD = false>
 __global__ __launch_bounds__(64 * kApsWaves) __attribute__((amdgpu_waves_per_eu(2, 2)))
 void attn_apply_stream64_kernel(AttnArgs a) {
   static_assert(!QPOS || C1S == 2 * ND, "q_pos needs c1 == d");
@@ -990,9 +990,13 @@
     for (int e = tid; e < ND * NOB * 512; e += 64 * kApsWaves) d2[e] = w2[e];
     if (tid < D) {
       s_c[tid] = p.bq[tid];
-      s_c[64 + tid] = p.ln1_g[tid];
-      s_c[128 + tid] = p.ln1_b[tid];
-
+      if constexpr (FOLD) {
+        s_c[64 + tid] = p.ffn0_seed[tid];
+        s_c[64 + D + tid] = p.ffn0_seed[D + tid];
+      } else {
+        s_c[64 + tid] = p.ln1_g[tid];
+        s_c[128 + tid] = p.ln1_b[tid];
+      }
       if (QPOS) s_p0[tid] = f32x4{p.pos0_w[3 * tid], p.pos0_w[3 * tid + 1], p.pos0_w[3 * tid + 2], p.pos0_b[tid]};
     }
     if (tid < 32 * NOB) {
@@ -1079,10 +1083,21 @@
     }
     PCR_AMARK(1);
     f32x16 q[ND];
-#pragma unroll
-    for (int cb = 0; cb < ND; cb++)
-#pragma unroll
-      for (int r = 0; r < 16; r++) q[cb][r] = 0.f;
+    if constexpr (FOLD && QPOS) {
+#pragma unroll
+      for (int cb = 0; cb < ND; cb++)
+#pragma unroll
+        for (int g = 0; g < 4; g++) {
+          const f32x4 sv = cvec(s_c, cb, g);
+#pragma unroll
+          for (int qq = 0; qq < 4; qq++) q[cb][4 * g + qq] = sv[qq];
+        }
+    } else {
+#pragma unroll
+      for (int cb = 0; cb < ND; cb++)
+#pragma unroll
+        for (int r = 0; r < 16; r++) q[cb][r] = 0.f;
+    }
     {
       const bf16x8 *wb = s_wq + lane;
 #pragma unroll
@@ -1121,11 +1136,11 @@
     for (int cb = 0; cb < ND; cb++)
 #pragma unroll
       for (int g = 0; g < 4; g++) {
-        const f32x4 bqv = cvec(s_c, cb, g), ksv = cvec(ksw, cb, g);
+        const f32x4 bqv = FOLD ? f32x4{0.f, 0.f, 0.f, 0.f} : cvec(s_c, cb, g), ksv = cvec(ksw, cb, g);
         float zz = 0.f;
 #pragma unroll
         for (int qq = 0; qq < 4; qq++) {
-          const float v = elu1(q[cb][4 * g + qq] + bqv[qq]);
+          const float v = elu1(FOLD ? q[cb][4 * g + qq] : q[cb][4 * g + qq] + bqv[qq]);
           q[cb][4 * g + qq] = v;
           zz += v * ksv[qq];
         }
@@ -1174,8 +1189,38 @@
 #pragma unroll
       for (int cb = 0; cb < ND; cb++) m[cb] = __builtin_amdgcn_mfma_f32_32x32x16_bf16(ml[s2][cb], ch_[s2], m[cb], 0, 0, 0);
     }
-    auto layernorm = [&](auto &v, auto nb_tag, const float *gam, const float *bet) __attribute__((always_inline)) {
+    auto layernorm = [&](auto &v, auto nb_tag, auto mode_tag, const float *gam, const float *bet) __attribute__((always_inline)) {
       constexpr int NB = decltype(nb_tag)::value;
+      constexpr int MODE = decltype(mode_tag)::value;
+      if constexpr (MODE != 0) {
+        float v0 = 0.f, v1 = 0.f;
+#pragma unroll
+        for (int cb = 0; cb < NB; cb++)
+#pragma unroll
+          for (int r = 0; r < 16; r += 2) {
+            v0 += v[cb][r] * v[cb][r];
+            v1 += v[cb][r + 1] * v[cb][r + 1];
+          }
+        float vr = v0 + v1;
+        vr += __shfl_xor(vr, 32, 64);
+        const float inv = 1.0f / sqrtf(vr / (32.0f * NB) + 1e-5f);
+        if constexpr (MODE == 1) {
+#pragma unroll
+          for (int cb = 0; cb < NB; cb++)
+#pragma unroll
+            for (int r = 0; r < 16; r++) v[cb][r] *= inv;
+        } else {
+#pragma unroll
+          for (int cb = 0; cb < NB; cb++)
+#pragma unroll
+            for (int g = 0; g < 4; g++) {
+              const f32x4 gv = cvec(gam, cb, g), bv = cvec(bet, cb, g);
+#pragma unroll
+              for (int qq = 0; qq < 4; qq++) v[cb][4 * g + qq] = v[cb][4 * g + qq] * (inv * gv[qq]) + bv[qq];
+            }
+        }
+        return;
+      }
       float sm = 0.f;
 #pragma unroll
       for (int cb = 0; cb < NB; cb++)
@@ -1203,7 +1248,7 @@
         }
     };
     PCR_AMARK(3);
-    layernorm(m, std::integral_constant<int, ND>{}, s_c + 64, s_c + 128);
+    layernorm(m, std::integral_constant<int, ND>{}, std::integral_constant<int, FOLD ? 1 : 0>{}, s_c + 64, s_c + 128);
     PCR_AMARK(4);
 #pragma unroll
     for (int s2 = 0; s2 < C1S; s2++) {
@@ -1217,10 +1262,21 @@
 #pragma unroll
       for (int G = 0; G < 2; G++) to_ops(m[cb], G, bh[C1S + 2 * cb + G], bl[C1S + 2 * cb + G]);
     f32x16 f[SD];
-#pragma unroll
-    for (int cb = 0; cb < SD; cb++)
-#pragma unroll
-      for (int r = 0; r < 16; r++) f[cb][r] = 0.f;
+    if constexpr (FOLD) {
+#pragma unroll
+      for (int cb = 0; cb < SD; cb++)
+#pragma unroll
+        for (int g = 0; g < 4; g++) {
+          const f32x4 sv = cvec(s_c + 64, cb, g);
+#pragma unroll
+          for (int qq = 0; qq < 4; qq++) f[cb][4 * g + qq] = sv[qq];
+        }
+    } else {
+#pragma unroll
+      for (int cb = 0; cb < SD; cb++)
+#pragma unroll
+        for (int r = 0; r < 16; r++) f[cb][r] = 0.f;
+    }
     {
       const bf16x8 *wb = s_w0 + lane;
 #pragma unroll
@@ -1271,7 +1327,8 @@
       }
     }
     PCR_AMARK(6);
-    layernorm(o, std::integral_constant<int, NOB>{}, s_c + 192, s_c + 192 + 32 * NOB);
+    layernorm(o, std::integral_constant<int, NOB>{}, std::integral_constant<int, FOLD ? (CF ? 1 : 2) : 0>{}, s_c + 192,
+              s_c + 192 + 32 * NOB);
     if constexpr (C1S == 2 * NOB) {
       if (p.residual) {
 #pragma unroll
@@ -1417,7 +1474,7 @@
   __syncthreads();
 }
 constexpr size_t kAp128Lds = (size_t)2 * kAp128ChunkU * 16 + (640 + 4 * 128 + kAp128Waves * 128) * sizeof(float);
-template <int NH>
+template <int NH, bool FOLD = false>
 __global__ __launch_bounds__(64 * kAp128Waves) __attribute__((amdgpu_waves_per_eu(1, 1)))
 void attn_apply_stream128_kernel(AttnArgs a) {
   constexpr int D = 128, ND = 4, SD = 8, GPH = 8 / NH;
@@ -1442,8 +1499,8 @@
   auto commit = [&](int k) __attribute__((always_inline)) { ring128_commit(s_ring, stg, k, tid); };
   for (int e = tid; e < D; e += 64 * kAp128Waves) {
     s_c[e] = p.bq[e];
-    s_c[128 + e] = p.ln1_g[e];
-    s_c[256 + e] = p.ln1_b[e];
+    s_c[128 + e] = FOLD ? p.ffn0_seed[e] : p.ln1_g[e];
+    s_c[256 + e] = FOLD ? p.ffn0_seed[128 + e] : p.ln1_b[e];
     s_c[384 + e] = p.ln2_g[e];
     s_c[512 + e] = p.ln2_b[e];
     s_p0[e] = f32x4{p.pos0_w[3 * e], p.pos0_w[3 * e + 1], p.pos0_w[3 * e + 2], p.pos0_b[e]};
@@ -1463,7 +1520,37 @@
     for (int e = 0; e < 8; e++) v[e] = acc[8 * G + e];
     bf_split8(v, oh, ol, true);
   };
-  auto layernorm = [&](f32x16 (&v)[ND], const float *gam, const float *bet) __attribute__((always_inline)) {
+  auto layernorm = [&](f32x16 (&v)[ND], auto mode_tag, const float *gam, const float *bet) __attribute__((always_inline)) {
+    constexpr int MODE = decltype(mode_tag)::value;
+    if constexpr (MODE != 0) {
+      float v0 = 0.f, v1 = 0.f;
+#pragma unroll
+      for (int cb = 0; cb < ND; cb++)
+#pragma unroll
+        for (int r = 0; r < 16; r += 2) {
+          v0 += v[cb][r] * v[cb][r];
+          v1 += v[cb][r + 1] * v[cb][r + 1];
+        }
+      float vr = v0 + v1;
+      vr += __shfl_xor(vr, 32, 64);
+      const float inv = 1.0f / sqrtf(vr / (float)D + 1e-5f);
+      if constexpr (MODE == 1) {
+#pragma unroll
+        for (int cb = 0; cb < ND; cb++)
+#pragma unroll
+          for (int r = 0; r < 16; r++) v[cb][r] *= inv;
+      } else {
+#pragma unroll
+        for (int cb = 0; cb < ND; cb++)
+#pragma unroll
+          for (int g = 0; g < 4; g++) {
+            const f32x4 gv = cvec(gam, cb, g), bv = cvec(bet, cb, g);
+#pragma unroll
+            for (int qq = 0; qq < 4; qq++) v[cb][4 * g + qq] = v[cb][4 * g + qq] * (inv * gv[qq]) + bv[qq];
+          }
+      }
+      return;
+    }
     float sm = 0.f;
 #pragma unroll
     for (int cb = 0; cb < ND; cb++)
@@ -1621,7 +1708,7 @@
         for (int cb = 0; cb < ND; cb++) q[cb] = __builtin_amdgcn_mfma_f32_32x32x16_bf16(ml[c][cb], ch_[s2], q[cb], 0, 0, 0);
       }
     }
-    layernorm(q, s_c + 128, s_c + 256);
+    layernorm(q, std::integral_constant<int, FOLD ? 1 : 0>{}, s_c + 128, s_c + 256);
 #pragma unroll
     for (int cb = 0; cb < ND; cb++)
 #pragma unroll
@@ -1630,7 +1717,11 @@
 #pragma unroll
     for (int cb = 0; cb < 2 * ND; cb++)
 #pragma unroll
-      for (int r = 0; r < 16; r++) f[cb][r] = 0.f;
+      for (int g = 0; g < 4; g++) {
+        const f32x4 sv = FOLD ? cvec(s_c + 128, cb, g) : f32x4{0.f, 0.f, 0.f, 0.f};
+#pragma unroll
+        for (int qq = 0; qq < 4; qq++) f[cb][4 * g + qq] = sv[qq];
+      }
 #pragma unroll
     for (int k = 4; k < 12; k++) {
       fetch(k + 1);
@@ -1663,7 +1754,7 @@
       for (int ls = 0; ls < 4; ls++) ap128_step<ND>(o, wb, ls, oh[ls], ol[ls]);
       commit(k + 1);
     }
-    layernorm(o, s_c + 384, s_c + 512);
+    layernorm(o, std::integral_constant<int, FOLD ? 2 : 0>{}, s_c + 384, s_c + 512);
 #pragma unroll
     for (int cb = 0; cb < ND; cb++)
 #pragma unroll
@@ -2045,12 +2136,47 @@
   return p.d == 64 && aps_in && aps_out && (p.Lq & 31) == 0 && (p.nhead == 1 || p.nhead == 2 || p.nhead == 4);
 }
 
+static size_t aps_lds_bytes(const pcr_attn_params &p) {
+  const int aps_c1s = (p.c1 + 15) >> 4, aps_nd = p.d >> 5;
+  return (size_t)((aps_c1s + (p.q_pos ? 2 * aps_nd : 0)) * aps_nd * 128 + (aps_c1s + 2 * aps_nd) * aps_nd * 256 +
+                  aps_nd * (p.cout >> 5) * 512) * 16 +
+         (size_t)(448 + 256 + 64 * kApsWaves) * sizeof(float);
+}
+
+static int attn_apply_form(const pcr_attn_params &p) {
+  static const int no_s128 = pcr_tune_int("PCR_ATTN_NO_STREAM128");
+  if (p.d == 128 && p.c1 == 128 && p.cout == 128 && !p.cfinal && p.q_pos && p.residual && (p.Lq & 31) == 0 && p.Lq >= 256 &&
+      (p.nhead == 1 || p.nhead == 2 || p.nhead == 4) && !no_s128)
+    return 128;
+  if (p.d == 32 && p.c1 == 32 && p.cout == 32 && !p.cfinal && (p.Lq & 31) == 0 && (p.nhead == 1 || p.nhead == 2)) return 32;
+  if (aps64_shape(p) && aps_lds_bytes(p) <= (size_t)kMaxDynLds) return 64;
+  return 0;
+}
+
+static bool attn_apply_folds(const pcr_attn_params &p) {
+  return attn_apply_form(p) != 0 && !(p.cfinal && p.residual);
+}
+
+static bool attn_kv_streams(const pcr_attn_params &p) {
+  const int tb = p.d <= 64 ? 2 : 1;
+  const int ntile = (p.Sk + 32 * tb - 1) / (32 * tb);
+  const int ns = p.kv_splits > 1 ? (p.kv_splits < ntile ? p.kv_splits : ntile) : 1;
+  if (ns != 1 || !p.wkv_bf || (p.Sk & 31) || p.c2 < p.d) return false;
+  static const int no_kv128 = pcr_tune_int("PCR_ATTN_NO_KV128");
+  if (p.d == 64) return (p.c2 == 64 || (p.c2 == 128 && p.Sk >= 128)) && 64 % p.nhead == 0;
+  if (p.d == 32) return p.c2 == 32 && 32 % p.nhead == 0;
+  if (p.d == 128) return p.c2 == 128 && p.Sk >= 256 && (p.nhead == 2 || p.nhead == 4) && !no_kv128;
+  return false;
+}
+
 static int attn_apply_launch(const pcr_attn_params *pp, pcr_stream_t stream) {
   const pcr_attn_params &p = *pp;
   AttnArgs a;
   a.p = p;
   a.dbg = 0;
   a.wpc = 0;
+  const bool fold = p.ln_folded != 0;
+  if (fold && (p.ln_folded != 3 || kAPrec == 0 || !p.ffn0_seed || !attn_apply_folds(p))) return PCR_ERR_INVALID;
   const int tb = p.d <= 32 ? 4 : (p.d <= 64 ? 2 : 1), T = 32 * tb, RP = T + 1;
   const int catP = ceil8(p.c1 + p.d);
   int rowsU = catP > 2 * p.d ? catP : 2 * p.d;
@@ -2063,28 +2189,30 @@
   hipStream_t st = pcr_s(stream);
   pcr_note_arith(kAPrec != 0 ? PCR_PREC_BF16X3 : PCR_PREC_F32);
 #if PCR_ATTN_PREC != 0
-  const int aps_c1s = (p.c1 + 15) >> 4, aps_nd = p.d >> 5;
-  const size_t aps_lds = (size_t)((aps_c1s + (p.q_pos ? 2 * aps_nd : 0)) * aps_nd * 128 + (aps_c1s + 2 * aps_nd) * aps_nd * 256 +
-                                  aps_nd * (p.cout >> 5) * 512) * 16 +
-                         (size_t)(448 + 256 + 64 * kApsWaves) * sizeof(float);
-  static const int no_s128 = pcr_tune_int("PCR_ATTN_NO_STREAM128");
-  if (p.d == 128 && p.c1 == 128 && p.cout == 128 && !p.cfinal && p.q_pos && p.residual && (p.Lq & 31) == 0 && p.Lq >= 256 &&
-      (p.nhead == 1 || p.nhead == 2 || p.nhead == 4) && !no_s128) {
+  const size_t aps_lds = aps_lds_bytes(p);
+  const int form = attn_apply_form(p);
+#define PCR_APS(...) (fold ? pcr_launch_lds<attn_apply_stream64_kernel<__VA_ARGS__, true>>(gg, bb, aps_lds, st, a) \
+                           : pcr_launch_lds<attn_apply_stream64_kernel<__VA_ARGS__, false>>(gg, bb, aps_lds, st, a))
+  if (form == 128) {
     const long nitem = (long)p.B * (p.Lq >> 5);
     const long nwg = (nitem + kAp128Waves - 1) / kAp128Waves;
     const dim3 gg((unsigned)(nwg < pcr_cu_count() ? nwg : pcr_cu_count())), bb(64 * kAp128Waves);
+    if (fold) {
+      if (p.nhead == 1) return pcr_launch_lds<attn_apply_stream128_kernel<1, true>>(gg, bb, kAp128Lds, st, a);
+      if (p.nhead == 2) return pcr_launch_lds<attn_apply_stream128_kernel<2, true>>(gg, bb, kAp128Lds, st, a);
+      return pcr_launch_lds<attn_apply_stream128_kernel<4, true>>(gg, bb, kAp128Lds, st, a);
+    }
     if (p.nhead == 1) return pcr_launch_lds<attn_apply_stream128_kernel<1>>(gg, bb, kAp128Lds, st, a);
     if (p.nhead == 2) return pcr_launch_lds<attn_apply_stream128_kernel<2>>(gg, bb, kAp128Lds, st, a);
     return pcr_launch_lds<attn_apply_stream128_kernel<4>>(gg, bb, kAp128Lds, st, a);
   }
-  if (p.d == 32 && p.c1 == 32 && p.cout == 32 && !p.cfinal && (p.Lq & 31) == 0 && (p.nhead == 1 || p.nhead == 2)) {
+  if (form == 32) {
     const long nitem = (long)p.B * (p.Lq >> 5);
     const long nwg = (nitem + kApsWaves - 1) / kApsWaves;
     const dim3 gg((unsigned)(nwg < pcr_cu_count() ? nwg : pcr_cu_count())), bb(64 * kApsWaves);
-    return p.q_pos ? pcr_launch_lds<attn_apply_stream64_kernel<true, 2, 0, 1, 1>>(gg, bb, aps_lds, st, a)
-                   : pcr_launch_lds<attn_apply_stream64_kernel<false, 2, 0, 1, 1>>(gg, bb, aps_lds, st, a);
-  }
-  if (aps64_shape(p) && aps_lds <= (size_t)kMaxDynLds) {
+    return p.q_pos ? PCR_APS(true, 2, 0, 1, 1, false) : PCR_APS(false, 2, 0, 1, 1, false);
+  }
+  if (form == 64) {
     const int nob = p.cout >> 5;
     const long nitem = (long)p.B * (p.Lq >> 5);
     const long nwg = (nitem + kApsWaves - 1) / kApsWaves;
@@ -2095,25 +2223,19 @@
     if (pp->pool_out) {
       const long nwgp = ((long)p.B + kApsWaves - 1) / kApsWaves;
       const dim3 ggp((unsigned)(nwgp < pcr_cu_count() ? nwgp : pcr_cu_count()));
-      return pcr_launch_lds<attn_apply_stream64_kernel<false, 4, 0, 2, 2, true>>(ggp, bb, aps_lds, st, a);
+      return fold ? pcr_launch_lds<attn_apply_stream64_kernel<false, 4, 0, 2, 2, true, true>>(ggp, bb, aps_lds, st, a)
+                  : pcr_launch_lds<attn_apply_stream64_kernel<false, 4, 0, 2, 2, true>>(ggp, bb, aps_lds, st, a);
     }
     int rc;
-    if (nob == 4)
-      rc = p.q_pos ? pcr_launch_lds<attn_apply_stream64_kernel<true, 4, 0, 4>>(gg, bb, aps_lds, st, a)
-                   : pcr_launch_lds<attn_apply_stream64_kernel<false, 4, 0, 4>>(gg, bb, aps_lds, st, a);
-    else if (p.c1 < 16) rc = pcr_launch_lds<attn_apply_stream64_kernel<false, 1, 2, 1>>(gg, bb, aps_lds, st, a);
-    else if (p.c1 == 32)
-      rc = cf ? pcr_launch_lds<attn_apply_stream64_kernel<false, 2, 4>>(gg, bb, aps_lds, st, a)
-              : pcr_launch_lds<attn_apply_stream64_kernel<false, 2, 0>>(gg, bb, aps_lds, st, a);
-    else if (p.q_pos)
-      rc = cf ? pcr_launch_lds<attn_apply_stream64_kernel<true, 4, 4>>(gg, bb, aps_lds, st, a)
-              : pcr_launch_lds<attn_apply_stream64_kernel<true, 4, 0>>(gg, bb, aps_lds, st, a);
-    else
-      rc = cf ? pcr_launch_lds<attn_apply_stream64_kernel<false, 4, 4>>(gg, bb, aps_lds, st, a)
-              : pcr_launch_lds<attn_apply_stream64_kernel<false, 4, 0>>(gg, bb, aps_lds, st, a);
+    if (nob == 4) rc = p.q_pos ? PCR_APS(true, 4, 0, 4, 2, false) : PCR_APS(false, 4, 0, 4, 2, false);
+    else if (p.c1 < 16) rc = PCR_APS(false, 1, 2, 1, 2, false);
+    else if (p.c1 == 32) rc = cf ? PCR_APS(false, 2, 4, 2, 2, false) : PCR_APS(false, 2, 0, 2, 2, false);
+    else if (p.q_pos) rc = cf ? PCR_APS(true, 4, 4, 2, 2, false) : PCR_APS(true, 4, 0, 2, 2, false);
+    else rc = cf ? PCR_APS(false, 4, 4, 2, 2, false) : PCR_APS(false, 4, 0, 2, 2, false);
     if (aptrace) attn_dump_trace(aptrace, "apply64", (int)gg.x, (int)p.B, p.Lq);
     return rc;
   }
+#undef PCR_APS
 #endif
   const bool wide = 2 * p.d > 128 || p.cout > 128 || p.cfinal > 128;
   if (tb == 4)
@@ -2190,9 +2312,17 @@
   return (pp && !attn_check(*pp) && attn_pool_ok(*pp)) ? 1 : 0;
 }
 
+PCR_EXPORT int pcr_attn_fold_ok(const pcr_attn_params *pp, int kv) {
+  pcr_attn_params q;
+  if (!pp || attn_check(*pp) || !attn_bf(*pp, q)) return 0;
+  if (kv) return attn_kv_streams(*pp) ? 2 : 0;
+  return attn_apply_folds(*pp) ? 3 : 0;
+}
+
 PCR_EXPORT int pcr_attn_apply_f32(const pcr_attn_params *pp, pcr_stream_t stream) {
   if (!pp || attn_check(*pp) || (!pp->out && !pp->pool_out)) return PCR_ERR_INVALID;
   if (pp->pool_out && !attn_pool_ok(*pp)) return PCR_ERR_INVALID;
+  if (pp->ln_folded && pcr_attn_fold_ok(pp, 0) != pp->ln_folded) return PCR_ERR_INVALID;
   if (pp->B == 0) return PCR_OK;
   if (pp->B > 65535) return PCR_ERR_INVALID;
   pcr_attn_params q;
diff --git a/point-cloud-reid_amd/pcr_amd/engine.py b/point-cloud-reid_amd/pcr_amd/engine.py
--- a/point-cloud-reid_amd/pcr_amd/engine.py
+++ b/point-cloud-reid_amd/pcr_amd/engine.py
@@ -134,7 +134,8 @@
                 ("precision", ctypes.c_int),
                 ("wq_bf", c_float_p), ("wmlp0_bf", c_float_p), ("wmlp2_bf", c_float_p), ("wfinal_bf", c_float_p),
                 ("kv_splits", ctypes.c_int), ("kv_part", c_float_p), ("wkv_bf", c_float_p),
-                ("wmlp0_bf_xpad", c_float_p), ("pool_out", c_float_p)]
+                ("wmlp0_bf_xpad", c_float_p), ("pool_out", c_float_p),
+                ("ffn0_seed", c_float_p), ("ln_folded", ctypes.c_int)]
 
 
 class HeadParams(ctypes.Structure):
@@ -360,6 +361,25 @@
         return out.transpose(1, 2) if out_point_major else out
 
 
+ATTN_FOLD = _os.environ.get("PCR_ATTN_FOLD", "1") != "0"
+
+
+def attn_fold(W0, W2, Wm, g1, b1, g2, b2, c1, Wf=None, bf=None):
+    cout, d = W2.shape[0], Wm.shape[0]
+    cen = lambda n: torch.eye(n, dtype=torch.float64) - torch.full((n, n), 1.0 / n, dtype=torch.float64)
+    W0f = W0.clone()
+    W0f[:, c1:] = W0[:, c1:] * g1[None, :]
+    out = dict(W2c=cen(cout) @ W2, Wmc=cen(d) @ Wm, W0f=W0f, seed=W0[:, c1:] @ b1)
+    if Wf is not None:
+        out.update(Wff=Wf * g2[None, :], bff=(bf if bf is not None else 0.0) + Wf @ b2)
+    return out
+
+
+def xpad_cols(w0, c1):
+    pad = torch.zeros(w0.shape[0], 16 * ((c1 + 15) // 16) - c1, dtype=w0.dtype)
+    return torch.cat([w0[:, :c1], pad, w0[:, c1:]], dim=1)
+
+
 class AttnPlan:
 
     def __init__(self, m, pos_name, device, nhead, q_pos, k_pos, residual, final=None):
@@ -397,8 +417,7 @@
                 self.t["wkv_bf"] = pack_weight_bf(wkv.float(), device)
             if d == 64 and self.c1 % 16:
                 w0 = m.mlp[0].weight.detach().float().cpu()
-                pad = torch.zeros(w0.shape[0], 16 * ((self.c1 + 15) // 16) - self.c1)
-                self.t["wmlp0_bf_xpad"] = pack_weight_bf(torch.cat([w0[:, :self.c1], pad, w0[:, self.c1:]], dim=1), device)
+                self.t["wmlp0_bf_xpad"] = pack_weight_bf(xpad_cols(w0, self.c1), device)
             self.t.update(wq_bf=pack_weight_bf(wq.float(), device),
                           wmlp0_bf=pack_weight_bf(m.mlp[0].weight, device), wmlp2_bf=pack_weight_bf(m.mlp[2].weight, device))
         if d > 128:
@@ -423,6 +442,27 @@
             bpad = torch.zeros((self.cfinal + 31) // 32 * 32, dtype=torch.float32, device=device)
             bpad[:self.cfinal] = final.bias.detach().to(device).float()
             self.t["bfinal"] = bpad
+        self.fold, self.tf, self.tkv = True, None, None
+        if d <= 128 and "wkv_bf" in self.t and all(getattr(x, "bias", None) is None for x in (m.mlp[0], m.mlp[2], m.merge)):
+            fin = final is not None and not residual
+            fz = attn_fold(f64(m.mlp[0].weight), f64(m.mlp[2].weight), f64(m.merge.weight), f64(m.norm1.weight),
+                           f64(m.norm1.bias), f64(m.norm2.weight), f64(m.norm2.bias), self.c1,
+                           f64(final.weight).reshape(self.cfinal, -1) if fin else None,
+                           (f64(final.bias) if final.bias is not None else None) if fin else None)
+            self.tf = dict(wmlp0_bf=pack_weight_bf(fz["W0f"].float(), device), wmlp2_bf=pack_weight_bf(fz["W2c"].float(), device),
+                           ffn0_seed=_dev32(fz["seed"].float(), device))
+            if "wmlp0_bf_xpad" in self.t:
+                self.tf["wmlp0_bf_xpad"] = pack_weight_bf(xpad_cols(fz["W0f"].float(), self.c1), device)
+            if fin:
+                bpad = torch.zeros_like(self.t["bfinal"])
+                bpad[:self.cfinal] = fz["bff"].float().to(device)
+                self.tf.update(wfinal_bf=pack_weight_bf(fz["Wff"].float(), device), bfinal=bpad)
+            self.tkv = dict(wmerge=_dev32(fz["Wmc"].float(), device))
+            if "wmerge_packed" in self.t:
+                self.tkv["wmerge_packed"] = pack_weight(fz["Wmc"].float(), device)
+
+    def _folding(self):
+        return bool(self.fold and ATTN_FOLD and self.tf is not None and PRECISION != "f32" and _LEVEL == 0)
 
     def _params(self, B, Lq, Sk, feat_q, xyz_q, feat_k, xyz_k, kv, out, kv_index=None, q_index=None):
         p = AttnParams()
@@ -451,11 +491,16 @@
         if ns > 1:
             part = torch.empty((B, ns, lib.pcr_attn_kv_floats(d)), dtype=torch.float32, device=feat_k.device)
             p.kv_splits, p.kv_part = ns, _p(part)
+        centred = self._folding() and lib.pcr_attn_fold_ok(ctypes.byref(p), 1) == 2
+        if centred:
+            for k, v in self.tkv.items():
+                setattr(p, k, _p(v))
         kv_flops = 2.0 * B * Sk * (3 * d + d * c2 + 2 * c2 * d + d * d / self.nhead)
         with _prof("attn_kv[d=%d,c2=%d,Sk=%d]" % (d, c2, Sk), kv_flops, 4.0 * B * (c2 * Sk + 3 * Sk + d * d + d),
                    arith="lib"):
             L.check(lib.pcr_attn_kv_f32(ctypes.byref(p), L.stream_ptr()), "pcr_attn_kv_f32")
         kv._pcr_precision = PRECISION
+        kv._pcr_centred = centred
         return kv
 
     def pool_ok(self, Lq, Sk):
@@ -464,7 +509,7 @@
         p.feat_q = p.feat_k = p.xyz_k = p.kv = p.out = 1
         return bool(L.load().pcr_attn_apply_pool_ok(ctypes.byref(p)))
 
-    def apply(self, feat_q, xyz_q, kv, Sk, kv_index=None, q_index=None, n_out=None, pooled=False):
+    def apply(self, feat_q, xyz_q, kv, Sk, kv_index=None, q_index=None, n_out=None, pooled=False, ln_folded=None):
         L.require_cuda(feat_q, kv)
         assert feat_q.is_contiguous() and feat_q.dtype == torch.float32 and (xyz_q is None or xyz_q.is_contiguous())
         Bq, c1, Lq = feat_q.shape
@@ -483,6 +528,18 @@
             out = torch.empty((B, self.cfinal or self.cout, Lq), dtype=torch.float32, device=feat_q.device)
             p = self._params(B, Lq, Sk, feat_q, xyz_q, feat_q, xyz_q if xyz_q is not None else feat_q, kv, out,
                              kv_index, q_index)
+        centred = bool(getattr(kv, "_pcr_centred", False))
+        if ln_folded is None:
+            ln_folded = 3 if (self._folding() and centred and L.load().pcr_attn_fold_ok(ctypes.byref(p), 0) == 3) else 0
+        if ln_folded:
+            if ln_folded != 3 or self.tf is None:
+                raise L.PcrError("ln_folded = %r: this plan has no such images" % (ln_folded,))
+            if not centred:
+                raise L.PcrError("ln_folded = 3 needs an attention state written from centred merge rows (AttnPlan.kv with "
+                                 "the fold on); this one is not marked as such")
+            for k, v in self.tf.items():
+                setattr(p, k, _p(v))
+            p.ln_folded = ln_folded
         d = self.d
         ap_flops = 2.0 * B * Lq * (c1 * d + d * d / self.nhead + d * d + (c1 + d) * 2 * d + 2 * d * self.cout
                                    + self.cout * self.cfinal + (self.q_pos * (3 * d + d * c1)))
```
